# zengxiaofei/HapHiC

Hardware: NVIDIA H100
Metric: hic_pairs_per_sec_matrix_build (higher is better)
Workload: dtype int32 counts / fp32 matrix

## Files before the change

### haphic_b200/_lib.py

```python

from __future__ import annotations

import ctypes as C
import weakref
import os

import numpy as np

HERE = os.path.dirname(os.path.abspath(__file__))
LIB_PATH = os.path.join(HERE, "libhaphic_b200.so")

HH_MEM_HOST, HH_MEM_DEVICE = 0, 1


class HHError(RuntimeError):
    pass


class LinksInfo(C.Structure):
    _fields_ = [("n_records", C.c_int64), ("n_used", C.c_int64), ("nnz_full", C.c_int64), ("nnz_flank", C.c_int64),
                ("table_slots", C.c_int64)]


class MclResult(C.Structure):
    _fields_ = [("rounds", C.c_int32), ("converged", C.c_int32), ("nnz", C.c_int64), ("products", C.c_int64),
                ("bytes", C.c_int64)]


class PreexpInfo(C.Structure):
    _fields_ = [("mode", C.c_int32), ("a_planes", C.c_int32), ("passes", C.c_int32), ("cta_group", C.c_int32),
                ("stages", C.c_int32), ("chunk_kb", C.c_int32), ("total_ms", C.c_float), ("densify_ms", C.c_float),
                ("gemm_ms", C.c_float), ("clip_ms", C.c_float), ("flops", C.c_double), ("products", C.c_int64),
                ("clip", C.c_float), ("b_planes", C.c_int32), ("fmt_a", C.c_int32), ("fmt_b", C.c_int32), ("k_chunks", C.c_int32)]


class MclStepInfo(C.Structure):
    _fields_ = [("it", C.c_int32), ("iter0", C.c_int32), ("iter0_w", C.c_int32), ("blk", C.c_int32), ("blk_f16", C.c_int32),
                ("blk_chunk", C.c_int32), ("blk_ldk", C.c_int64), ("n_win", C.c_int32), ("n_big", C.c_int32),
                ("wmax", C.c_int32), ("small", C.c_int32), ("small_cols", C.c_int32), ("small_overflow", C.c_int32),
                ("col", C.c_int32), ("col_cols", C.c_int32), ("col_w", C.c_int32), ("col_smem", C.c_int32),
                ("col_track", C.c_int32), ("col_flat", C.c_int32)]


class CorrectRoundInfo(C.Structure):
    _fields_ = [("n_examined", C.c_int32), ("n_broken", C.c_int32), ("n_breaks", C.c_int32), ("n_frag", C.c_int32),
                ("n_links", C.c_int64)]


HH_PREEXP_AUTO, HH_PREEXP_SPARSE, HH_PREEXP_DENSE = 0, 1, 2

_P = C.c_void_p
_SIGNATURES = {
    "hh_version": (C.c_int, []),
    "hh_last_error": (C.c_char_p, []),
    "hh_ctx_create": (C.c_int, [C.c_int, C.POINTER(_P)]),
    "hh_ctx_destroy": (C.c_int, [_P]),
    "hh_ctx_sync": (C.c_int, [_P]),
    "hh_ctx_stream": (_P, [_P]),
    "hh_ctx_device": (C.c_int, [_P]),
    "hh_ctx_sm_count": (C.c_int, [_P]),
    "hh_ctx_launches": (C.c_int64, [_P]),
    "hh_ctx_mem_available": (C.c_int, [_P, C.POINTER(C.c_size_t)]),
    "hh_links_create": (C.c_int, [_P, C.c_int32, _P, _P, _P, C.c_int64, C.c_int64, C.POINTER(_P)]),
    "hh_links_create_frags": (C.c_int, [_P, C.c_int32, _P, _P, C.c_int32, _P, _P, _P, C.c_int64, C.c_int64, C.c_int64,
                                        C.POINTER(_P)]),
    "hh_links_add": (C.c_int, [_P, _P, C.c_int64, C.c_int64, C.c_int]),
    "hh_links_add_async": (C.c_int, [_P, _P, C.c_int64, C.c_int64]),
    "hh_links_finish": (C.c_int, [_P, C.POINTER(LinksInfo)]),
    "hh_links_agg_info": (C.c_int, [_P, C.POINTER(C.c_int64), C.POINTER(C.c_int64), C.POINTER(C.c_int64)]),
    "hh_links_fetch": (C.c_int, [_P, _P, _P, _P, _P, _P, _P, _P]),
    "hh_links_fetch_phased": (C.c_int, [_P, _P, C.c_double, _P, _P, _P, _P, C.POINTER(C.c_int64)]),
    "hh_links_set_ul_pairs": (C.c_int, [_P, _P, _P, _P, C.c_int64]),
    "hh_links_fetch_ctg": (C.c_int, [_P, _P]),
    "hh_stats_create": (C.c_int, [_P, C.c_int32, _P, _P, _P, _P, C.c_int64, C.POINTER(_P)]),
    "hh_stats_rank": (C.c_int, [_P, _P, C.c_int32, C.POINTER(C.c_int64)]),
    "hh_stats_fetch_ranked": (C.c_int, [_P, _P, _P, _P, _P]),
    "hh_stats_best": (C.c_int, [_P, _P, C.c_int32, _P, C.c_int, _P, _P, _P, _P, _P, _P]),
    "hh_stats_destroy": (C.c_int, [_P]),
    "hh_links_export": (C.c_int, [_P, _P, _P]),
    "hh_links_merge": (C.c_int, [_P, _P, C.c_int64, _P, C.c_int64, C.c_int64]),
    "hh_links_route": (C.c_int, [_P, _P, C.c_int64, C.c_int64, C.c_int, _P, _P, _P]),
    "hh_links_add_routed": (C.c_int, [_P, _P, _P, C.c_int64]),
    "hh_links_finish_partition": (C.c_int, [_P, _P]),
    "hh_links_adopt": (C.c_int, [_P, _P, C.c_int64, _P, C.c_int64, C.c_int64, C.c_int64]),
    "hh_links_destroy": (C.c_int, [_P]),
    "hh_links_linked_index": (C.c_int, [_P, _P, _P, C.POINTER(C.c_int32)]),
    "hh_matrix_from_links": (C.c_int, [_P, _P, _P, C.c_int32, C.c_int, C.c_int, C.POINTER(_P)]),
    "hh_links_linked_index_phased": (C.c_int, [_P, _P, C.c_int, _P, C.c_double, _P, C.POINTER(C.c_int32)]),
    "hh_matrix_from_links_phased": (C.c_int, [_P, _P, _P, C.c_int32, C.c_int, C.c_int, _P, C.c_double, C.POINTER(_P)]),
    "hh_matrix_from_links_ex": (C.c_int, [_P, _P, _P, C.c_int32, C.c_int, C.c_int, _P, C.c_double, _P, _P, C.POINTER(_P)]),
    "hh_matrix_rank_sums": (C.c_int, [_P, C.c_int, _P]),
    "hh_matrix_from_csc": (C.c_int, [_P, C.c_int32, _P, _P, _P, C.POINTER(_P)]),
    "hh_matrix_info": (C.c_int, [_P, C.POINTER(C.c_int32), C.POINTER(C.c_int64)]),
    "hh_matrix_fetch_csc": (C.c_int, [_P, _P, _P, _P]),
    "hh_matrix_destroy": (C.c_int, [_P]),
    "hh_mcl_create": (C.c_int, [_P, C.c_int, C.c_int32, C.c_int32, C.POINTER(_P)]),
    "hh_mcl_create_ex": (C.c_int, [_P, C.c_int, C.c_int32, C.c_int32, C.c_int, C.POINTER(_P)]),
    "hh_mcl_choose_preexp": (C.c_int, [_P, C.c_int, C.c_int, C.POINTER(C.c_int)]),
    "hh_mcl_footprint": (C.c_int, [_P, C.c_int, C.c_int32, C.c_int, C.c_double, C.POINTER(C.c_size_t), C.POINTER(C.c_size_t)]),
    "hh_mcl_preexp_info": (C.c_int, [_P, C.POINTER(PreexpInfo)]),
    "hh_mcl_info": (C.c_int, [_P, C.POINTER(C.c_int32), C.POINTER(C.c_int64), C.POINTER(C.c_int64),
                              C.POINTER(C.c_float), C.POINTER(C.c_float)]),
    "hh_mcl_fetch_m0": (C.c_int, [_P, _P, _P, _P]),
    "hh_mcl_fetch_m1": (C.c_int, [_P, _P]),
    "hh_mcl_fetch_m1_cols": (C.c_int, [_P, C.c_int32, C.c_int32, _P]),
    "hh_mcl_run": (C.c_int, [_P, C.c_double, C.c_int, C.c_double, C.POINTER(MclResult), _P, _P, _P, _P]),
    "hh_mcl_fetch_result": (C.c_int, [_P, _P, _P, _P]),
    "hh_mcl_begin": (C.c_int, [_P, C.c_double, C.c_double]),
    "hh_mcl_step": (C.c_int, [_P, C.c_int, C.POINTER(C.c_int64), C.POINTER(C.c_int64), C.POINTER(C.c_float),
                              C.POINTER(C.c_float)]),
    "hh_mcl_pack": (C.c_int, [_P, _P, _P, _P]),
    "hh_mcl_unpack": (C.c_int, [_P, C.c_int32, C.c_int32, _P, _P, _P, C.c_int64]),
    "hh_mcl_commit": (C.c_int, [_P]),
    "hh_mcl_step_info": (C.c_int, [_P, C.POINTER(MclStepInfo)]),
    "hh_mcl_set_block": (C.c_int, [_P, C.c_int32, C.c_int32]),
    "hh_mcl_destroy": (C.c_int, [_P]),
    "hh_correct_create": (C.c_int, [_P, C.c_int32, _P, C.c_int64, C.POINTER(_P)]),
    "hh_correct_add": (C.c_int, [_P, _P, C.c_int64, C.c_int]),
    "hh_correct_round": (C.c_int, [_P, C.c_double, C.c_double, C.c_int64, C.c_int, C.POINTER(CorrectRoundInfo)]),
    "hh_correct_fetch_breaks": (C.c_int, [_P, _P, _P, _P]),
    "hh_correct_info": (C.c_int, [_P, C.POINTER(C.c_int32), C.POINTER(C.c_int64), C.POINTER(C.c_int64)]),
    "hh_correct_fetch_cov": (C.c_int, [_P, _P, _P, _P]),
    "hh_correct_set_layout": (C.c_int, [_P, _P, _P, _P, C.c_int32]),
    "hh_correct_remap": (C.c_int, [_P, _P, _P, C.c_int64, C.c_int]),
    "hh_correct_destroy": (C.c_int, [_P]),
    "hh_contact_create": (C.c_int, [_P, C.c_int32, _P, _P, _P, _P, _P, _P, C.c_int32, C.c_int64, C.POINTER(_P)]),
    "hh_contact_load": (C.c_int, [_P, C.c_int32, _P, C.POINTER(_P)]),
    "hh_contact_add": (C.c_int, [_P, _P, C.c_int64, C.c_int]),
    "hh_contact_add_async": (C.c_int, [_P, _P, C.c_int64]),
    "hh_contact_error": (C.c_int, [_P, C.POINTER(C.c_int64), C.POINTER(C.c_int32), C.POINTER(C.c_int32),
                                   C.POINTER(C.c_int64)]),
    "hh_contact_finish": (C.c_int, [_P]),
    "hh_contact_info": (C.c_int, [_P, C.POINTER(C.c_int32), C.POINTER(C.c_int32), C.POINTER(C.c_int64)]),
    "hh_contact_fetch": (C.c_int, [_P, _P]),
    "hh_contact_kr": (C.c_int, [_P, C.c_int32, _P, _P, C.c_double, C.c_double, C.c_double, C.c_int32, C.c_int32, _P, _P,
                                _P, _P]),
    "hh_contact_normalize": (C.c_int, [_P, C.c_int, C.c_int32, _P, _P, _P, _P, _P, C.POINTER(C.c_double),
                                       C.POINTER(C.c_double), C.POINTER(C.c_int64)]),
    "hh_contact_destroy": (C.c_int, [_P]),
    "hh_pairs_open":(C.c_int, [C.c_char_p, _P, C.c_int32, C.c_char_p, C.c_int, C.c_int, C.POINTER(_P)]),
    "hh_pairs_next": (C.c_int, [_P, _P, C.c_int64, C.POINTER(C.c_int64)]),
    "hh_pairs_close": (C.c_int, [_P]),
    "hh_pairs_write": (C.c_int, [C.c_char_p, _P, C.c_int32, _P, C.c_int64, C.c_int64, C.c_int, C.c_int]),
    "hh_bam_open": (C.c_int, [C.c_char_p, C.c_char_p, C.c_int32, C.c_int, C.c_int, C.POINTER(_P)]),
    "hh_bam_header_text": (C.c_int, [_P, C.POINTER(C.c_char_p), C.POINTER(C.c_int64)]),
    "hh_bam_next": (C.c_int, [_P, _P, C.c_int64, C.POINTER(C.c_int64)]),
    "hh_bam_close": (C.c_int, [_P]),
    "hh_ul_open": (C.c_int, [C.c_char_p, C.c_int, C.c_int32, C.c_int64, C.c_int64, C.c_double, C.c_int64, C.POINTER(_P)]),
    "hh_ul_info": (C.c_int, [_P, C.POINTER(C.c_int32), C.POINTER(C.c_int64), C.POINTER(C.c_int64), C.POINTER(C.c_int64)]),
    "hh_ul_fetch": (C.c_int, [_P, _P, _P, _P]),
    "hh_ul_close": (C.c_int, [_P]),
    "hh_pickle_links": (C.c_int, [C.c_char_p, _P, C.c_int32, _P, _P, C.c_int64, _P, _P, _P]),
    "hh_pickle_links_mixed": (C.c_int, [C.c_char_p, _P, C.c_int32, _P, _P, C.c_int64, _P, _P]),
    "hh_clm_from_records": (C.c_int, [C.c_char_p, _P, C.c_int32, _P, C.c_int64, _P, _P, C.c_int]),
}

_lib = None


def exported_symbols():
    return sorted(_SIGNATURES)


def load():
    global _lib
    if _lib is not None:
        return _lib
    if not os.path.exists(LIB_PATH):
        raise HHError(
            "{} is missing: build it with `python -c 'import __graft_entry__ as g; g.build()'` "
            "(or `python -m haphic_b200.build`). haphic_b200 has no CPU fallback.".format(LIB_PATH))
    lib = C.CDLL(LIB_PATH)
    for name, (res, args) in _SIGNATURES.items():
        fn = getattr(lib, name)
        fn.restype = res
        fn.argtypes = args
    _lib = lib
    return lib


def check(rc: int):
    if rc != 0:
        msg = load().hh_last_error()
        raise HHError("libhaphic_b200 error {}: {}".format(rc, msg.decode() if msg else "?"))


def ptr(x):
    if x is None:
        return None
    if isinstance(x, np.ndarray):
        return x.ctypes.data_as(C.c_void_p)
    if hasattr(x, "data_ptr"):
        return C.c_void_p(x.data_ptr())
    if isinstance(x, int):
        return C.c_void_p(x)
    raise TypeError("cannot take the address of {!r}".format(type(x)))


class Context:

    def __init__(self, device: int = 0):
        self._h = C.c_void_p()
        lib = load()
        check(lib.hh_ctx_create(int(device), C.byref(self._h)))
        self.device = int(device)
        self._children = weakref.WeakSet()

    def adopt(self, obj):
        self._children.add(obj)

    @property
    def handle(self):
        if not self._h:
            raise HHError("context already closed")
        return self._h

    def sync(self):
        check(load().hh_ctx_sync(self.handle))

    @property
    def stream(self) -> int:
        return int(load().hh_ctx_stream(self.handle) or 0)

    @property
    def sm_count(self) -> int:
        return load().hh_ctx_sm_count(self.handle)

    @property
    def launches(self) -> int:
        return int(load().hh_ctx_launches(self.handle))

    def close(self):
        if self._h:
            for obj in sorted(self._children, key=lambda o: -getattr(o, "_close_order", 0)):
                obj.close()
            load().hh_ctx_destroy(self._h)
            self._h = C.c_void_p()

    def __enter__(self):
        return self

    def __exit__(self, *exc):
        self.close()

    def __del__(self):
        try:
            self.close()
        except Exception:
            pass
```

### haphic_b200/csrc/hh_common.cuh

```cuda
#pragma once

#include <cuda_runtime.h>
#include <stdint.h>
#include <stdio.h>
#include <stdarg.h>
#include <string.h>
#include <new>
#include <vector>

#include "../../include/haphic_b200.h"

void hh_set_error(const char* fmt, ...);

#define HH_CUDA(expr)                                                                         \
    do {                                                                                      \
        cudaError_t _e = (expr);                                                              \
        if (_e != cudaSuccess) {                                                              \
            hh_set_error("%s:%d: %s failed: %s", __FILE__, __LINE__, #expr, cudaGetErrorString(_e)); \
            return (_e == cudaErrorMemoryAllocation) ? HH_ERR_NOMEM : HH_ERR_CUDA;            \
        }                                                                                     \
    } while (0)

#define HH_CHECK(expr)                                                                        \
    do {                                                                                      \
        int _rc = (expr);                                                                     \
        if (_rc != HH_OK) return _rc;                                                         \
    } while (0)

#define HH_REQUIRE(cond, code, ...)                                                           \
    do {                                                                                      \
        if (!(cond)) {                                                                        \
            hh_set_error(__VA_ARGS__);                                                        \
            return (code);                                                                    \
        }                                                                                     \
    } while (0)

#define HH_LAUNCH(ctx, kernel, grid, block, smem, ...)                                        \
    do {                                                                                      \
        kernel<<<(grid), (block), (smem), (ctx)->stream>>>(__VA_ARGS__);                      \
        (ctx)->launches++;                                                                    \
        HH_CUDA(cudaGetLastError());                                                          \
    } while (0)

struct hh_ctx {
    int device;
    int sm_count;
    size_t smem_optin;
    size_t l2_bytes;
    cudaStream_t stream;
    int64_t launches;
    uint64_t* h_scratch;
    uint64_t* d_scratch;
    struct ws_block {
        void* p;
        size_t bytes;
        bool used;
        uint64_t tick;
    };
    std::vector<ws_block>* ws;
    uint64_t ws_tick;
};

void* hh_ws_alloc_bytes(hh_ctx* ctx, size_t bytes);
bool hh_ws_release(hh_ctx* ctx, void* p);
void hh_ws_free_ptr(hh_ctx* ctx, void* p);
template <typename T>
static inline int hh_ws_alloc(hh_ctx* ctx, T** p, size_t count) {
    *p = reinterpret_cast<T*>(hh_ws_alloc_bytes(ctx, (count ? count : 1) * sizeof(T)));
    return *p ? HH_OK : HH_ERR_NOMEM;
}
template <typename T>
static inline void hh_ws_free(hh_ctx* ctx, T*& p) {
    if (p) hh_ws_free_ptr(ctx, (void*)p);
    p = nullptr;
}

extern thread_local hh_ctx* hh_tls_ctx;
struct hh_scope {
    hh_ctx* prev;
    explicit hh_scope(hh_ctx* c) : prev(hh_tls_ctx) {
        hh_tls_ctx = c;
        if (c) cudaSetDevice(c->device);
    }
    ~hh_scope() { hh_tls_ctx = prev; }
};

#define HH_WS_MIN ((size_t)32 << 20)
template <typename T>
static inline int hh_dmalloc(T** p, size_t count) {
    *p = nullptr;
    if (count == 0) count = 1;
    if (hh_tls_ctx && count * sizeof(T) >= HH_WS_MIN) {
        *p = reinterpret_cast<T*>(hh_ws_alloc_bytes(hh_tls_ctx, count * sizeof(T)));
        return *p ? HH_OK : HH_ERR_NOMEM;
    }
    cudaError_t e = hh_tls_ctx ? cudaMallocAsync((void**)p, count * sizeof(T), hh_tls_ctx->stream)
                               : cudaMalloc((void**)p, count * sizeof(T));
    if (e != cudaSuccess) {
        hh_set_error("cudaMalloc of %zu bytes failed: %s", count * sizeof(T), cudaGetErrorString(e));
        cudaGetLastError();
        return HH_ERR_NOMEM;
    }
    return HH_OK;
}
template <typename T>
static inline void hh_dfree(T*& p) {
    if (p) {
        if (hh_ws_release(hh_tls_ctx, (void*)p)) {
        } else if (hh_tls_ctx) {
            cudaFreeAsync((void*)p, hh_tls_ctx->stream);
        } else {
            cudaFree((void*)p);
        }
    }
    p = nullptr;
}

#define HH_FULL_MASK 0xffffffffu

__device__ __forceinline__ int hh_lane() { return threadIdx.x & 31; }
__device__ __forceinline__ int hh_warp() { return threadIdx.x >> 5; }

__device__ __forceinline__ double hh_warp_sum(double v) {
#pragma unroll
    for (int o = 16; o > 0; o >>= 1) v += __shfl_xor_sync(HH_FULL_MASK, v, o);
    return v;
}
__device__ __forceinline__ int hh_warp_sum(int v) {
#pragma unroll
    for (int o = 16; o > 0; o >>= 1) v += __shfl_xor_sync(HH_FULL_MASK, v, o);
    return v;
}
__device__ __forceinline__ unsigned long long hh_warp_sum(unsigned long long v) {
#pragma unroll
    for (int o = 16; o > 0; o >>= 1) v += __shfl_xor_sync(HH_FULL_MASK, v, o);
    return v;
}
template <typename T>
__device__ __forceinline__ T hh_warp_incl_scan(T v) {
#pragma unroll
    for (int o = 1; o < 32; o <<= 1) {
        const T t = __shfl_up_sync(HH_FULL_MASK, v, o);
        if (hh_lane() >= o) v += t;
    }
    return v;
}
__device__ __forceinline__ float hh_warp_max(float v) {
#pragma unroll
    for (int o = 16; o > 0; o >>= 1) v = fmaxf(v, __shfl_xor_sync(HH_FULL_MASK, v, o));
    return v;
}

__device__ __forceinline__ int4 hh_ld_stream(const int4* p) {
    int4 r;
    asm volatile("ld.global.nc.L1::no_allocate.v4.s32 {%0, %1, %2, %3}, [%4];"
                 : "=r"(r.x), "=r"(r.y), "=r"(r.z), "=r"(r.w)
                 : "l"(p));
    return r;
}
__device__ __forceinline__ float4 hh_ld_stream_f4(const float4* p) {
    float4 r;
    asm volatile("ld.global.nc.L1::no_allocate.v4.f32 {%0, %1, %2, %3}, [%4];"
                 : "=f"(r.x), "=f"(r.y), "=f"(r.z), "=f"(r.w)
                 : "l"(p));
    return r;
}

template <typename K>
static inline int hh_resident_grid(hh_ctx* ctx, K kernel, int threads, size_t smem, int* grid) {
    int per_sm = 0;
    HH_CUDA(cudaOccupancyMaxActiveBlocksPerMultiprocessor(&per_sm, kernel, threads, smem));
    HH_REQUIRE(per_sm > 0, HH_ERR_CUDA, "a kernel of %d threads and %zu bytes of shared memory does not fit an SM", threads, smem);
    *grid = ctx->sm_count * per_sm;
    return HH_OK;
}

__global__ void hh_k_scan_small(const int* __restrict__ in, int64_t* __restrict__ out, int n);
int hh_exclusive_scan_i32(hh_ctx* ctx, const int* d_in, int64_t* d_out, int n);
```

### haphic_b200/csrc/hh_links.cu

```cuda
#include "hh_common.cuh"
#include "hh_internal.cuh"
#include <cub/cub.cuh>
#include <stdlib.h>
#include <algorithm>
#include <vector>

#define HH_EMPTY_KEY 0xFFFFFFFFFFFFFFFFull
#define HH_NONE32 0xFFFFFFFFu

struct __align__(32) hh_slot {
    uint32_t first_full, first_flank, full, flank, ht, th, tt, pad;
};

struct hh_partset {
    int4* buf;
    unsigned long long* cursor;
    uint64_t pcap;
    int64_t sized_for, sent;
};

struct hh_links {
    hh_ctx* ctx;
    int32_t n_ctg;
    int64_t flank_bp;
    int32_t* d_len;
    int32_t* d_rank;
    uint8_t* d_nx;
    int32_t n_src;
    int32_t* d_src_rank;
    int32_t* d_fbase;
    int64_t bin_size;
    unsigned long long* d_ctg;
    uint64_t* d_keys;
    hh_slot* d_vals;
    uint64_t cap;
    unsigned long long* d_counters;
    int64_t n_records, stream_end;
    int64_t known_unique, since_known;
    bool finished;
    bool ordered;
    int64_t nnz, nnz_flank, n_used;
    int64_t peer_used;
    uint32_t* d_compact;
    int4* d_stage[2];
    cudaEvent_t ev_copied[2], ev_consumed[2];
    cudaStream_t copy_stream;
    int64_t stage_records;
    int mode;
    int npart_log;
    uint64_t scap;
    int64_t agg_buckets, agg_smem, agg_fallback;
    uint64_t spill_cap;
    std::vector<hh_partset> psets;
    int4* d_spill;
    unsigned long long* d_spill_cursor;
    int64_t capacity_hint;
    int32_t* d_index;
    int32_t n_linked;
    uint8_t* d_keep;
    int32_t* d_hap;
    bool phased;
    int32_t* d_deg;
    int64_t n_pass;
    uint64_t gen;
    bool ix_valid;
    uint64_t ix_gen;
    int ix_normalize;
    double ix_w;
    std::vector<uint8_t> ix_keep;
    std::vector<int32_t> ix_hap;
    unsigned long long* d_ul_key = nullptr;
    int32_t* d_ul_slot = nullptr;
    int64_t n_ul = 0;
};

__device__ __forceinline__ uint64_t hh_mix64(uint64_t k) {
    k ^= k >> 33;
    k *= 0xff51afd7ed558ccdull;
    k ^= k >> 33;
    k *= 0xc4ceb9fe1a85ec53ull;
    k ^= k >> 33;
    return k;
}

__device__ __forceinline__ uint64_t hh_probe_insert(uint64_t* __restrict__ keys, uint64_t cap, uint64_t key, bool* inserted) {
    const uint64_t mask = cap - 1;
    uint64_t slot = hh_mix64(key) & mask;
    *inserted = false;
    for (uint64_t probes = 0; probes < cap; ++probes) {
        uint64_t k = *((volatile uint64_t*)(keys + slot));
        if (k == key) return slot;
        if (k == HH_EMPTY_KEY) {
            unsigned long long prev = atomicCAS((unsigned long long*)(keys + slot), (unsigned long long)HH_EMPTY_KEY,
                                                (unsigned long long)key);
            if (prev == HH_EMPTY_KEY) {
                *inserted = true;
                return slot;
            }
            if (prev == key) return slot;
        }
        slot = (slot + 1) & mask;
    }
    return cap;
}

__global__ void hh_k_links_init(uint64_t* __restrict__ keys, hh_slot* __restrict__ vals, uint64_t cap) {
    const uint64_t stride = (uint64_t)gridDim.x * blockDim.x;
    for (uint64_t s = (uint64_t)blockIdx.x * blockDim.x + threadIdx.x; s < cap; s += stride) {
        keys[s] = HH_EMPTY_KEY;
        uint4* v = reinterpret_cast<uint4*>(vals + s);
        v[0] = make_uint4(HH_NONE32, HH_NONE32, 0u, 0u);
        v[1] = make_uint4(0u, 0u, 0u, 0u);
    }
}

#define HH_F_FLANK 1u
#define HH_F_TI 2u
#define HH_F_TJ 4u

struct hh_pair {
    int a, b;
    unsigned flags;
};

__device__ __forceinline__ uint64_t hh_pair_key(int a, int b) { return ((uint64_t)(uint32_t)a << 32) | (uint64_t)(uint32_t)b; }

__device__ __forceinline__ void hh_swap_ends(int& a, int& b, int& pa, int& pb) {
    int t = a; a = b; b = t;
    t = pa; pa = pb; pb = t;
}

__device__ __forceinline__ void hh_pair_flags(int a, int b, int pa, int pb, const int32_t* __restrict__ ctg_len,
                                              const uint8_t* __restrict__ in_nx, int64_t flank_bp, hh_pair* out) {
    const int64_t coord_i = (int64_t)pa + 1, coord_j = (int64_t)pb + 1;
    const int64_t li = ctg_len[a], lj = ctg_len[b];
    const bool fi = (flank_bp == 0) || (coord_i <= flank_bp) || (coord_i > li - flank_bp);
    const bool fj = (flank_bp == 0) || (coord_j <= flank_bp) || (coord_j > lj - flank_bp);
    out->a = a;
    out->b = b;
    out->flags = ((fi && fj && in_nx[a] && in_nx[b]) ? HH_F_FLANK : 0u)
                 | ((coord_i * 2 > li) ? HH_F_TI : 0u) | ((coord_j * 2 > lj) ? HH_F_TJ : 0u);
}

__device__ __forceinline__ bool hh_classify_contig(int4 r, int32_t n_ctg, const int32_t* __restrict__ ctg_len,
                                                   const int32_t* __restrict__ name_rank, const uint8_t* __restrict__ in_nx,
                                                   int64_t flank_bp, hh_pair* out) {
    int a = r.x, b = r.z, pa = r.y, pb = r.w;
    if (a == b || (unsigned)a >= (unsigned)n_ctg || (unsigned)b >= (unsigned)n_ctg) return false;
    if (name_rank[a] > name_rank[b]) hh_swap_ends(a, b, pa, pb);
    hh_pair_flags(a, b, pa, pb, ctg_len, in_nx, flank_bp, out);
    return true;
}

__device__ __forceinline__ int64_t hh_floor_div(int64_t x, int64_t d) { return x >= 0 ? x / d : -((-x + d - 1) / d); }

__device__ __forceinline__ bool hh_to_bin(int& f, int& p, int nbins, int64_t bin_size) {
    const int64_t nb = ((int64_t)p + 1 + bin_size - 1) / bin_size;
    const bool exists = p >= 0 && nb >= 1 && nb <= (int64_t)nbins;
    f += (int)(nb - 1);
    p = (int)((int64_t)p - (nb - 1) * bin_size);
    return exists;
}

__device__ __forceinline__ bool hh_classify_frag(int4 r, int32_t n_src, const int32_t* __restrict__ src_rank,
                                                 const int32_t* __restrict__ fbase, int64_t bin_size, const int32_t* __restrict__ ctg_len,
                                                 const int32_t* __restrict__ name_rank, const uint8_t* __restrict__ in_nx,
                                                 int64_t flank_bp, uint32_t idx, unsigned long long* __restrict__ counters,
                                                 hh_pair* out) {
    int a = r.x, b = r.z, pa = r.y, pb = r.w;
    if ((unsigned)a >= (unsigned)n_src || (unsigned)b >= (unsigned)n_src) return false;
    if (a == b && fbase[a + 1] - fbase[a] <= 1) return false;
    if (src_rank[a] > src_rank[b] || (a == b && pa > pb)) hh_swap_ends(a, b, pa, pb);
    int fa = fbase[a], fb = fbase[b];
    const int na = fbase[a + 1] - fa, nb = fbase[b + 1] - fb;
    if (a == b && hh_floor_div((int64_t)pa, bin_size) == hh_floor_div((int64_t)pb, bin_size)) return false;
    bool bad = false;
    if (na > 1) bad = !hh_to_bin(fa, pa, na, bin_size);
    if (nb > 1) bad = !hh_to_bin(fb, pb, nb, bin_size) || bad;
    if (bad) {
        atomicAdd(counters + 5, 1ull);
        atomicMax(counters + 6, (unsigned long long)idx + 1ull);
        return false;
    }
    if (fa == fb) return false;
    if ((na > 1 || nb > 1) && name_rank[fa] > name_rank[fb]) hh_swap_ends(fa, fb, pa, pb);
    hh_pair_flags(fa, fb, pa, pb, ctg_len, in_nx, flank_bp, out);
    return true;
}

struct hh_group {
    bool leader;
    uint32_t first_all, first_flank;
    unsigned full, flank, ht, th, tt;
};

__device__ __forceinline__ hh_group hh_warp_fold(bool ok, uint64_t key, uint32_t idx, unsigned flags) {
    const int lane = threadIdx.x & 31;
    if (!ok) key = HH_EMPTY_KEY - 1 - (uint64_t)lane;
    const unsigned peers = __match_any_sync(HH_FULL_MASK, key);
    const bool fl = ok && (flags & HH_F_FLANK), ti = (flags & HH_F_TI) != 0, tj = (flags & HH_F_TJ) != 0;
    hh_group g;
    g.first_all = __reduce_min_sync(peers, ok ? idx : HH_NONE32);
    g.first_flank = __reduce_min_sync(peers, fl ? idx : HH_NONE32);
    const unsigned b_fl = __ballot_sync(HH_FULL_MASK, fl);
    const unsigned b_ht = __ballot_sync(HH_FULL_MASK, ok && !ti && tj);
    const unsigned b_th = __ballot_sync(HH_FULL_MASK, ok && ti && !tj);
    const unsigned b_tt = __ballot_sync(HH_FULL_MASK, ok && ti && tj);
    g.leader = ok && lane == (__ffs(peers) - 1);
    g.full = __popc(peers);
    g.flank = __popc(peers & b_fl);
    g.ht = __popc(peers & b_ht);
    g.th = __popc(peers & b_th);
    g.tt = __popc(peers & b_tt);
    return g;
}

__device__ __forceinline__ void hh_slot_update(hh_slot* v, const hh_group& g) {
    atomicAdd(&v->full, g.full);
    atomicMin(&v->first_full, g.first_all);
    if (g.flank) {
        atomicAdd(&v->flank, g.flank);
        atomicMin(&v->first_flank, g.first_flank);
    }
    if (g.ht) atomicAdd(&v->ht, g.ht);
    if (g.th) atomicAdd(&v->th, g.th);
    if (g.tt) atomicAdd(&v->tt, g.tt);
}

__device__ __forceinline__ void hh_entry_store(uint32_t* __restrict__ o, uint64_t key, uint32_t full, uint32_t flank, uint32_t first_full,
                                               uint32_t first_flank, uint32_t ht, uint32_t th, uint32_t tt) {
    o[HH_E_I] = (uint32_t)(key >> 32);
    o[HH_E_J] = (uint32_t)key;
    o[HH_E_FULL] = full;
    o[HH_E_FLANK] = flank;
    o[HH_E_FIRST_FULL] = first_full;
    o[HH_E_FIRST_FLANK] = first_flank;
    o[HH_E_HT] = ht;
    o[HH_E_TH] = th;
    o[HH_E_TT] = tt;
}

__device__ __forceinline__ void hh_entry_store(uint32_t* __restrict__ o, uint64_t key, uint4 v0, uint4 v1) {
    hh_entry_store(o, key, v0.z, v0.w, v0.x, v0.y, v1.x, v1.y, v1.z);
}

__device__ __forceinline__ unsigned int hh_block_rank(unsigned int cnt, unsigned int* s_wtot, unsigned int* total) {
    const int lane = threadIdx.x & 31, wv = threadIdx.x >> 5;
    unsigned int incl = cnt;
#pragma unroll
    for (int o = 1; o < 32; o <<= 1) {
        const unsigned int t = __shfl_up_sync(HH_FULL_MASK, incl, o);
        if (lane >= o) incl += t;
    }
    __syncthreads();
    if (lane == 31) s_wtot[wv] = incl;
    __syncthreads();
    unsigned int before = 0, all = 0;
#pragma unroll
    for (int k = 0; k < 8; ++k) {
        const unsigned int t = s_wtot[k];
        before += (k < wv) ? t : 0u;
        all += t;
    }
    *total = all;
    return before + incl - cnt;
}

__global__ void __launch_bounds__(256)
hh_k_links_insert(const int4* __restrict__ rec, int64_t n_rec, uint32_t stream_off, int32_t n_ctg,
                  const int32_t* __restrict__ ctg_len, const int32_t* __restrict__ name_rank,
                  const uint8_t* __restrict__ in_nx, int64_t flank_bp, uint64_t* __restrict__ keys,
                  hh_slot* __restrict__ vals, uint64_t cap, unsigned long long* __restrict__ ctg_links,
                  unsigned long long* __restrict__ counters, const int32_t* __restrict__ src_rank,
                  const int32_t* __restrict__ fbase, int64_t bin_size, int32_t n_src, const uint32_t* __restrict__ pos) {
    __shared__ unsigned int s_new, s_used, s_over;
    if (threadIdx.x == 0) {
        s_new = 0;
        s_used = 0;
        s_over = 0;
    }
    __syncthreads();
    const int lane = threadIdx.x & 31;
    const int64_t stride = (int64_t)gridDim.x * blockDim.x;
    unsigned int my_new = 0, my_used = 0;
    for (int64_t i0 = (int64_t)blockIdx.x * blockDim.x + (threadIdx.x - lane); i0 < n_rec; i0 += stride) {
        const int64_t i = i0 + lane;
        bool ok = i < n_rec;
        hh_pair p = {0, 0, 0u};
        uint32_t idx = HH_NONE32;
        if (ok) {
            const int4 r = hh_ld_stream(rec + i);
            idx = pos ? pos[i] : stream_off + (uint32_t)i;
            ok = fbase == nullptr ? hh_classify_contig(r, n_ctg, ctg_len, name_rank, in_nx, flank_bp, &p)
                                  : hh_classify_frag(r, n_src, src_rank, fbase, bin_size, ctg_len, name_rank, in_nx, flank_bp, idx,
                                                     counters, &p);
        }
        if (ok) my_used++;
        const uint64_t key = hh_pair_key(p.a, p.b);
        const hh_group g = hh_warp_fold(ok, key, idx, p.flags);
        if (g.leader) {
            bool inserted;
            const uint64_t slot = hh_probe_insert(keys, cap, key, &inserted);
            if (slot >= cap) {
                s_over = 1;
            } else {
                if (inserted) my_new++;
                hh_slot_update(vals + slot, g);
                if (g.flank) {
                    atomicAdd(ctg_links + p.a, (unsigned long long)g.flank);
                    atomicAdd(ctg_links + p.b, (unsigned long long)g.flank);
                }
            }
        }
    }
    if (my_new) atomicAdd(&s_new, my_new);
    if (my_used) atomicAdd(&s_used, my_used);
    __syncthreads();
    if (threadIdx.x == 0) {
        if (s_new) atomicAdd(counters + 0, (unsigned long long)s_new);
        if (s_used) atomicAdd(counters + 1, (unsigned long long)s_used);
        if (s_over) atomicExch(counters + 2, 1ull);
    }
}

#define HH_PART_TILE 4096
#define HH_PART_MAX 1024

#define HH_STAGE_SMEM ((size_t)HH_PART_TILE * sizeof(int4))

__device__ __forceinline__ unsigned int hh_tile_scan(unsigned int* c, int n, unsigned int* s_wtot) {
    const int lane = threadIdx.x & 31, wv = threadIdx.x >> 5;
    const int per = (n + 511) >> 9, lo = threadIdx.x * per;
    __syncthreads();
    unsigned int sum = 0;
    for (int k = 0; k < per; ++k)
        if (lo + k < n) sum += c[lo + k];
    unsigned int incl = sum;
#pragma unroll
    for (int o = 1; o < 32; o <<= 1) {
        const unsigned int t = __shfl_up_sync(HH_FULL_MASK, incl, o);
        if (lane >= o) incl += t;
    }
    if (lane == 31) s_wtot[wv] = incl;
    __syncthreads();
    unsigned int run = incl - sum, all = 0;
#pragma unroll
    for (int k = 0; k < 16; ++k) {
        const unsigned int t = s_wtot[k];
        run += (k < wv) ? t : 0u;
        all += t;
    }
    for (int k = 0; k < per; ++k) {
        if (lo + k < n) {
            const unsigned int t = c[lo + k];
            c[lo + k] = run;
            run += t;
        }
    }
    __syncthreads();
    return all;
}

__global__ void __launch_bounds__(512, 2)
hh_k_part_scatter(const int4* __restrict__ rec, int64_t n_rec, uint32_t stream_off, int32_t n_ctg, const int32_t* __restrict__ ctg_len,
                  const int32_t* __restrict__ name_rank, const uint8_t* __restrict__ in_nx, int64_t flank_bp, int npart_log,
                  int4* __restrict__ pbuf, uint64_t pcap, unsigned long long* __restrict__ cursor, int4* __restrict__ spill,
                  uint64_t spill_cap, unsigned long long* __restrict__ spill_cursor, unsigned long long* __restrict__ counters) {
    extern __shared__ int4 s_stage[];
    __shared__ unsigned int s_cnt[HH_PART_MAX];
    __shared__ unsigned long long s_base[HH_PART_MAX];
    __shared__ unsigned int s_wtot[16];
    __shared__ unsigned int s_used;
    const int npart = 1 << npart_log;
    const int64_t tiles = (n_rec + HH_PART_TILE - 1) / HH_PART_TILE;
    unsigned int my_used = 0;
    if (threadIdx.x == 0) s_used = 0;
    for (int64_t t = blockIdx.x; t < tiles; t += gridDim.x) {
        for (int k = threadIdx.x; k < npart; k += 512) s_cnt[k] = 0;
        __syncthreads();
        int4 out[8];
        unsigned int rnk[8];
#pragma unroll
        for (int k = 0; k < 8; ++k) {
            const int64_t i = t * HH_PART_TILE + (int64_t)k * 512 + threadIdx.x;
            rnk[k] = HH_NONE32;
            if (i < n_rec) {
                hh_pair pr;
                if (hh_classify_contig(hh_ld_stream(rec + i), n_ctg, ctg_len, name_rank, in_nx, flank_bp, &pr)) {
                    const int p = (int)(hh_mix64(hh_pair_key(pr.a, pr.b)) >> (64 - npart_log));
                    rnk[k] = atomicAdd(&s_cnt[p], 1u);
                    out[k] = make_int4(pr.a, pr.b, (int)(stream_off + (uint32_t)i), (int)(pr.flags | ((unsigned)p << 8)));
                    my_used++;
                }
            }
        }
        __syncthreads();
        for (int k = threadIdx.x; k < npart; k += 512)
            if (s_cnt[k]) s_base[k] = atomicAdd(cursor + k, (unsigned long long)s_cnt[k]);
        const unsigned int n_tile = hh_tile_scan(s_cnt, npart, s_wtot);
#pragma unroll
        for (int k = 0; k < 8; ++k)
            if (rnk[k] != HH_NONE32) s_stage[s_cnt[(unsigned)out[k].w >> 8] + rnk[k]] = out[k];
        __syncthreads();
        for (unsigned int e = threadIdx.x; e < n_tile; e += 512) {
            const int4 r = s_stage[e];
            const unsigned int p = (unsigned)r.w >> 8;
            const unsigned long long q = s_base[p] + (e - s_cnt[p]);
            if (q < pcap) {
                pbuf[(size_t)p * (size_t)pcap + (size_t)q] = r;
            } else {
                const unsigned long long sq = atomicAdd(spill_cursor, 1ull);
                if (sq < spill_cap) spill[sq] = r;
                else atomicExch(counters + 2, 3ull);
            }
        }
        __syncthreads();
    }
    my_used = (unsigned)hh_warp_sum((int)my_used);
    if ((threadIdx.x & 31) == 0 && my_used) atomicAdd(&s_used, my_used);
    __syncthreads();
    if (threadIdx.x == 0 && s_used) atomicAdd(counters + 1, (unsigned long long)s_used);
}

#define HH_AGG_MEAN 2048
#define HH_SUB_MAX_LOG 12
#define HH_AGG_SLOTS 2048
#define HH_AGG_LIST (HH_AGG_SLOTS / 4 * 3)
#define HH_AGG_THREADS 256
#define HH_AGG_HOT 32

__device__ __forceinline__ uint32_t hh_bucket_of(int4 r, int bucket_log) {
    return (uint32_t)(hh_mix64(hh_pair_key(r.x, r.y)) >> (64 - bucket_log));
}

__global__ void __launch_bounds__(512)
hh_k_part_hist(const int4* __restrict__ pbuf, uint64_t pcap, const unsigned long long* __restrict__ cursor, int npart_log, int64_t tpr,
               const int4* __restrict__ spill, int64_t n_spill, int bucket_log, unsigned int* __restrict__ bcnt) {
    __shared__ unsigned int s_cnt[1 << HH_SUB_MAX_LOG];
    const int sub_log = bucket_log - npart_log, nsub = 1 << sub_log;
    const int64_t region_tiles = ((int64_t)1 << npart_log) * tpr;
    const int64_t tiles = region_tiles + (n_spill + HH_PART_TILE - 1) / HH_PART_TILE;
    for (int64_t t = blockIdx.x; t < tiles; t += gridDim.x) {
        if (t >= region_tiles) {
            const int64_t base = (t - region_tiles) * HH_PART_TILE;
            for (int k = threadIdx.x; k < HH_PART_TILE; k += 512)
                if (base + k < n_spill) atomicAdd(bcnt + hh_bucket_of(hh_ld_stream(spill + base + k), bucket_log), 1u);
            continue;
        }
        const int p = (int)(t / tpr);
        const uint64_t start = (uint64_t)(t % tpr) * HH_PART_TILE;
        const uint64_t fill = min((uint64_t)cursor[p], pcap);
        if (start >= fill) continue;
        for (int k = threadIdx.x; k < nsub; k += 512) s_cnt[k] = 0;
        __syncthreads();
        const int4* reg = pbuf + (size_t)p * (size_t)pcap;
#pragma unroll
        for (int k = 0; k < 8; ++k) {
            const uint64_t i = start + (uint64_t)k * 512 + threadIdx.x;
            if (i < fill) atomicAdd(&s_cnt[hh_bucket_of(hh_ld_stream(reg + i), bucket_log) & (nsub - 1)], 1u);
        }
        __syncthreads();
        for (int k = threadIdx.x; k < nsub; k += 512)
            if (s_cnt[k]) atomicAdd(bcnt + ((size_t)p << sub_log) + k, s_cnt[k]);
        __syncthreads();
    }
}

__global__ void __launch_bounds__(512, 2)
hh_k_part_scatter2(const int4* __restrict__ pbuf, uint64_t pcap, const unsigned long long* __restrict__ cursor, int npart_log, int64_t tpr,
                   const int4* __restrict__ spill, int64_t n_spill, int bucket_log, const int64_t* __restrict__ boff,
                   unsigned int* __restrict__ bfill, int4* __restrict__ out, uint64_t n_out, unsigned long long* __restrict__ counters) {
    extern __shared__ int4 s_stage[];
    __shared__ unsigned int s_cnt[1 << HH_SUB_MAX_LOG];
    __shared__ unsigned int s_base[1 << HH_SUB_MAX_LOG];
    __shared__ unsigned int s_wtot[16];
    const int sub_log = bucket_log - npart_log, nsub = 1 << sub_log;
    const int64_t region_tiles = ((int64_t)1 << npart_log) * tpr;
    const int64_t tiles = region_tiles + (n_spill + HH_PART_TILE - 1) / HH_PART_TILE;
    for (int64_t t = blockIdx.x; t < tiles; t += gridDim.x) {
        if (t >= region_tiles) {
            const int64_t base = (t - region_tiles) * HH_PART_TILE;
            for (int k = threadIdx.x; k < HH_PART_TILE; k += 512) {
                if (base + k >= n_spill) break;
                const int4 r = hh_ld_stream(spill + base + k);
                const uint32_t b = hh_bucket_of(r, bucket_log);
                const uint64_t q = (uint64_t)boff[b] + atomicAdd(bfill + b, 1u);
                if (q < n_out) out[q] = r;
                else atomicExch(counters + 2, 6ull);
            }
            continue;
        }
        const int p = (int)(t / tpr);
        const uint64_t start = (uint64_t)(t % tpr) * HH_PART_TILE;
        const uint64_t fill = min((uint64_t)cursor[p], pcap);
        if (start >= fill) continue;
        for (int k = threadIdx.x; k < nsub; k += 512) s_cnt[k] = 0;
        __syncthreads();
        const int4* reg = pbuf + (size_t)p * (size_t)pcap;
        int4 r[8];
        uint32_t at[8];
#pragma unroll
        for (int k = 0; k < 8; ++k) {
            const uint64_t i = start + (uint64_t)k * 512 + threadIdx.x;
            at[k] = HH_NONE32;
            if (i < fill) {
                r[k] = hh_ld_stream(reg + i);
                const uint32_t sub = hh_bucket_of(r[k], bucket_log) & (nsub - 1);
                at[k] = (sub << 16) | atomicAdd(&s_cnt[sub], 1u);
            }
        }
        __syncthreads();
        for (int k = threadIdx.x; k < nsub; k += 512)
            if (s_cnt[k]) s_base[k] = atomicAdd(bfill + ((size_t)p << sub_log) + k, s_cnt[k]);
        const unsigned int n_tile = hh_tile_scan(s_cnt, nsub, s_wtot);
#pragma unroll
        for (int k = 0; k < 8; ++k)
            if (at[k] != HH_NONE32) s_stage[s_cnt[at[k] >> 16] + (at[k] & 0xFFFFu)] = r[k];
        __syncthreads();
        for (unsigned int e = threadIdx.x; e < n_tile; e += 512) {
            const int4 rec = s_stage[e];
            const uint32_t sub = hh_bucket_of(rec, bucket_log) & (nsub - 1);
            const size_t b = ((size_t)p << sub_log) + sub;
            const uint64_t q = (uint64_t)boff[b] + s_base[sub] + (e - s_cnt[sub]);
            if (q < n_out) out[q] = rec;
            else atomicExch(counters + 2, 6ull);
        }
        __syncthreads();
    }
}

#define HH_PK_FLANK 12
#define HH_PK_HT 24
#define HH_PK_TH 36
#define HH_PK_TT 48
#define HH_PK_MASK 0xFFFull
#define HH_PK_HEAD (1ull << 63)

struct hh_run {
    unsigned long long c;
    uint32_t first_full, first_flank;
};

struct hh_run_op {
    __device__ __forceinline__ hh_run operator()(const hh_run& a, const hh_run& b) const {
        if (b.c & HH_PK_HEAD) return b;
        return hh_run{a.c + b.c, min(a.first_full, b.first_full), min(a.first_flank, b.first_flank)};
    }
};

template <typename K>
__device__ __forceinline__ int hh_lower_bound(const K* a, int n, K k) {
    int lo = 0, hi = n;
    while (lo < hi) {
        const int mid = (lo + hi) >> 1;
        if (a[mid] < k) lo = mid + 1;
        else hi = mid;
    }
    return lo;
}

template <typename K, int ITEMS>
struct hh_bc_smem {
    typedef cub::BlockRadixSort<K, HH_AGG_THREADS, ITEMS, uint32_t> sort_t;
    typedef cub::BlockScan<hh_run, HH_AGG_THREADS> run_scan_t;
    typedef cub::BlockScan<unsigned int, HH_AGG_THREADS> cnt_scan_t;
    K key[HH_AGG_LIST];
    uint32_t val[HH_E_WORDS - 2][HH_AGG_LIST];
    uint32_t z[HH_AGG_THREADS * ITEMS];
    union {
        typename sort_t::TempStorage sort;
        struct {
            K first[HH_AGG_THREADS], last[HH_AGG_THREADS];
        } edge;
        K fresh[HH_AGG_THREADS * ITEMS];
    } u;
    typename run_scan_t::TempStorage run_scan;
    typename cnt_scan_t::TempStorage cnt_scan;
    unsigned long long base;
    int bucket;
};

template <typename K, int ITEMS>
__global__ void __launch_bounds__(HH_AGG_THREADS, 3)
hh_k_bucket_count(const int4* __restrict__ rec, const int64_t* __restrict__ boff, int nbuckets, uint64_t hot, int kbits,
                  uint32_t* __restrict__ compact, uint64_t compact_cap, unsigned long long* __restrict__ ctg_links,
                  unsigned long long* __restrict__ counters, unsigned long long* __restrict__ agg, uint32_t* __restrict__ fallback) {
    typedef hh_bc_smem<K, ITEMS> smem_t;
    constexpr int S = HH_AGG_THREADS * ITEMS;
    extern __shared__ __align__(16) unsigned char hh_agg_smem[];
    smem_t& sm = *reinterpret_cast<smem_t*>(hh_agg_smem);
    const int t = threadIdx.x;
    const K jmask = ((K)1 << kbits) - 1;
    const hh_run none = {HH_PK_HEAD, HH_NONE32, HH_NONE32};
    unsigned int nfl = 0, n_done = 0;
    for (;;) {
        __syncthreads();
        if (t == 0) sm.bucket = (int)atomicAdd(agg + 0, 1ull);
        __syncthreads();
        const int bk = sm.bucket;
        if (bk >= nbuckets) break;
        const int64_t lo = boff[bk], n = boff[bk + 1] - lo;
        if ((uint64_t)n > hot) {
            if (t == 0) fallback[atomicAdd(agg + 1, 1ull)] = (uint32_t)bk;
            continue;
        }
        int tsize = HH_AGG_THREADS;
        while (tsize < HH_AGG_SLOTS && (int64_t)tsize * 2 < n * 3) tsize <<= 1;
        const int limit = tsize / 4 * 3;
        int na = 0;
        bool abandon = false;
        for (int64_t c0 = 0; c0 < n; c0 += S) {
            const int m = (int)min((int64_t)S, n - c0);
            K key[ITEMS];
            uint32_t pay[ITEMS];
            __syncthreads();
#pragma unroll
            for (int q = 0; q < ITEMS; ++q) {
                const int l = q * HH_AGG_THREADS + t;
                key[q] = ~(K)0;
                pay[q] = 0;
                if (l < m) {
                    const int4 r = hh_ld_stream(rec + lo + c0 + l);
                    key[q] = ((K)(uint32_t)r.x << kbits) | (K)(uint32_t)r.y;
                    pay[q] = (uint32_t)l | (((uint32_t)r.w & 7u) << 11);
                    sm.z[l] = (uint32_t)r.z;
                }
            }
            typename smem_t::sort_t(sm.u.sort).Sort(key, pay, 0, 2 * kbits);
            __syncthreads();
            sm.u.edge.first[t] = key[0];
            sm.u.edge.last[t] = key[ITEMS - 1];
            __syncthreads();
            const K prev = t > 0 ? sm.u.edge.last[t - 1] : ~(K)0;
            const K next = t + 1 < HH_AGG_THREADS ? sm.u.edge.first[t + 1] : ~(K)0;
            auto item = [&](int q) -> hh_run {
                const int pos = t * ITEMS + q;
                if (pos >= m) return none;
                const unsigned f = (pay[q] >> 11) & 7u;
                const uint32_t z = sm.z[pay[q] & 0x7FFu];
                const bool fl = f & HH_F_FLANK, ti = f & HH_F_TI, tj = f & HH_F_TJ;
                hh_run r;
                const bool head = pos == 0 || key[q] != (q ? key[q - 1] : prev);
                r.c = 1ull | ((unsigned long long)head << 63) | ((unsigned long long)fl << HH_PK_FLANK) | ((unsigned long long)(!ti && tj) << HH_PK_HT) |
                      ((unsigned long long)(ti && !tj) << HH_PK_TH) | ((unsigned long long)(ti && tj) << HH_PK_TT);
                r.first_full = z;
                r.first_flank = fl ? z : HH_NONE32;
                return r;
            };
            const hh_run_op op;
            hh_run acc = item(0);
#pragma unroll
            for (int q = 1; q < ITEMS; ++q) acc = op(acc, item(q));
            hh_run carry;
            typename smem_t::run_scan_t(sm.run_scan).ExclusiveScan(acc, carry, hh_run{0ull, HH_NONE32, HH_NONE32}, op);
            unsigned int nnew = 0;
            hh_run run = carry;
#pragma unroll
            for (int q = 0; q < ITEMS; ++q) {
                run = op(run, item(q));
                const int pos = t * ITEMS + q;
                if (pos < m && (pos + 1 == m || key[q] != (q + 1 < ITEMS ? key[q + 1] : next))) {
                    const int lb = hh_lower_bound(sm.key, na, key[q]);
                    if (lb < na && sm.key[lb] == key[q]) {
                        sm.val[HH_E_FULL - 2][lb] += (uint32_t)(run.c & HH_PK_MASK);
                        sm.val[HH_E_FLANK - 2][lb] += (uint32_t)((run.c >> HH_PK_FLANK) & HH_PK_MASK);
                        sm.val[HH_E_FIRST_FULL - 2][lb] = min(sm.val[HH_E_FIRST_FULL - 2][lb], run.first_full);
                        sm.val[HH_E_FIRST_FLANK - 2][lb] = min(sm.val[HH_E_FIRST_FLANK - 2][lb], run.first_flank);
                        sm.val[HH_E_HT - 2][lb] += (uint32_t)((run.c >> HH_PK_HT) & HH_PK_MASK);
                        sm.val[HH_E_TH - 2][lb] += (uint32_t)((run.c >> HH_PK_TH) & HH_PK_MASK);
                        sm.val[HH_E_TT - 2][lb] += (uint32_t)((run.c >> HH_PK_TT) & HH_PK_MASK);
                    } else {
                        pay[q] |= (uint32_t)(lb + 1) << 16;
                        nnew++;
                    }
                }
            }
            unsigned int rank, fresh;
            typename smem_t::cnt_scan_t(sm.cnt_scan).ExclusiveSum(nnew, rank, fresh);
            if (na + (int)fresh > limit) {
                abandon = true;
                break;
            }
            if (fresh == 0) continue;
            if (na) {
                unsigned int r = rank;
#pragma unroll
                for (int q = 0; q < ITEMS; ++q)
                    if (pay[q] >> 16) sm.u.fresh[r++] = key[q];
                __syncthreads();
                for (int hi = na; hi > 0; hi -= HH_AGG_THREADS) {
                    const int a = hi - HH_AGG_THREADS + t;
                    K k = 0;
                    uint32_t v[HH_E_WORDS - 2];
                    int d = a;
                    if (a >= 0) {
                        k = sm.key[a];
#pragma unroll
                        for (int w = 0; w < HH_E_WORDS - 2; ++w) v[w] = sm.val[w][a];
                        d = a + hh_lower_bound(sm.u.fresh, (int)fresh, k);
                    }
                    __syncthreads();
                    if (d > a) {
                        sm.key[d] = k;
#pragma unroll
                        for (int w = 0; w < HH_E_WORDS - 2; ++w) sm.val[w][d] = v[w];
                    }
                    __syncthreads();
                }
            }
            run = carry;
#pragma unroll
            for (int q = 0; q < ITEMS; ++q) {
                run = op(run, item(q));
                if ((pay[q] >> 16) == 0) continue;
                const int d = (int)(pay[q] >> 16) - 1 + (int)rank++;
                const hh_run& o = run;
                sm.key[d] = key[q];
                sm.val[HH_E_FULL - 2][d] = (uint32_t)(o.c & HH_PK_MASK);
                sm.val[HH_E_FLANK - 2][d] = (uint32_t)((o.c >> HH_PK_FLANK) & HH_PK_MASK);
                sm.val[HH_E_FIRST_FULL - 2][d] = o.first_full;
                sm.val[HH_E_FIRST_FLANK - 2][d] = o.first_flank;
                sm.val[HH_E_HT - 2][d] = (uint32_t)((o.c >> HH_PK_HT) & HH_PK_MASK);
                sm.val[HH_E_TH - 2][d] = (uint32_t)((o.c >> HH_PK_TH) & HH_PK_MASK);
                sm.val[HH_E_TT - 2][d] = (uint32_t)((o.c >> HH_PK_TT) & HH_PK_MASK);
            }
            na += (int)fresh;
        }
        if (abandon) {
            if (t == 0) fallback[atomicAdd(agg + 1, 1ull)] = (uint32_t)bk;
            continue;
        }
        __syncthreads();
        if (t == 0) sm.base = na ? atomicAdd(counters + 0, (unsigned long long)na) : 0ull;
        __syncthreads();
        const unsigned long long base = sm.base;
        for (int w = t; w < na * HH_E_WORDS; w += HH_AGG_THREADS) {
            const int e = w / HH_E_WORDS, f = w - e * HH_E_WORDS;
            const uint32_t x = f == HH_E_I ? (uint32_t)(sm.key[e] >> kbits)
                             : f == HH_E_J ? (uint32_t)(sm.key[e] & jmask) : sm.val[f - 2][e];
            if (base + e < compact_cap) compact[base * HH_E_WORDS + w] = x;
            else atomicExch(counters + 2, 5ull);
        }
        for (int e = t; e < na; e += HH_AGG_THREADS) {
            const uint32_t flank = sm.val[HH_E_FLANK - 2][e];
            if (flank) {
                nfl++;
                atomicAdd(ctg_links + (uint32_t)(sm.key[e] >> kbits), (unsigned long long)flank);
                atomicAdd(ctg_links + (uint32_t)(sm.key[e] & jmask), (unsigned long long)flank);
            }
        }
        n_done++;
    }
    nfl = (unsigned)hh_warp_sum((int)nfl);
    if ((t & 31) == 0 && nfl) atomicAdd(counters + 3, (unsigned long long)nfl);
    if (t == 0 && n_done) atomicAdd(agg + 2, (unsigned long long)n_done);
}

#define HH_FB_BATCH (1 << 19)

__global__ void hh_k_gather_buckets(const int4* __restrict__ src, const int64_t* __restrict__ src_off, const int64_t* __restrict__ pre,
                                    int nf, int4* __restrict__ dst) {
    const int64_t total = pre[nf];
    const int64_t stride = (int64_t)gridDim.x * blockDim.x;
    for (int64_t i = (int64_t)blockIdx.x * blockDim.x + threadIdx.x; i < total; i += stride) {
        int lo = 0, hi = nf - 1;
        while (lo < hi) {
            const int mid = (lo + hi + 1) >> 1;
            if (pre[mid] <= i) lo = mid;
            else hi = mid - 1;
        }
        dst[i] = hh_ld_stream(src + src_off[lo] + (i - pre[lo]));
    }
}

__device__ __forceinline__ void hh_part_count(const int4* __restrict__ prec, int64_t n, uint64_t* __restrict__ keys,
                                              hh_slot* __restrict__ vals, uint64_t cap, unsigned long long* __restrict__ counters) {
    const int lane = threadIdx.x & 31;
    const int64_t stride = (int64_t)gridDim.x * blockDim.x;
    for (int64_t i0 = (int64_t)blockIdx.x * blockDim.x + (threadIdx.x - lane); i0 < n; i0 += stride) {
        const int64_t i = i0 + lane;
        const bool ok = i < n;
        int4 r = make_int4(0, 0, 0, 0);
        if (ok) r = hh_ld_stream(prec + i);
        const uint64_t key = hh_pair_key(r.x, r.y);
        const hh_group g = hh_warp_fold(ok, key, (uint32_t)r.z, (unsigned)r.w);
        if (g.leader) {
            bool inserted;
            const uint64_t slot = hh_probe_insert(keys, cap, key, &inserted);
            if (slot >= cap) atomicExch(counters + 2, 4ull);
            else hh_slot_update(vals + slot, g);
        }
    }
}

__global__ void __launch_bounds__(256)
hh_k_part_step(const int4* __restrict__ prec, int64_t n, uint64_t* __restrict__ ckeys, hh_slot* __restrict__ cvals,
               uint64_t* __restrict__ ekeys, hh_slot* __restrict__ evals, uint64_t cap, uint32_t* __restrict__ compact,
               uint64_t compact_cap, unsigned long long* __restrict__ ctg_links, unsigned long long* __restrict__ counters) {
    if (ekeys != nullptr) {
        __shared__ unsigned int s_wtot[8];
        __shared__ unsigned long long s_base;
        unsigned int nfl = 0;
        constexpr int E = 2;
        for (uint64_t r0 = (uint64_t)blockIdx.x * (256ull * E); r0 < cap; r0 += (uint64_t)gridDim.x * (256ull * E)) {
            uint64_t key[E];
            unsigned int cnt = 0;
#pragma unroll
            for (int q = 0; q < E; ++q) {
                const uint64_t sl = r0 + (uint64_t)q * 256ull + threadIdx.x;
                key[q] = (sl < cap) ? ekeys[sl] : HH_EMPTY_KEY;
                cnt += (key[q] != HH_EMPTY_KEY) ? 1u : 0u;
            }
            unsigned int total;
            const unsigned int rank = hh_block_rank(cnt, s_wtot, &total);
            if (threadIdx.x == 0) s_base = total ? atomicAdd(counters + 0, (unsigned long long)total) : 0ull;
            __syncthreads();
            if (cnt) {
                unsigned long long pos = s_base + rank;
                uint4 v0[E], v1[E];
#pragma unroll
                for (int q = 0; q < E; ++q) {
                    if (key[q] != HH_EMPTY_KEY) {
                        const uint4* vp = reinterpret_cast<const uint4*>(evals + (r0 + (uint64_t)q * 256ull + threadIdx.x));
                        v0[q] = vp[0];
                        v1[q] = vp[1];
                    }
                }
#pragma unroll
                for (int q = 0; q < E; ++q) {
                    if (key[q] == HH_EMPTY_KEY) continue;
                    const uint64_t sl = r0 + (uint64_t)q * 256ull + threadIdx.x;
                    if (pos < compact_cap) hh_entry_store(compact + pos * HH_E_WORDS, key[q], v0[q], v1[q]);
                    else atomicExch(counters + 2, 5ull);
                    pos++;
                    if (v0[q].w) {
                        nfl++;
                        atomicAdd(ctg_links + (uint32_t)(key[q] >> 32), (unsigned long long)v0[q].w);
                        atomicAdd(ctg_links + (uint32_t)key[q], (unsigned long long)v0[q].w);
                    }
                    ekeys[sl] = HH_EMPTY_KEY;
                    uint4* vw = reinterpret_cast<uint4*>(evals + sl);
                    vw[0] = make_uint4(HH_NONE32, HH_NONE32, 0u, 0u);
                    vw[1] = make_uint4(0u, 0u, 0u, 0u);
                }
            }
        }
        nfl = (unsigned)hh_warp_sum((int)nfl);
        if ((threadIdx.x & 31) == 0 && nfl) atomicAdd(counters + 3, (unsigned long long)nfl);
    }
    if (ckeys != nullptr && n > 0) hh_part_count(prec, n, ckeys, cvals, cap, counters);
}

__global__ void hh_k_links_rehash(const uint64_t* __restrict__ okeys, const hh_slot* __restrict__ ovals, uint64_t ocap,
                                  uint64_t* __restrict__ keys, hh_slot* __restrict__ vals, uint64_t cap,
                                  unsigned long long* __restrict__ counters) {
    const uint64_t stride = (uint64_t)gridDim.x * blockDim.x;
    for (uint64_t s = (uint64_t)blockIdx.x * blockDim.x + threadIdx.x; s < ocap; s += stride) {
        const uint64_t k = okeys[s];
        if (k == HH_EMPTY_KEY) continue;
        bool inserted;
        const uint64_t slot = hh_probe_insert(keys, cap, k, &inserted);
        if (slot >= cap) {
            atomicExch(counters + 2, 1ull);
            continue;
        }
        const uint4* src = reinterpret_cast<const uint4*>(ovals + s);
        uint4* dst = reinterpret_cast<uint4*>(vals + slot);
        dst[0] = src[0];
        dst[1] = src[1];
    }
}

__global__ void hh_k_links_merge(const uint32_t* __restrict__ ent, int64_t n_ent, uint64_t* __restrict__ keys,
                                 hh_slot* __restrict__ vals, uint64_t cap, unsigned long long* __restrict__ counters) {
    __shared__ unsigned int s_new;
    if (threadIdx.x == 0) s_new = 0;
    __syncthreads();
    const int64_t stride = (int64_t)gridDim.x * blockDim.x;
    unsigned int my_new = 0, my_last = 0;
    for (int64_t e = (int64_t)blockIdx.x * blockDim.x + threadIdx.x; e < n_ent; e += stride) {
        const uint32_t* p = ent + e * HH_E_WORDS;
        const uint64_t key = ((uint64_t)p[HH_E_I] << 32) | (uint64_t)p[HH_E_J];
        bool inserted;
        const uint64_t slot = hh_probe_insert(keys, cap, key, &inserted);
        if (slot >= cap) {
            atomicExch(counters + 2, 1ull);
            continue;
        }
        if (inserted) my_new++;
        hh_slot* v = vals + slot;
        atomicAdd(&v->full, p[HH_E_FULL]);
        if (p[HH_E_FLANK]) atomicAdd(&v->flank, p[HH_E_FLANK]);
        atomicMin(&v->first_full, p[HH_E_FIRST_FULL]);
        atomicMin(&v->first_flank, p[HH_E_FIRST_FLANK]);
        my_last = max(my_last, p[HH_E_FIRST_FULL]);
        if (p[HH_E_HT]) atomicAdd(&v->ht, p[HH_E_HT]);
        if (p[HH_E_TH]) atomicAdd(&v->th, p[HH_E_TH]);
        if (p[HH_E_TT]) atomicAdd(&v->tt, p[HH_E_TT]);
    }
    if (my_new) atomicAdd(&s_new, my_new);
    my_last = __reduce_max_sync(HH_FULL_MASK, my_last);
    if ((threadIdx.x & 31) == 0 && my_last) atomicMax(counters + 4, (unsigned long long)my_last);
    __syncthreads();
    if (threadIdx.x == 0 && s_new) atomicAdd(counters + 0, (unsigned long long)s_new);
}

__global__ void hh_k_add_u64(unsigned long long* __restrict__ dst, const int64_t* __restrict__ src, int n) {
    int i = blockIdx.x * blockDim.x + threadIdx.x;
    if (i < n) dst[i] += (unsigned long long)src[i];
}

#define HH_MAX_WORLD 64

__device__ __forceinline__ int hh_owner(int a, int b, int world) {
    const uint32_t lo = (uint32_t)min(a, b), hi = (uint32_t)max(a, b);
    return (int)(hh_mix64(((uint64_t)lo << 32) | (uint64_t)hi) % (uint64_t)world);
}

__device__ __forceinline__ int hh_route_dest(const int4 r, int n_src, bool contig_mode, int world) {
    if ((unsigned)r.x >= (unsigned)n_src || (unsigned)r.z >= (unsigned)n_src) return -1;
    if (contig_mode && r.x == r.z) return -1;
    return hh_owner(r.x, r.z, world);
}

__global__ void __launch_bounds__(256)
hh_k_route_count(const int4* __restrict__ rec, int64_t n_rec, int n_src, int contig_mode, int world,
                 unsigned long long* __restrict__ counts) {
    __shared__ unsigned int s_cnt[HH_MAX_WORLD];
    if (threadIdx.x < HH_MAX_WORLD) s_cnt[threadIdx.x] = 0;
    __syncthreads();
    const int64_t stride = (int64_t)gridDim.x * blockDim.x;
    for (int64_t i = (int64_t)blockIdx.x * blockDim.x + threadIdx.x; i < n_rec; i += stride) {
        const int d = hh_route_dest(hh_ld_stream(rec + i), n_src, contig_mode != 0, world);
        if (d >= 0) atomicAdd(&s_cnt[d], 1u);
    }
    __syncthreads();
    if (threadIdx.x < world && s_cnt[threadIdx.x]) atomicAdd(counts + threadIdx.x, (unsigned long long)s_cnt[threadIdx.x]);
}

__global__ void __launch_bounds__(256)
hh_k_route_scatter(const int4* __restrict__ rec, int64_t n_rec, uint32_t stream_off, int n_src, int contig_mode, int world,
                   unsigned long long* __restrict__ cursor, int4* __restrict__ rec_out, uint32_t* __restrict__ pos_out) {
    __shared__ unsigned int s_cnt[HH_MAX_WORLD];
    __shared__ unsigned long long s_base[HH_MAX_WORLD];
    const int64_t tiles = (n_rec + 255) / 256;
    for (int64_t t = blockIdx.x; t < tiles; t += gridDim.x) {
        if (threadIdx.x < HH_MAX_WORLD) s_cnt[threadIdx.x] = 0;
        __syncthreads();
        const int64_t i = t * 256 + threadIdx.x;
        int4 r = make_int4(-1, 0, -1, 0);
        int d = -1;
        unsigned int my = 0;
        if (i < n_rec) {
            r = hh_ld_stream(rec + i);
            d = hh_route_dest(r, n_src, contig_mode != 0, world);
            if (d >= 0) my = atomicAdd(&s_cnt[d], 1u);
        }
        __syncthreads();
        if (threadIdx.x < world && s_cnt[threadIdx.x])
            s_base[threadIdx.x] = atomicAdd(cursor + threadIdx.x, (unsigned long long)s_cnt[threadIdx.x]);
        __syncthreads();
        if (d >= 0) {
            const unsigned long long q = s_base[d] + my;
            rec_out[q] = r;
            pos_out[q] = stream_off + (uint32_t)i;
        }
        __syncthreads();
    }
}

__global__ void hh_k_links_mark_slots(const uint64_t* __restrict__ keys, uint64_t cap, uint32_t* __restrict__ order) {
    const uint64_t stride = (uint64_t)gridDim.x * blockDim.x;
    for (uint64_t s = (uint64_t)blockIdx.x * blockDim.x + threadIdx.x; s < cap; s += stride)
        order[s] = (keys[s] == HH_EMPTY_KEY) ? HH_NONE32 : (uint32_t)s;
}

__global__ void hh_k_list_scatter_order(const uint32_t* __restrict__ ent, int64_t nnz, uint32_t* __restrict__ order, int64_t stream_end,
                                        unsigned long long* __restrict__ counters) {
    const int64_t stride = (int64_t)gridDim.x * blockDim.x;
    for (int64_t e = (int64_t)blockIdx.x * blockDim.x + threadIdx.x; e < nnz; e += stride) {
        const uint32_t f = ent[e * HH_E_WORDS + HH_E_FIRST_FULL];
        if ((int64_t)f < stream_end) order[f] = (uint32_t)e;
        else atomicExch(counters + 2, 2ull);
    }
}

__global__ void hh_k_list_count_flank(const uint32_t* __restrict__ ent, int64_t nnz, unsigned long long* __restrict__ counters) {
    const int64_t stride = (int64_t)gridDim.x * blockDim.x;
    unsigned int c = 0;
    for (int64_t e = (int64_t)blockIdx.x * blockDim.x + threadIdx.x; e < nnz; e += stride)
        c += ent[e * HH_E_WORDS + HH_E_FLANK] ? 1u : 0u;
    c = hh_warp_sum((int)c);
    if ((threadIdx.x & 31) == 0 && c) atomicAdd(counters + 3, (unsigned long long)c);
}

__global__ void hh_k_links_scatter_order(const uint64_t* __restrict__ keys, const hh_slot* __restrict__ vals, uint64_t cap,
                                         uint32_t* __restrict__ order, int64_t stream_end,
                                         unsigned long long* __restrict__ counters) {
    const uint64_t stride = (uint64_t)gridDim.x * blockDim.x;
    for (uint64_t s = (uint64_t)blockIdx.x * blockDim.x + threadIdx.x; s < cap; s += stride) {
        if (keys[s] == HH_EMPTY_KEY) continue;
        const uint32_t f = vals[s].first_full;
        if ((int64_t)f < stream_end) order[f] = (uint32_t)s;
        else atomicExch(counters + 2, 2ull);
    }
}

#define HH_CMP_TILE 2048

__global__ void __launch_bounds__(256)
hh_k_compact_count(const uint32_t* __restrict__ order, int64_t n, int* __restrict__ block_cnt) {
    __shared__ int s_cnt;
    if (threadIdx.x == 0) s_cnt = 0;
    __syncthreads();
    const int64_t base = (int64_t)blockIdx.x * HH_CMP_TILE + (int64_t)threadIdx.x * 8;
    int c = 0;
#pragma unroll
    for (int k = 0; k < 8; ++k) {
        const int64_t e = base + k;
        if (e < n && order[e] != HH_NONE32) c++;
    }
    c = hh_warp_sum(c);
    if ((threadIdx.x & 31) == 0 && c) atomicAdd(&s_cnt, c);
    __syncthreads();
    if (threadIdx.x == 0) block_cnt[blockIdx.x] = s_cnt;
}

__global__ void __launch_bounds__(256)
hh_k_compact_gather(const uint32_t* __restrict__ order, int64_t n, const int64_t* __restrict__ block_off,
                    const uint64_t* __restrict__ keys, const hh_slot* __restrict__ vals,
                    uint32_t* __restrict__ compact, unsigned long long* __restrict__ counters) {
    __shared__ unsigned int s_wtot[8];
    __shared__ unsigned int s_flank;
    if (threadIdx.x == 0) s_flank = 0;
    const int64_t base = (int64_t)blockIdx.x * HH_CMP_TILE + (int64_t)threadIdx.x * 8;
    uint32_t slot[8];
    unsigned int c = 0;
#pragma unroll
    for (int k = 0; k < 8; ++k) {
        const int64_t e = base + k;
        slot[k] = (e < n) ? order[e] : HH_NONE32;
        if (slot[k] != HH_NONE32) c++;
    }
    unsigned int total;
    int64_t q = block_off[blockIdx.x] + hh_block_rank(c, s_wtot, &total);
    unsigned int nfl = 0;
#pragma unroll
    for (int k = 0; k < 8; ++k) {
        if (slot[k] == HH_NONE32) continue;
        uint32_t* o = compact + q * HH_E_WORDS;
        q++;
        if (keys == nullptr) {
            const uint32_t* src = reinterpret_cast<const uint32_t*>(vals) + (size_t)slot[k] * HH_E_WORDS;
#pragma unroll
            for (int w = 0; w < HH_E_WORDS; ++w) o[w] = src[w];
            continue;
        }
        const uint4* v = reinterpret_cast<const uint4*>(vals + slot[k]);
        const uint4 v0 = v[0], v1 = v[1];
        hh_entry_store(o, keys[slot[k]], v0, v1);
        if (v0.w) nfl++;
    }
    if (nfl) atomicAdd(&s_flank, nfl);
    __syncthreads();
    if (threadIdx.x == 0 && s_flank) atomicAdd(counters + 3, (unsigned long long)s_flank);
}

__global__ void __launch_bounds__(256)
hh_k_touch(const uint32_t* __restrict__ compact, int64_t nnz, const uint8_t* __restrict__ keep,
           const unsigned long long* __restrict__ ctg_tot, int normalize, const int32_t* __restrict__ hap, double w,
           unsigned long long* __restrict__ touch, int* __restrict__ deg, unsigned long long* __restrict__ n_pass) {
    __shared__ unsigned int s_pass;
    if (threadIdx.x == 0) s_pass = 0;
    __syncthreads();
    unsigned int my_pass = 0;
    const int64_t stride = (int64_t)gridDim.x * blockDim.x;
    for (int64_t e = (int64_t)blockIdx.x * blockDim.x + threadIdx.x; e < nnz; e += stride) {
        const uint32_t* p = compact + e * HH_E_WORDS;
        if (p[HH_E_FLANK] == 0) continue;
        const uint32_t i = p[HH_E_I], j = p[HH_E_J];
        if (!keep[i] || !keep[j]) continue;
        double x;
        if (!hh_flank_value(p, ctg_tot, normalize, hap, w, nullptr, nullptr, &x)) continue;
        const unsigned long long t = (unsigned long long)p[HH_E_FIRST_FLANK] * 2ull;
        if (t < __ldcg(touch + i)) atomicMin(touch + i, t);
        if (t + 1ull < __ldcg(touch + j)) atomicMin(touch + j, t + 1ull);
        atomicAdd(deg + i, 1);
        atomicAdd(deg + j, 1);
        my_pass++;
    }
    my_pass = (unsigned)hh_warp_sum((int)my_pass);
    if ((threadIdx.x & 31) == 0 && my_pass) atomicAdd(&s_pass, my_pass);
    __syncthreads();
    if (threadIdx.x == 0 && s_pass) atomicAdd(n_pass, (unsigned long long)s_pass);
}

__global__ void hh_k_iota_i32(int32_t* __restrict__ p, int n) {
    const int k = blockIdx.x * blockDim.x + threadIdx.x;
    if (k < n) p[k] = k;
}

__global__ void hh_k_rank_sorted(const unsigned long long* __restrict__ touch_sorted, const int32_t* __restrict__ frag_sorted, int n,
                                 int32_t* __restrict__ index, unsigned long long* __restrict__ out) {
    const int k = blockIdx.x * blockDim.x + threadIdx.x;
    if (k >= n) return;
    const bool touched = touch_sorted[k] != ~0ull;
    index[frag_sorted[k]] = touched ? k : -1;
    if (touched && (k == n - 1 || touch_sorted[k + 1] == ~0ull)) out[0] = (unsigned long long)(k + 1);
}

static inline int hh_grid(hh_ctx* ctx, int per_sm) { return ctx->sm_count * per_sm; }

static inline int links_grid(hh_ctx* ctx, int64_t n) {
    return (int)std::max<int64_t>(1, std::min<int64_t>((n + 255) / 256, hh_grid(ctx, 8)));
}

static int links_alloc_table(hh_links* lk, uint64_t cap, uint64_t** keys, hh_slot** vals) {
    HH_CHECK(hh_dmalloc(keys, cap));
    int rc = hh_dmalloc(vals, cap);
    if (rc != HH_OK) {
        hh_dfree(*keys);
        return rc;
    }
    HH_LAUNCH(lk->ctx, hh_k_links_init, hh_grid(lk->ctx, 8), 256, 0, *keys, *vals, cap);
    return HH_OK;
}

static int links_read_counters(hh_links* lk, unsigned long long out[8]) {
    hh_ctx* ctx = lk->ctx;
    HH_CUDA(cudaMemcpyAsync(ctx->h_scratch, lk->d_counters, 8 * sizeof(unsigned long long), cudaMemcpyDeviceToHost, ctx->stream));
    HH_CUDA(cudaStreamSynchronize(ctx->stream));
    for (int k = 0; k < 8; ++k) out[k] = ctx->h_scratch[k];
    return HH_OK;
}

static int links_need_table(hh_links* lk) {
    if (lk->d_keys) return HH_OK;
    uint64_t cap = 1ull << 16;
    const double want = lk->capacity_hint > 0 ? (double)lk->capacity_hint / 0.5 : 0.0;
    while ((double)cap < want) cap <<= 1;
    HH_CHECK(links_alloc_table(lk, cap, &lk->d_keys, &lk->d_vals));
    lk->cap = cap;
    return HH_OK;
}

static int links_ensure_capacity(hh_links* lk, int64_t incoming) {
    const double max_load = 0.7;
    HH_CHECK(links_need_table(lk));
    if ((double)(lk->known_unique + lk->since_known + incoming) <= max_load * (double)lk->cap) return HH_OK;
    unsigned long long c[8];
    HH_CHECK(links_read_counters(lk, c));
    HH_REQUIRE(c[2] == 0, HH_ERR_CAPACITY, "hh_links: hash table overflow (capacity %llu slots)", (unsigned long long)lk->cap);
    lk->known_unique = (int64_t)c[0];
    lk->since_known = 0;
    if ((double)(lk->known_unique + incoming) <= max_load * (double)lk->cap) return HH_OK;
    uint64_t ncap = lk->cap;
    while ((double)(lk->known_unique + incoming) > max_load * (double)ncap) ncap <<= 1;
    uint64_t* nkeys;
    hh_slot* nvals;
    HH_CHECK(links_alloc_table(lk, ncap, &nkeys, &nvals));
    HH_LAUNCH(lk->ctx, hh_k_links_rehash, hh_grid(lk->ctx, 8), 256, 0, lk->d_keys, lk->d_vals, lk->cap, nkeys, nvals, ncap,
              lk->d_counters);
    HH_CUDA(cudaStreamSynchronize(lk->ctx->stream));
    hh_dfree(lk->d_keys);
    hh_dfree(lk->d_vals);
    lk->d_keys = nkeys;
    lk->d_vals = nvals;
    lk->cap = ncap;
    return HH_OK;
}

static int links_create_common(hh_ctx* ctx, int32_t n_key, const int64_t* key_len, const int32_t* key_rank, const uint8_t* in_nx,
                               int64_t flank_bp, int64_t capacity_hint, int32_t n_src, const int32_t* src_rank,
                               const int32_t* frag_base, int64_t bin_size, hh_links** out) {
    *out = nullptr;
    std::vector<int32_t> len32(n_key);
    for (int32_t c = 0; c < n_key; ++c) {
        HH_REQUIRE(key_len[c] > 0 && key_len[c] <= 0x7fffffffLL, HH_ERR_UNSUPPORTED,
                   "hh_links_create: object %d has length %lld; records carry int32 positions (pos_int_type int32, "
                   "HapHiC_cluster.py:116-147)", c, (long long)key_len[c]);
        HH_REQUIRE(key_rank[c] >= 0 && key_rank[c] < n_key, HH_ERR_ARG, "hh_links_create: name_rank[%d] out of range", c);
        len32[c] = (int32_t)key_len[c];
    }
    hh_links* lk = new (std::nothrow) hh_links();
    HH_REQUIRE(lk != nullptr, HH_ERR_NOMEM, "hh_links_create: out of host memory");
    lk->ctx = ctx;
    lk->n_ctg = n_key;
    lk->n_src = frag_base ? n_src : n_key;
    lk->bin_size = bin_size;
    lk->flank_bp = flank_bp;
    int rc = HH_OK;
    do {
        if ((rc = hh_dmalloc(&lk->d_len, n_key)) != HH_OK) break;
        if ((rc = hh_dmalloc(&lk->d_rank, n_key)) != HH_OK) break;
        if ((rc = hh_dmalloc(&lk->d_nx, n_key)) != HH_OK) break;
        if ((rc = hh_dmalloc(&lk->d_ctg, n_key)) != HH_OK) break;
        if ((rc = hh_dmalloc(&lk->d_counters, 8)) != HH_OK) break;
        if ((rc = hh_dmalloc(&lk->d_index, n_key)) != HH_OK) break;
        if ((rc = hh_dmalloc(&lk->d_keep, n_key)) != HH_OK) break;
        if ((rc = hh_dmalloc(&lk->d_deg, n_key)) != HH_OK) break;
        if (frag_base) {
            if ((rc = hh_dmalloc(&lk->d_src_rank, n_src)) != HH_OK) break;
            if ((rc = hh_dmalloc(&lk->d_fbase, (size_t)n_src + 1)) != HH_OK) break;
        }
    } while (0);
    if (rc != HH_OK) {
        hh_links_destroy(lk);
        return rc;
    }
    cudaStream_t st = ctx->stream;
    HH_CUDA(cudaMemcpyAsync(lk->d_len, len32.data(), n_key * sizeof(int32_t), cudaMemcpyHostToDevice, st));
    HH_CUDA(cudaMemcpyAsync(lk->d_rank, key_rank, n_key * sizeof(int32_t), cudaMemcpyHostToDevice, st));
    HH_CUDA(cudaMemcpyAsync(lk->d_nx, in_nx, n_key * sizeof(uint8_t), cudaMemcpyHostToDevice, st));
    HH_CUDA(cudaMemsetAsync(lk->d_ctg, 0, n_key * sizeof(unsigned long long), st));
    HH_CUDA(cudaMemsetAsync(lk->d_counters, 0, 8 * sizeof(unsigned long long), st));
    if (frag_base) {
        HH_CUDA(cudaMemcpyAsync(lk->d_src_rank, src_rank, (size_t)n_src * sizeof(int32_t), cudaMemcpyHostToDevice, st));
        HH_CUDA(cudaMemcpyAsync(lk->d_fbase, frag_base, ((size_t)n_src + 1) * sizeof(int32_t), cudaMemcpyHostToDevice, st));
    }
    HH_CUDA(cudaStreamSynchronize(st));
    lk->capacity_hint = capacity_hint;
    HH_CUDA(cudaStreamCreateWithFlags(&lk->copy_stream, cudaStreamNonBlocking));
    for (int k = 0; k < 2; ++k) {
        HH_CUDA(cudaEventCreateWithFlags(&lk->ev_copied[k], cudaEventDisableTiming));
        HH_CUDA(cudaEventCreateWithFlags(&lk->ev_consumed[k], cudaEventDisableTiming));
    }
    *out = lk;
    return HH_OK;
}

extern "C" int hh_links_create(hh_ctx* ctx, int32_t n_ctg, const int64_t* ctg_len, const int32_t* name_rank,
                               const uint8_t* in_nx, int64_t flank_bp, int64_t capacity_hint, hh_links** out) {
    HH_REQUIRE(ctx && out && ctg_len && name_rank && in_nx, HH_ERR_ARG, "hh_links_create: NULL argument");
    HH_REQUIRE(n_ctg > 0, HH_ERR_ARG, "hh_links_create: n_ctg must be positive");
    HH_REQUIRE(flank_bp >= 0, HH_ERR_ARG, "hh_links_create: flank_bp must be >= 0");
    hh_scope _scope(ctx);
    return links_create_common(ctx, n_ctg, ctg_len, name_rank, in_nx, flank_bp, capacity_hint, n_ctg, nullptr, nullptr, 0, out);
}

extern "C" int hh_links_create_frags(hh_ctx* ctx, int32_t n_ctg, const int32_t* ctg_rank, const int32_t* frag_base,
                                     int32_t n_frag, const int64_t* frag_len, const int32_t* frag_rank, const uint8_t* frag_in_nx,
                                     int64_t bin_size, int64_t flank_bp, int64_t capacity_hint, hh_links** out) {
    HH_REQUIRE(ctx && out && ctg_rank && frag_base && frag_len && frag_rank && frag_in_nx, HH_ERR_ARG,
               "hh_links_create_frags: NULL argument");
    HH_REQUIRE(n_ctg > 0 && n_frag >= n_ctg, HH_ERR_ARG, "hh_links_create_frags: need n_frag >= n_ctg > 0");
    HH_REQUIRE(flank_bp >= 0 && bin_size > 0, HH_ERR_ARG, "hh_links_create_frags: flank_bp >= 0 and bin_size > 0 required");
    HH_REQUIRE(frag_base[0] == 0 && frag_base[n_ctg] == n_frag, HH_ERR_ARG, "hh_links_create_frags: frag_base must span [0, n_frag]");
    for (int32_t c = 0; c < n_ctg; ++c) {
        HH_REQUIRE(frag_base[c + 1] > frag_base[c], HH_ERR_ARG, "hh_links_create_frags: contig %d has no fragment", c);
        HH_REQUIRE(ctg_rank[c] >= 0 && ctg_rank[c] < n_ctg, HH_ERR_ARG, "hh_links_create_frags: ctg_rank[%d] out of range", c);
    }
    hh_scope _scope(ctx);
    return links_create_common(ctx, n_frag, frag_len, frag_rank, frag_in_nx, flank_bp, capacity_hint, n_ctg, ctg_rank, frag_base,
                               bin_size, out);
}

static int links_env_int(const char* name, int dflt) {
    const char* v = getenv(name);
    return (v && *v) ? atoi(v) : dflt;
}

static int links_new_partset(hh_links* lk, int64_t n_rec) {
    const int npart = 1 << lk->npart_log;
    hh_partset ps;
    memset(&ps, 0, sizeof(ps));
    ps.pcap = (uint64_t)((double)n_rec / npart * 1.5) + 4096;
    ps.sized_for = n_rec;
    HH_CHECK(hh_ws_alloc(lk->ctx, &ps.buf, (size_t)npart * (size_t)ps.pcap));
    int rc = hh_dmalloc(&ps.cursor, (size_t)npart);
    if (rc != HH_OK) {
        hh_ws_free(lk->ctx, ps.buf);
        return rc;
    }
    HH_CUDA(cudaMemsetAsync(ps.cursor, 0, (size_t)npart * sizeof(unsigned long long), lk->ctx->stream));
    lk->psets.push_back(ps);
    return HH_OK;
}

static int links_size_spill(hh_links* lk) {
    int64_t sized = 0;
    for (const hh_partset& ps : lk->psets) sized += ps.sized_for;
    const uint64_t need = (uint64_t)(sized / 8) + (4u << 20);
    if (lk->d_spill && need <= lk->spill_cap) return HH_OK;
    int4* grown = nullptr;
    HH_CHECK(hh_ws_alloc(lk->ctx, &grown, (size_t)need));
    if (lk->d_spill) {
        const cudaError_t e = cudaMemcpyAsync(grown, lk->d_spill, (size_t)lk->spill_cap * sizeof(int4), cudaMemcpyDeviceToDevice,
                                              lk->ctx->stream);
        if (e != cudaSuccess) hh_ws_free(lk->ctx, grown);
        HH_CUDA(e);
        hh_ws_free(lk->ctx, lk->d_spill);
    }
    lk->d_spill = grown;
    lk->spill_cap = need;
    return HH_OK;
}

static int links_choose_mode(hh_links* lk, int64_t total) {
    if (lk->mode) return HH_OK;
    const int want = links_env_int("HH_LINKS_PARTITION", -1);
    const bool can = lk->d_fbase == nullptr && lk->d_keys == nullptr;
    const bool big = total >= (16ll << 20) && lk->n_ctg >= 2048;
    if (!can || want == 0 || (want < 0 && !big)) {
        lk->mode = 1;
        return HH_OK;
    }
    lk->mode = 2;
    int lg = 4;
    while (lg < 9 && ((int64_t)400000 << lg) < total) lg++;
    lk->npart_log = links_env_int("HH_LINKS_NPART_LOG", lg);
    if (lk->npart_log < 1) lk->npart_log = 1;
    if (lk->npart_log > 10) lk->npart_log = 10;
    HH_CHECK(links_new_partset(lk, total));
    HH_CHECK(links_size_spill(lk));
    HH_CHECK(hh_dmalloc(&lk->d_spill_cursor, 1));
    HH_CUDA(cudaMemsetAsync(lk->d_spill_cursor, 0, sizeof(unsigned long long), lk->ctx->stream));
    return HH_OK;
}

static int links_launch_insert(hh_links* lk, const int4* d_rec, int64_t n_rec, int64_t stream_offset,
                               const uint32_t* d_pos = nullptr) {
    hh_ctx* ctx = lk->ctx;
    if (lk->mode == 2 && d_pos == nullptr) {
        const int64_t tiles = (n_rec + HH_PART_TILE - 1) / HH_PART_TILE;
        int grid = 0;
        HH_CUDA(cudaFuncSetAttribute(hh_k_part_scatter, cudaFuncAttributeMaxDynamicSharedMemorySize, (int)HH_STAGE_SMEM));
        HH_CHECK(hh_resident_grid(ctx, hh_k_part_scatter, 512, HH_STAGE_SMEM, &grid));
        grid = (int)std::max<int64_t>(1, std::min<int64_t>(tiles, grid));
        const hh_partset& ps = lk->psets.back();
        HH_LAUNCH(ctx, hh_k_part_scatter, grid, 512, HH_STAGE_SMEM, d_rec, n_rec, (uint32_t)stream_offset, lk->n_ctg, lk->d_len, lk->d_rank, lk->d_nx,
                  lk->flank_bp, lk->npart_log, ps.buf, ps.pcap, ps.cursor, lk->d_spill, lk->spill_cap, lk->d_spill_cursor,
                  lk->d_counters);
        return HH_OK;
    }
    HH_CHECK(links_need_table(lk));
    HH_LAUNCH(ctx, hh_k_links_insert, links_grid(ctx, n_rec), 256, 0, d_rec, n_rec, (uint32_t)stream_offset, lk->n_ctg, lk->d_len,
              lk->d_rank, lk->d_nx, lk->flank_bp, lk->d_keys, lk->d_vals, lk->cap, lk->d_ctg, lk->d_counters, lk->d_src_rank,
              lk->d_fbase, lk->bin_size, lk->n_src, d_pos);
    return HH_OK;
}

static int links_part_room(hh_links* lk, int64_t n_rec) {
    hh_partset& ps = lk->psets.back();
    if (ps.sent > 0 && ps.sent + n_rec > ps.sized_for + ps.sized_for / 8) {
        HH_CHECK(links_new_partset(lk, n_rec));
        lk->psets.back().sent = n_rec;
        return links_size_spill(lk);
    }
    ps.sent += n_rec;
    return HH_OK;
}

static const int64_t HH_ADD_CHUNK = 1ll << 23;
static int links_add_chunks(hh_links* lk, const int4* d_rec, const uint32_t* d_pos, int64_t n_rec, int64_t stream_offset) {
    for (int64_t off = 0; off < n_rec; off += HH_ADD_CHUNK) {
        const int64_t m = std::min(n_rec - off, HH_ADD_CHUNK);
        if (lk->mode != 2) HH_CHECK(links_ensure_capacity(lk, m));
        HH_CHECK(links_launch_insert(lk, d_rec + off, m, stream_offset + off, d_pos ? d_pos + off : nullptr));
        lk->since_known += m;
    }
    return HH_OK;
}

extern "C" int hh_links_add_async(hh_links* lk, const int32_t* rec_dev, int64_t n_rec, int64_t stream_offset) {
    HH_REQUIRE(lk && (rec_dev || n_rec == 0), HH_ERR_ARG, "hh_links_add_async: NULL argument");
    hh_scope _scope(lk->ctx);
    HH_REQUIRE(!lk->finished, HH_ERR_STATE, "hh_links_add_async: stream already finished");
    HH_REQUIRE(n_rec >= 0 && stream_offset >= 0 && stream_offset + n_rec <= 0xFFFFFFFELL, HH_ERR_UNSUPPORTED,
               "hh_links_add: stream indices must fit 32 bits (offset %lld + %lld records)", (long long)stream_offset,
               (long long)n_rec);
    HH_REQUIRE(((uintptr_t)rec_dev & 15) == 0, HH_ERR_ARG, "hh_links_add: records must be 16-byte aligned");
    if (n_rec == 0) return HH_OK;
    HH_CUDA(cudaSetDevice(lk->ctx->device));
    HH_CHECK(links_choose_mode(lk, n_rec));
    if (lk->mode == 2) HH_CHECK(links_part_room(lk, n_rec));
    HH_CHECK(links_launch_insert(lk, reinterpret_cast<const int4*>(rec_dev), n_rec, stream_offset));
    lk->n_records += n_rec;
    lk->since_known += n_rec;
    if (stream_offset + n_rec > lk->stream_end) lk->stream_end = stream_offset + n_rec;
    return HH_OK;
}

extern "C" int hh_links_add(hh_links* lk, const int32_t* rec, int64_t n_rec, int64_t stream_offset, int mem) {
    HH_REQUIRE(lk && (rec || n_rec == 0), HH_ERR_ARG, "hh_links_add: NULL argument");
    hh_scope _scope(lk->ctx);
    HH_REQUIRE(!lk->finished, HH_ERR_STATE, "hh_links_add: stream already finished");
    HH_REQUIRE(mem == HH_MEM_HOST || mem == HH_MEM_DEVICE, HH_ERR_ARG, "hh_links_add: bad mem flag %d", mem);
    HH_REQUIRE(n_rec >= 0 && stream_offset >= 0 && stream_offset + n_rec <= 0xFFFFFFFELL, HH_ERR_UNSUPPORTED,
               "hh_links_add: stream indices must fit 32 bits (offset %lld + %lld records)", (long long)stream_offset,
               (long long)n_rec);
    if (n_rec == 0) return HH_OK;
    hh_ctx* ctx = lk->ctx;
    HH_CUDA(cudaSetDevice(ctx->device));
    const int64_t CH = HH_ADD_CHUNK;
    HH_CHECK(links_choose_mode(lk, n_rec));
    if (lk->mode == 2) HH_CHECK(links_part_room(lk, n_rec));
    if (mem == HH_MEM_DEVICE) {
        HH_REQUIRE(((uintptr_t)rec & 15) == 0, HH_ERR_ARG, "hh_links_add: records must be 16-byte aligned");
        HH_CHECK(links_add_chunks(lk, reinterpret_cast<const int4*>(rec), nullptr, n_rec, stream_offset));
    } else {
        if (!lk->d_stage[0]) {
            lk->stage_records = CH;
            HH_CUDA(cudaMalloc((void**)&lk->d_stage[0], (size_t)CH * sizeof(int4)));
            HH_CUDA(cudaMalloc((void**)&lk->d_stage[1], (size_t)CH * sizeof(int4)));
        }
        int buf = 0;
        for (int64_t off = 0; off < n_rec; off += CH, buf ^= 1) {
            const int64_t m = (n_rec - off < CH) ? (n_rec - off) : CH;
            HH_CUDA(cudaStreamWaitEvent(lk->copy_stream, lk->ev_consumed[buf], 0));
            HH_CUDA(cudaMemcpyAsync(lk->d_stage[buf], rec + off * 4, (size_t)m * 16, cudaMemcpyHostToDevice, lk->copy_stream));
            HH_CUDA(cudaEventRecord(lk->ev_copied[buf], lk->copy_stream));
            if (lk->mode != 2) HH_CHECK(links_ensure_capacity(lk, m));
            HH_CUDA(cudaStreamWaitEvent(ctx->stream, lk->ev_copied[buf], 0));
            HH_CHECK(links_launch_insert(lk, lk->d_stage[buf], m, stream_offset + off));
            HH_CUDA(cudaEventRecord(lk->ev_consumed[buf], ctx->stream));
            lk->since_known += m;
        }
        HH_CUDA(cudaStreamSynchronize(ctx->stream));
    }
    lk->n_records += n_rec;
    if (stream_offset + n_rec > lk->stream_end) lk->stream_end = stream_offset + n_rec;
    return HH_OK;
}

static void links_free_partsets(hh_links* lk) {
    for (hh_partset& ps : lk->psets) {
        hh_ws_free(lk->ctx, ps.buf);
        hh_dfree(ps.cursor);
    }
    lk->psets.clear();
    hh_ws_free(lk->ctx, lk->d_spill);
    hh_dfree(lk->d_spill_cursor);
}

static int links_bucket_log(int64_t n_used, int npart_log) {
    int b = npart_log;
    while (b < npart_log + HH_SUB_MAX_LOG && (n_used >> b) > HH_AGG_MEAN) b++;
    return b;
}

static uint64_t links_hot_records(int64_t n_used, int bucket_log) {
    const uint64_t mean = ((uint64_t)n_used + (1ull << bucket_log) - 1) >> bucket_log;
    return (uint64_t)HH_AGG_HOT * (mean > HH_AGG_MEAN / 2 ? mean : HH_AGG_MEAN / 2);
}

template <typename K, int ITEMS>
static int links_bucket_count(hh_links* lk, const int4* rec, const int64_t* boff, int nb, uint64_t hot, int kbits, uint32_t* compact,
                              uint64_t compact_cap, unsigned long long* agg, uint32_t* fallback) {
    hh_ctx* ctx = lk->ctx;
    auto kernel = hh_k_bucket_count<K, ITEMS>;
    const size_t smem = sizeof(hh_bc_smem<K, ITEMS>);
    HH_CUDA(cudaFuncSetAttribute(kernel, cudaFuncAttributeMaxDynamicSharedMemorySize, (int)smem));
    int grid = 0;
    HH_CHECK(hh_resident_grid(ctx, kernel, HH_AGG_THREADS, smem, &grid));
    HH_LAUNCH(ctx, kernel, grid, HH_AGG_THREADS, smem, rec, boff, nb, hot, kbits, compact, compact_cap, lk->d_ctg, lk->d_counters, agg,
              fallback);
    return HH_OK;
}

static int links_finish_partitioned(hh_links* lk) {
    hh_ctx* ctx = lk->ctx;
    unsigned long long c[8];
    HH_CHECK(links_read_counters(lk, c));
    HH_REQUIRE(c[2] == 0, HH_ERR_CAPACITY,
               "hh_links_finish: the spill list of the partitioned counting overflowed (a few contig pairs own most of the stream): "
               "set HH_LINKS_PARTITION=0 to use the direct hash table");
    lk->n_used = lk->peer_used + (int64_t)c[1];
    const int64_t U = (int64_t)c[1];
    HH_REQUIRE(U < (1ll << 31), HH_ERR_UNSUPPORTED,
               "hh_links_finish: %lld usable records; the partitioned counting takes fewer than 2^31: set HH_LINKS_PARTITION=0",
               (long long)U);
    unsigned long long n_spill = 0;
    HH_CUDA(cudaMemcpyAsync(&n_spill, lk->d_spill_cursor, sizeof(unsigned long long), cudaMemcpyDeviceToHost, ctx->stream));
    HH_CUDA(cudaStreamSynchronize(ctx->stream));
    const int blog = links_bucket_log(U, lk->npart_log);
    const int nb = 1 << blog;
    const uint64_t hot = links_hot_records(U, blog);
    const uint64_t compact_cap = (uint64_t)(U > 0 ? U : 1);
    unsigned int *d_bcnt = nullptr, *d_bfill = nullptr;
    uint32_t *d_fallback = nullptr, *d_stage_compact = nullptr;
    int64_t* d_boff = nullptr;
    unsigned long long* d_agg = nullptr;
    int4 *d_rec2 = nullptr, *d_fb_rec = nullptr;
    int64_t* d_fb_off = nullptr;
    uint64_t* skeys[2] = {nullptr, nullptr};
    hh_slot* svals[2] = {nullptr, nullptr};
    hh_dfree(lk->d_compact);
    int rc = [&]() -> int {
        HH_CHECK(hh_dmalloc(&d_bcnt, (size_t)nb));
        HH_CHECK(hh_dmalloc(&d_bfill, (size_t)nb));
        HH_CHECK(hh_dmalloc(&d_boff, (size_t)nb + 1));
        HH_CHECK(hh_dmalloc(&d_fallback, (size_t)nb));
        HH_CHECK(hh_dmalloc(&d_agg, 4));
        HH_CHECK(hh_ws_alloc(ctx, &d_rec2, (size_t)compact_cap));
        HH_CUDA(cudaMemsetAsync(d_bcnt, 0, (size_t)nb * sizeof(unsigned int), ctx->stream));
        HH_CUDA(cudaMemsetAsync(d_bfill, 0, (size_t)nb * sizeof(unsigned int), ctx->stream));
        HH_CUDA(cudaMemsetAsync(d_agg, 0, 4 * sizeof(unsigned long long), ctx->stream));
        int grid = 0, grid2 = 0;
        HH_CHECK(hh_resident_grid(ctx, hh_k_part_hist, 512, 0, &grid));
        HH_CUDA(cudaFuncSetAttribute(hh_k_part_scatter2, cudaFuncAttributeMaxDynamicSharedMemorySize, (int)HH_STAGE_SMEM));
        HH_CHECK(hh_resident_grid(ctx, hh_k_part_scatter2, 512, HH_STAGE_SMEM, &grid2));
        for (size_t k = 0; k < lk->psets.size(); ++k) {
            const hh_partset& ps = lk->psets[k];
            const int64_t tpr = (int64_t)((ps.pcap + HH_PART_TILE - 1) / HH_PART_TILE);
            HH_LAUNCH(ctx, hh_k_part_hist, grid, 512, 0, ps.buf, ps.pcap, ps.cursor, lk->npart_log, tpr, lk->d_spill,
                      k == 0 ? (int64_t)n_spill : 0, blog, d_bcnt);
        }
        HH_CHECK(hh_exclusive_scan_i32(ctx, reinterpret_cast<const int*>(d_bcnt), d_boff, nb));
        for (size_t k = 0; k < lk->psets.size(); ++k) {
            const hh_partset& ps = lk->psets[k];
            const int64_t tpr = (int64_t)((ps.pcap + HH_PART_TILE - 1) / HH_PART_TILE);
            HH_LAUNCH(ctx, hh_k_part_scatter2, grid2, 512, HH_STAGE_SMEM, ps.buf, ps.pcap, ps.cursor, lk->npart_log, tpr, lk->d_spill,
                      k == 0 ? (int64_t)n_spill : 0, blog, d_boff, d_bfill, d_rec2, compact_cap, lk->d_counters);
        }
        links_free_partsets(lk);
        HH_CHECK(hh_ws_alloc(ctx, &d_stage_compact, (size_t)compact_cap * HH_E_WORDS));
        HH_CUDA(cudaMemsetAsync(lk->d_counters + 0, 0, sizeof(unsigned long long), ctx->stream));
        HH_CUDA(cudaMemsetAsync(lk->d_counters + 3, 0, sizeof(unsigned long long), ctx->stream));
        int kbits = 1;
        while ((1ll << kbits) < (int64_t)lk->n_ctg) kbits++;
        auto count = 2 * kbits <= 32 ? links_bucket_count<uint32_t, 8> : links_bucket_count<uint64_t, 5>;
        HH_CHECK(count(lk, d_rec2, d_boff, nb, hot, kbits, d_stage_compact, compact_cap, d_agg, d_fallback));
        unsigned long long agg[4];
        HH_CUDA(cudaMemcpyAsync(agg, d_agg, sizeof(agg), cudaMemcpyDeviceToHost, ctx->stream));
        HH_CHECK(links_read_counters(lk, c));
        lk->agg_buckets = nb;
        lk->agg_smem = (int64_t)agg[2];
        lk->agg_fallback = (int64_t)agg[1];
        lk->scap = HH_AGG_SLOTS;
        if (agg[1]) {
            const int nf = (int)agg[1];
            std::vector<uint32_t> fb((size_t)nf);
            std::vector<int64_t> off((size_t)nb + 1), src_off((size_t)nf), pre((size_t)nf + 1, 0);
            HH_CUDA(cudaMemcpyAsync(fb.data(), d_fallback, fb.size() * sizeof(uint32_t), cudaMemcpyDeviceToHost, ctx->stream));
            HH_CUDA(cudaMemcpyAsync(off.data(), d_boff, off.size() * sizeof(int64_t), cudaMemcpyDeviceToHost, ctx->stream));
            HH_CUDA(cudaStreamSynchronize(ctx->stream));
            std::vector<int64_t> cut(1, 0);
            for (int k = 0; k < nf; ++k) {
                src_off[k] = off[fb[k]];
                const int64_t n = off[fb[k] + 1] - off[fb[k]];
                if (pre[k] > cut.back() && pre[k] + n - cut.back() > HH_FB_BATCH) cut.push_back(pre[k]);
                pre[k + 1] = pre[k] + n;
            }
            cut.push_back(pre[nf]);
            int64_t worst = 1;
            for (size_t t = 0; t + 1 < cut.size(); ++t) worst = std::max(worst, cut[t + 1] - cut[t]);
            uint64_t scap = 1ull << 12;
            while ((double)scap * 0.6 < (double)worst) scap <<= 1;
            lk->scap = scap;
            HH_CHECK(hh_dmalloc(&d_fb_off, 2 * (size_t)nf + 1));
            HH_CUDA(cudaMemcpyAsync(d_fb_off, src_off.data(), (size_t)nf * sizeof(int64_t), cudaMemcpyHostToDevice, ctx->stream));
            HH_CUDA(cudaMemcpyAsync(d_fb_off + nf, pre.data(), ((size_t)nf + 1) * sizeof(int64_t), cudaMemcpyHostToDevice, ctx->stream));
            HH_CHECK(hh_ws_alloc(ctx, &d_fb_rec, (size_t)pre[nf]));
            HH_LAUNCH(ctx, hh_k_gather_buckets, hh_grid(ctx, 8), 256, 0, d_rec2, d_fb_off, d_fb_off + nf, nf, d_fb_rec);
            hh_ws_free(ctx, d_rec2);
            for (int t = 0; t < 2; ++t) HH_CHECK(links_alloc_table(lk, scap, &skeys[t], &svals[t]));
            const int g = hh_grid(ctx, 8);
            const int nbatch = (int)cut.size() - 1;
            for (int t = 0; t <= nbatch; ++t) {
                const int cb = t & 1, eb = cb ^ 1;
                const bool have = t < nbatch;
                HH_LAUNCH(ctx, hh_k_part_step, g, 256, 0, have ? d_fb_rec + cut[t] : (const int4*)nullptr,
                          have ? cut[t + 1] - cut[t] : (int64_t)0, have ? skeys[cb] : (uint64_t*)nullptr,
                          have ? svals[cb] : (hh_slot*)nullptr, t > 0 ? skeys[eb] : (uint64_t*)nullptr,
                          t > 0 ? svals[eb] : (hh_slot*)nullptr, scap, d_stage_compact, compact_cap, lk->d_ctg, lk->d_counters);
            }
            HH_CHECK(links_read_counters(lk, c));
        }
        HH_REQUIRE(c[2] == 0, HH_ERR_CAPACITY,
                   "hh_links_finish: a bucket of the partitioned counting overflowed (code %llu): set HH_LINKS_PARTITION=0", c[2]);
        lk->nnz = (int64_t)c[0];
        lk->nnz_flank = (int64_t)c[3];
        HH_CHECK(hh_dmalloc(&lk->d_compact, (size_t)(lk->nnz > 0 ? lk->nnz : 1) * HH_E_WORDS));
        if (lk->nnz)
            HH_CUDA(cudaMemcpyAsync(lk->d_compact, d_stage_compact, (size_t)lk->nnz * HH_E_WORDS * sizeof(uint32_t), cudaMemcpyDeviceToDevice,
                                    ctx->stream));
        return HH_OK;
    }();
    hh_ws_free(ctx, d_stage_compact);
    hh_ws_free(ctx, d_rec2);
    hh_ws_free(ctx, d_fb_rec);
    hh_dfree(d_fb_off);
    hh_dfree(d_bcnt);
    hh_dfree(d_bfill);
    hh_dfree(d_boff);
    hh_dfree(d_fallback);
    hh_dfree(d_agg);
    for (int t = 0; t < 2; ++t) {
        hh_dfree(skeys[t]);
        hh_dfree(svals[t]);
    }
    links_free_partsets(lk);
    HH_CHECK(rc);
    lk->finished = true;
    lk->gen++;
    lk->ordered = false;
    return HH_OK;
}

extern "C" int hh_links_agg_info(hh_links* lk, int64_t* buckets, int64_t* smem_buckets, int64_t* fallback_buckets) {
    HH_REQUIRE(lk != nullptr, HH_ERR_ARG, "hh_links_agg_info: NULL handle");
    if (buckets) *buckets = lk->agg_buckets;
    if (smem_buckets) *smem_buckets = lk->agg_smem;
    if (fallback_buckets) *fallback_buckets = lk->agg_fallback;
    return HH_OK;
}

static int links_compact(hh_links* lk, const uint32_t* d_order, int64_t S, const uint64_t* keys, const hh_slot* vals, uint32_t* dst) {
    hh_ctx* ctx = lk->ctx;
    const int64_t nb = (S + HH_CMP_TILE - 1) / HH_CMP_TILE;
    int* d_bcnt = nullptr;
    int64_t* d_boff = nullptr;
    const int rc = [&]() -> int {
        HH_CHECK(hh_dmalloc(&d_bcnt, (size_t)nb));
        HH_CHECK(hh_dmalloc(&d_boff, (size_t)nb + 1));
        HH_LAUNCH(ctx, hh_k_compact_count, (unsigned)nb, 256, 0, d_order, S, d_bcnt);
        HH_CHECK(hh_exclusive_scan_i32(ctx, d_bcnt, d_boff, (int)nb));
        HH_LAUNCH(ctx, hh_k_compact_gather, (unsigned)nb, 256, 0, d_order, S, d_boff, keys, vals, dst, lk->d_counters);
        return HH_OK;
    }();
    hh_dfree(d_bcnt);
    hh_dfree(d_boff);
    return rc;
}

static int links_finish_direct(hh_links* lk, bool ordered, const char* who) {
    hh_ctx* ctx = lk->ctx;
    HH_CHECK(links_need_table(lk));
    unsigned long long c[8];
    HH_CHECK(links_read_counters(lk, c));
    HH_REQUIRE(c[2] == 0, HH_ERR_CAPACITY, "%s: hash table overflow (capacity %llu slots)%s", who, (unsigned long long)lk->cap,
               ordered ? ": pass a larger capacity_hint or use hh_links_add" : "");
    HH_REQUIRE(c[5] == 0, HH_ERR_ARG,
               "%s: %llu records have a position outside their contig's bins (e.g. record %llu of the stream)%s", who, c[5], c[6] - 1ull,
               ordered ? ": positions must lie in [0, contig length)" : "");
    lk->nnz = (int64_t)c[0];
    lk->n_used = lk->peer_used + (int64_t)c[1];
    HH_CUDA(cudaMemsetAsync(lk->d_counters + 3, 0, sizeof(unsigned long long), ctx->stream));
    if (ordered && lk->nnz > 0 && (int64_t)c[4] + 1 > lk->stream_end) lk->stream_end = (int64_t)c[4] + 1;
    hh_dfree(lk->d_compact);
    HH_CHECK(hh_dmalloc(&lk->d_compact, (size_t)(lk->nnz > 0 ? lk->nnz : 1) * HH_E_WORDS));
    if (lk->nnz > 0) {
        HH_REQUIRE(ordered || lk->cap <= 0xFFFFFFFFull, HH_ERR_UNSUPPORTED, "%s: table too large", who);
        const int64_t S = ordered ? lk->stream_end : (int64_t)lk->cap;
        uint32_t* d_order = nullptr;
        HH_CHECK(hh_dmalloc(&d_order, (size_t)S));
        const int rc = [&]() -> int {
            if (ordered) {
                HH_CUDA(cudaMemsetAsync(d_order, 0xFF, (size_t)S * sizeof(uint32_t), ctx->stream));
                HH_LAUNCH(ctx, hh_k_links_scatter_order, hh_grid(ctx, 8), 256, 0, lk->d_keys, lk->d_vals, lk->cap, d_order, S,
                          lk->d_counters);
            } else {
                HH_LAUNCH(ctx, hh_k_links_mark_slots, hh_grid(ctx, 8), 256, 0, lk->d_keys, lk->cap, d_order);
            }
            HH_CHECK(links_compact(lk, d_order, S, lk->d_keys, lk->d_vals, lk->d_compact));
            return links_read_counters(lk, c);
        }();
        hh_dfree(d_order);
        HH_CHECK(rc);
        HH_REQUIRE(c[2] == 0, HH_ERR_STATE, "%s: first-seen index beyond the stream end (stream_offset misuse)", who);
        lk->nnz_flank = (int64_t)c[3];
    }
    lk->finished = true;
    lk->gen++;
    lk->ordered = ordered;
    return HH_OK;
}

static void links_fill_info(hh_links* lk, hh_links_info* info, int64_t table_slots) {
    if (!info) return;
    info->n_records = lk->n_records;
    info->n_used = lk->n_used;
    info->nnz_full = lk->nnz;
    info->nnz_flank = lk->nnz_flank;
    info->table_slots = table_slots;
}

extern "C" int hh_links_finish(hh_links* lk, hh_links_info* info) {
    HH_REQUIRE(lk != nullptr, HH_ERR_ARG, "hh_links_finish: NULL handle");
    hh_scope _scope(lk->ctx);
    HH_CUDA(cudaSetDevice(lk->ctx->device));
    if (!lk->finished) HH_CHECK(lk->mode == 2 ? links_finish_partitioned(lk) : links_finish_direct(lk, true, "hh_links_finish"));
    links_fill_info(lk, info, (int64_t)(lk->mode == 2 ? lk->scap : lk->cap));
    return HH_OK;
}

__device__ __forceinline__ int hh_ul_slot(const unsigned long long* __restrict__ keys, const int32_t* __restrict__ slot, int64_t n,
                                          uint32_t i, uint32_t j) {
    const unsigned long long key = ((unsigned long long)i << 32) | j;
    int64_t lo = 0, hi = n;
    while (lo < hi) {
        const int64_t mid = (lo + hi) >> 1;
        if (keys[mid] < key) lo = mid + 1;
        else hi = mid;
    }
    return (lo < n && keys[lo] == key) ? slot[lo] : -1;
}

__global__ void hh_k_links_split(const uint32_t* __restrict__ compact, int64_t nnz, uint32_t* __restrict__ soa, int64_t ht_off,
                                 const unsigned long long* __restrict__ ul_key, const int32_t* __restrict__ ul_slot, int64_t n_ul,
                                 int* __restrict__ overflow) {
    const int64_t stride = (int64_t)gridDim.x * blockDim.x;
    for (int64_t e = (int64_t)blockIdx.x * blockDim.x + threadIdx.x; e < nnz; e += stride) {
        const uint32_t* p = compact + e * HH_E_WORDS;
#pragma unroll
        for (int w = HH_E_I; w <= HH_E_FIRST_FLANK; ++w) soa[w * nnz + e] = p[w];
        uint4 h;
        h.y = p[HH_E_HT];
        h.z = p[HH_E_TH];
        h.w = p[HH_E_TT];
        h.x = p[HH_E_FULL] - p[HH_E_HT] - p[HH_E_TH] - p[HH_E_TT];
        const int s = n_ul ? hh_ul_slot(ul_key, ul_slot, n_ul, p[HH_E_I], p[HH_E_J]) : -1;
        if (s >= 0) {
            const uint32_t hs = s == 0 ? h.x : s == 1 ? h.y : s == 2 ? h.z : h.w;
            if (p[HH_E_FULL] > 0x7FFFFFFFu || hs > 0x7FFFFFFFu) atomicExch(overflow, 1);
            soa[HH_E_FULL * nnz + e] = p[HH_E_FULL] * 2u;
            h.x = s == 0 ? h.x * 2u : h.x;
            h.y = s == 1 ? h.y * 2u : h.y;
            h.z = s == 2 ? h.z * 2u : h.z;
            h.w = s == 3 ? h.w * 2u : h.w;
        }
        reinterpret_cast<uint4*>(soa + ht_off)[e] = h;
    }
}

extern "C" int hh_links_route(hh_links* lk, const int32_t* rec_dev, int64_t n_rec, int64_t stream_offset, int world,
                              int32_t* rec_out_dev, uint32_t* pos_out_dev, int64_t* counts) {
    HH_REQUIRE(lk && counts && (n_rec == 0 || (rec_dev && rec_out_dev && pos_out_dev)), HH_ERR_ARG, "hh_links_route: NULL argument");
    HH_REQUIRE(world >= 1 && world <= HH_MAX_WORLD, HH_ERR_ARG, "hh_links_route: world must be in [1, %d]", HH_MAX_WORLD);
    HH_REQUIRE(n_rec >= 0 && stream_offset >= 0 && stream_offset + n_rec <= 0xFFFFFFFELL, HH_ERR_UNSUPPORTED,
               "hh_links_route: stream indices must fit 32 bits (offset %lld + %lld records)", (long long)stream_offset,
               (long long)n_rec);
    HH_REQUIRE((((uintptr_t)rec_dev | (uintptr_t)rec_out_dev) & 15) == 0, HH_ERR_ARG, "hh_links_route: records must be 16-byte aligned");
    hh_scope _scope(lk->ctx);
    hh_ctx* ctx = lk->ctx;
    HH_CUDA(cudaSetDevice(ctx->device));
    for (int d = 0; d < world; ++d) counts[d] = 0;
    if (n_rec == 0) return HH_OK;
    unsigned long long* d_cnt = nullptr;
    HH_CHECK(hh_dmalloc(&d_cnt, 2 * HH_MAX_WORLD));
    int rc = [&]() -> int {
        HH_CUDA(cudaMemsetAsync(d_cnt, 0, 2 * HH_MAX_WORLD * sizeof(unsigned long long), ctx->stream));
        const int contig_mode = lk->d_fbase == nullptr;
        const int grid = links_grid(ctx, n_rec);
        const int4* rec4 = reinterpret_cast<const int4*>(rec_dev);
        HH_LAUNCH(ctx, hh_k_route_count, grid, 256, 0, rec4, n_rec, lk->n_src, contig_mode, world, d_cnt);
        unsigned long long h[HH_MAX_WORLD];
        HH_CUDA(cudaMemcpyAsync(h, d_cnt, (size_t)world * sizeof(unsigned long long), cudaMemcpyDeviceToHost, ctx->stream));
        HH_CUDA(cudaStreamSynchronize(ctx->stream));
        unsigned long long base[HH_MAX_WORLD], acc = 0;
        for (int d = 0; d < world; ++d) {
            counts[d] = (int64_t)h[d];
            base[d] = acc;
            acc += h[d];
        }
        HH_CUDA(cudaMemcpyAsync(d_cnt + HH_MAX_WORLD, base, (size_t)world * sizeof(unsigned long long), cudaMemcpyHostToDevice,
                                ctx->stream));
        HH_LAUNCH(ctx, hh_k_route_scatter, grid, 256, 0, rec4, n_rec, (uint32_t)stream_offset, lk->n_src, contig_mode, world,
                  d_cnt + HH_MAX_WORLD, reinterpret_cast<int4*>(rec_out_dev), pos_out_dev);
        HH_CUDA(cudaStreamSynchronize(ctx->stream));
        return HH_OK;
    }();
    hh_dfree(d_cnt);
    HH_CHECK(rc);
    lk->n_records += n_rec;
    if (stream_offset + n_rec > lk->stream_end) lk->stream_end = stream_offset + n_rec;
    return HH_OK;
}

extern "C" int hh_links_add_routed(hh_links* lk, const int32_t* rec_dev, const uint32_t* pos_dev, int64_t n_rec) {
    HH_REQUIRE(lk && (n_rec == 0 || (rec_dev && pos_dev)), HH_ERR_ARG, "hh_links_add_routed: NULL argument");
    hh_scope _scope(lk->ctx);
    HH_REQUIRE(!lk->finished, HH_ERR_STATE, "hh_links_add_routed: stream already finished");
    HH_REQUIRE(n_rec >= 0, HH_ERR_ARG, "hh_links_add_routed: negative record count");
    HH_REQUIRE(((uintptr_t)rec_dev & 15) == 0, HH_ERR_ARG, "hh_links_add_routed: records must be 16-byte aligned");
    if (n_rec == 0) return HH_OK;
    HH_CUDA(cudaSetDevice(lk->ctx->device));
    HH_REQUIRE(lk->mode != 2, HH_ERR_STATE, "hh_links_add_routed: this table counts a partitioned stream (hh_links_add of a long stream)");
    lk->mode = 1;
    return links_add_chunks(lk, reinterpret_cast<const int4*>(rec_dev), pos_dev, n_rec, 0);
}

extern "C" int hh_links_finish_partition(hh_links* lk, hh_links_info* info) {
    HH_REQUIRE(lk != nullptr, HH_ERR_ARG, "hh_links_finish_partition: NULL handle");
    hh_scope _scope(lk->ctx);
    HH_CUDA(cudaSetDevice(lk->ctx->device));
    if (!lk->finished)
        HH_CHECK(lk->mode == 2 ? links_finish_partitioned(lk) : links_finish_direct(lk, false, "hh_links_finish_partition"));
    links_fill_info(lk, info, (int64_t)lk->cap);
    return HH_OK;
}

extern "C" int hh_links_adopt(hh_links* lk, const uint32_t* entries_dev, int64_t n_entries, const int64_t* ctg_links_dev,
                              int64_t n_records, int64_t n_used, int64_t stream_end) {
    HH_REQUIRE(lk && ctg_links_dev && (entries_dev || n_entries == 0), HH_ERR_ARG, "hh_links_adopt: NULL argument");
    HH_REQUIRE(n_entries >= 0 && stream_end >= 0 && stream_end <= 0xFFFFFFFELL, HH_ERR_ARG, "hh_links_adopt: bad sizes");
    hh_scope _scope(lk->ctx);
    hh_ctx* ctx = lk->ctx;
    HH_CUDA(cudaSetDevice(ctx->device));
    hh_dfree(lk->d_keys);
    hh_dfree(lk->d_vals);
    lk->d_keys = nullptr;
    lk->d_vals = nullptr;
    lk->cap = 0;
    hh_dfree(lk->d_compact);
    lk->d_compact = nullptr;
    lk->gen++;
    HH_CHECK(hh_dmalloc(&lk->d_compact, (size_t)(n_entries > 0 ? n_entries : 1) * HH_E_WORDS));
    HH_CUDA(cudaMemsetAsync(lk->d_counters + 2, 0, 2 * sizeof(unsigned long long), ctx->stream));
    if (n_entries) {
        HH_CUDA(cudaMemcpyAsync(lk->d_compact, entries_dev, (size_t)n_entries * HH_E_WORDS * sizeof(uint32_t), cudaMemcpyDeviceToDevice,
                                ctx->stream));
        const int grid = links_grid(ctx, n_entries);
        HH_LAUNCH(ctx, hh_k_list_count_flank, grid, 256, 0, lk->d_compact, n_entries, lk->d_counters);
    }
    HH_CUDA(cudaMemcpyAsync(lk->d_ctg, ctg_links_dev, (size_t)lk->n_ctg * sizeof(int64_t), cudaMemcpyDeviceToDevice, ctx->stream));
    unsigned long long c[8];
    HH_CHECK(links_read_counters(lk, c));
    lk->nnz = n_entries;
    lk->nnz_flank = (int64_t)c[3];
    lk->n_records = n_records;
    lk->n_used = n_used;
    lk->peer_used = 0;
    lk->stream_end = stream_end;
    lk->finished = true;
    lk->ordered = false;
    return HH_OK;
}

static int links_order_list(hh_links* lk) {
    if (lk->ordered || lk->nnz == 0) {
        lk->ordered = true;
        return HH_OK;
    }
    hh_ctx* ctx = lk->ctx;
    const int64_t S = lk->stream_end;
    uint32_t *d_order = nullptr, *d_sorted = nullptr;
    const int rc = [&]() -> int {
        HH_CHECK(hh_dmalloc(&d_order, (size_t)S));
        HH_CHECK(hh_dmalloc(&d_sorted, (size_t)lk->nnz * HH_E_WORDS));
        HH_CUDA(cudaMemsetAsync(d_order, 0xFF, (size_t)S * sizeof(uint32_t), ctx->stream));
        HH_CUDA(cudaMemsetAsync(lk->d_counters + 2, 0, sizeof(unsigned long long), ctx->stream));
        HH_LAUNCH(ctx, hh_k_list_scatter_order, links_grid(ctx, lk->nnz), 256, 0, lk->d_compact, lk->nnz, d_order, S, lk->d_counters);
        HH_CHECK(links_compact(lk, d_order, S, nullptr, reinterpret_cast<const hh_slot*>(lk->d_compact), d_sorted));
        unsigned long long c[8];
        HH_CHECK(links_read_counters(lk, c));
        HH_REQUIRE(c[2] == 0, HH_ERR_STATE, "hh_links: first-seen index beyond the stream end (stream_end misuse in hh_links_adopt)");
        return HH_OK;
    }();
    hh_dfree(d_order);
    if (rc != HH_OK) {
        hh_dfree(d_sorted);
        return rc;
    }
    hh_dfree(lk->d_compact);
    lk->d_compact = d_sorted;
    lk->ordered = true;
    return HH_OK;
}

extern "C" int hh_links_fetch(hh_links* lk, int32_t* key_i, int32_t* key_j, uint32_t* full, uint32_t* flank,
                              uint32_t* first_full, uint32_t* first_flank, uint32_t* ht) {
    HH_REQUIRE(lk != nullptr, HH_ERR_ARG, "hh_links_fetch: NULL handle");
    hh_scope _scope(lk->ctx);
    HH_REQUIRE(lk->finished, HH_ERR_STATE, "hh_links_fetch: call hh_links_finish first");
    if (lk->nnz == 0) return HH_OK;
    hh_ctx* ctx = lk->ctx;
    HH_CUDA(cudaSetDevice(ctx->device));
    HH_CHECK(links_order_list(lk));
    const int64_t nnz = lk->nnz;
    uint32_t* d_soa = nullptr;
    HH_CHECK(hh_dmalloc(&d_soa, (size_t)nnz * 10 + 4));
    int rc = [&]() -> int {
        uint32_t* base = d_soa;
        const int64_t ht_off = (6 * nnz + 3) & ~3ll;
        const int grid = links_grid(ctx, nnz);
        int* d_err = reinterpret_cast<int*>(ctx->d_scratch + 10);
        HH_CUDA(cudaMemsetAsync(d_err, 0, sizeof(int), ctx->stream));
        HH_LAUNCH(ctx, hh_k_links_split, grid, 256, 0, lk->d_compact, nnz, base, ht_off, lk->d_ul_key, lk->d_ul_slot, lk->n_ul, d_err);
        void* dst[6] = {key_i, key_j, full, flank, first_full, first_flank};
        for (int k = 0; k < 6; ++k)
            if (dst[k])
                HH_CUDA(cudaMemcpyAsync(dst[k], base + (size_t)k * nnz, (size_t)nnz * 4, cudaMemcpyDeviceToHost, ctx->stream));
        if (ht) HH_CUDA(cudaMemcpyAsync(ht, base + ht_off, (size_t)nnz * 16, cudaMemcpyDeviceToHost, ctx->stream));
        HH_CUDA(cudaMemcpyAsync(ctx->h_scratch + 10, d_err, sizeof(int), cudaMemcpyDeviceToHost, ctx->stream));
        HH_CUDA(cudaStreamSynchronize(ctx->stream));
        HH_REQUIRE(*reinterpret_cast<int*>(ctx->h_scratch + 10) == 0, HH_ERR_UNSUPPORTED,
                   "hh_links_fetch: an ultra-long-read doubled link count exceeds 2^32 - 1");
        return HH_OK;
    }();
    hh_dfree(d_soa);
    return rc;
}

__device__ __forceinline__ double hh_full_value(const uint32_t* __restrict__ p, const int32_t* __restrict__ hap, double w,
                                                bool* is_float) {
    const double x = (double)p[HH_E_FULL];
    *is_float = hap[p[HH_E_I]] != hap[p[HH_E_J]];
    return *is_float ? __dsub_rn(x, __dmul_rn(x, w)) : x;
}

__global__ void __launch_bounds__(256)
hh_k_phased_mark(const uint32_t* __restrict__ compact, int64_t nnz, const int32_t* __restrict__ hap, double w,
                 uint32_t* __restrict__ order, unsigned long long* __restrict__ n_kept) {
    const int64_t stride = (int64_t)gridDim.x * blockDim.x;
    int kept = 0;
    for (int64_t e = (int64_t)blockIdx.x * blockDim.x + threadIdx.x; e < nnz; e += stride) {
        bool f;
        const bool keep = hh_full_value(compact + e * HH_E_WORDS, hap, w, &f) != 0.0;
        order[e] = keep ? (uint32_t)e : HH_NONE32;
        kept += keep;
    }
    kept = hh_warp_sum(kept);
    if ((threadIdx.x & 31) == 0 && kept) atomicAdd(n_kept, (unsigned long long)kept);
}

__global__ void __launch_bounds__(256)
hh_k_phased_split(const uint32_t* __restrict__ kept, int64_t n, const int32_t* __restrict__ hap, double w, int32_t* __restrict__ ki,
                  int32_t* __restrict__ kj, double* __restrict__ val, uint8_t* __restrict__ flt,
                  const unsigned long long* __restrict__ ul_key, const int32_t* __restrict__ ul_slot, int64_t n_ul) {
    const int64_t stride = (int64_t)gridDim.x * blockDim.x;
    for (int64_t e = (int64_t)blockIdx.x * blockDim.x + threadIdx.x; e < n; e += stride) {
        const uint32_t* p = kept + e * HH_E_WORDS;
        bool f;
        const bool ul = n_ul && hh_ul_slot(ul_key, ul_slot, n_ul, p[HH_E_I], p[HH_E_J]) >= 0;
        val[e] = (ul ? 2.0 : 1.0) * hh_full_value(p, hap, w, &f);
        ki[e] = (int32_t)p[HH_E_I];
        kj[e] = (int32_t)p[HH_E_J];
        flt[e] = f;
    }
}

extern "C" int hh_links_fetch_phased(hh_links* lk, const int32_t* hap, double w, int32_t* key_i, int32_t* key_j, double* values,
                                     uint8_t* is_float, int64_t* n_out) {
    HH_REQUIRE(lk && hap && key_i && key_j && values && is_float && n_out, HH_ERR_ARG, "hh_links_fetch_phased: NULL argument");
    HH_REQUIRE(w >= 0.0 && w <= 1.0, HH_ERR_ARG, "hh_links_fetch_phased: phasing weight %g outside [0, 1]", w);
    hh_scope _scope(lk->ctx);
    HH_REQUIRE(lk->finished, HH_ERR_STATE, "hh_links_fetch_phased: call hh_links_finish first");
    *n_out = 0;
    if (lk->nnz == 0) return HH_OK;
    hh_ctx* ctx = lk->ctx;
    HH_CHECK(links_order_list(lk));
    const int64_t nnz = lk->nnz;
    int32_t* d_hap = nullptr;
    uint32_t *d_order = nullptr, *d_kept = nullptr;
    uint8_t* d_soa = nullptr;
    unsigned long long* d_n = nullptr;
    const int rc = [&]() -> int {
        HH_CHECK(hh_dmalloc(&d_hap, (size_t)lk->n_ctg));
        HH_CHECK(hh_dmalloc(&d_order, (size_t)nnz));
        HH_CHECK(hh_dmalloc(&d_n, 1));
        HH_CUDA(cudaMemcpyAsync(d_hap, hap, (size_t)lk->n_ctg * sizeof(int32_t), cudaMemcpyHostToDevice, ctx->stream));
        HH_CUDA(cudaMemsetAsync(d_n, 0, sizeof(unsigned long long), ctx->stream));
        HH_LAUNCH(ctx, hh_k_phased_mark, links_grid(ctx, nnz), 256, 0, lk->d_compact, nnz, d_hap, w, d_order, d_n);
        unsigned long long n_kept = 0;
        HH_CUDA(cudaMemcpyAsync(&n_kept, d_n, sizeof(n_kept), cudaMemcpyDeviceToHost, ctx->stream));
        HH_CUDA(cudaStreamSynchronize(ctx->stream));
        const int64_t n = (int64_t)n_kept;
        *n_out = n;
        if (n == 0) return HH_OK;
        HH_CHECK(hh_dmalloc(&d_kept, (size_t)n * HH_E_WORDS));
        HH_CHECK(links_compact(lk, d_order, nnz, nullptr, reinterpret_cast<const hh_slot*>(lk->d_compact), d_kept));
        HH_CHECK(hh_dmalloc(&d_soa, (size_t)n * 17));
        int32_t* ki = reinterpret_cast<int32_t*>(d_soa);
        double* val = reinterpret_cast<double*>(d_soa + (size_t)n * 8);
        uint8_t* flt = d_soa + (size_t)n * 16;
        HH_LAUNCH(ctx, hh_k_phased_split, links_grid(ctx, n), 256, 0, d_kept, n, d_hap, w, ki, ki + n, val, flt, lk->d_ul_key,
                  lk->d_ul_slot, lk->n_ul);
        HH_CUDA(cudaMemcpyAsync(key_i, ki, (size_t)n * 4, cudaMemcpyDeviceToHost, ctx->stream));
        HH_CUDA(cudaMemcpyAsync(key_j, ki + n, (size_t)n * 4, cudaMemcpyDeviceToHost, ctx->stream));
        HH_CUDA(cudaMemcpyAsync(values, val, (size_t)n * 8, cudaMemcpyDeviceToHost, ctx->stream));
        HH_CUDA(cudaMemcpyAsync(is_float, flt, (size_t)n, cudaMemcpyDeviceToHost, ctx->stream));
        HH_CUDA(cudaStreamSynchronize(ctx->stream));
        return HH_OK;
    }();
    hh_dfree(d_hap);
    hh_dfree(d_order);
    hh_dfree(d_kept);
    hh_dfree(d_soa);
    hh_dfree(d_n);
    return rc;
}

extern "C" int hh_links_set_ul_pairs(hh_links* lk, const int32_t* key_i, const int32_t* key_j, const int32_t* ht_slot, int64_t n_pairs) {
    HH_REQUIRE(lk && n_pairs >= 0 && (n_pairs == 0 || (key_i && key_j && ht_slot)), HH_ERR_ARG, "hh_links_set_ul_pairs: bad argument");
    hh_scope _scope(lk->ctx);
    hh_ctx* ctx = lk->ctx;
    HH_CUDA(cudaSetDevice(ctx->device));
    std::vector<std::pair<unsigned long long, int32_t>> pairs((size_t)n_pairs);
    for (int64_t k = 0; k < n_pairs; ++k) {
        HH_REQUIRE(key_i[k] >= 0 && key_i[k] < lk->n_ctg && key_j[k] >= 0 && key_j[k] < lk->n_ctg && key_i[k] != key_j[k] &&
                       ht_slot[k] >= 0 && ht_slot[k] < 4,
                   HH_ERR_ARG, "hh_links_set_ul_pairs: pair %lld is out of range", (long long)k);
        pairs[(size_t)k] = {((unsigned long long)key_i[k] << 32) | (uint32_t)key_j[k], ht_slot[k]};
    }
    std::sort(pairs.begin(), pairs.end());
    for (size_t k = 1; k < pairs.size(); ++k)
        HH_REQUIRE(pairs[k].first != pairs[k - 1].first, HH_ERR_ARG, "hh_links_set_ul_pairs: a contig pair is listed twice");
    hh_dfree(lk->d_ul_key);
    hh_dfree(lk->d_ul_slot);
    lk->d_ul_key = nullptr;
    lk->d_ul_slot = nullptr;
    lk->n_ul = 0;
    if (n_pairs == 0) return HH_OK;
    std::vector<unsigned long long> keys((size_t)n_pairs);
    std::vector<int32_t> slots((size_t)n_pairs);
    for (size_t k = 0; k < pairs.size(); ++k) {
        keys[k] = pairs[k].first;
        slots[k] = pairs[k].second;
    }
    HH_CHECK(hh_dmalloc(&lk->d_ul_key, (size_t)n_pairs));
    HH_CHECK(hh_dmalloc(&lk->d_ul_slot, (size_t)n_pairs));
    HH_CUDA(cudaMemcpyAsync(lk->d_ul_key, keys.data(), keys.size() * sizeof(unsigned long long), cudaMemcpyHostToDevice, ctx->stream));
    HH_CUDA(cudaMemcpyAsync(lk->d_ul_slot, slots.data(), slots.size() * sizeof(int32_t), cudaMemcpyHostToDevice, ctx->stream));
    HH_CUDA(cudaStreamSynchronize(ctx->stream));
    lk->n_ul = n_pairs;
    return HH_OK;
}

extern "C" int hh_links_fetch_ctg(hh_links* lk, int64_t* ctg_links) {
    HH_REQUIRE(lk && ctg_links, HH_ERR_ARG, "hh_links_fetch_ctg: NULL argument");
    HH_CUDA(cudaSetDevice(lk->ctx->device));
    HH_CUDA(cudaMemcpyAsync(ctg_links, lk->d_ctg, (size_t)lk->n_ctg * sizeof(int64_t), cudaMemcpyDeviceToHost, lk->ctx->stream));
    HH_CUDA(cudaStreamSynchronize(lk->ctx->stream));
    return HH_OK;
}

extern "C" int hh_links_export(hh_links* lk, uint32_t* entries_dev, int64_t* ctg_links_dev) {
    HH_REQUIRE(lk != nullptr, HH_ERR_ARG, "hh_links_export: NULL handle");
    HH_REQUIRE(lk->finished, HH_ERR_STATE, "hh_links_export: call hh_links_finish first");
    HH_CUDA(cudaSetDevice(lk->ctx->device));
    if (entries_dev && lk->nnz)
        HH_CUDA(cudaMemcpyAsync(entries_dev, lk->d_compact, (size_t)lk->nnz * HH_E_WORDS * sizeof(uint32_t), cudaMemcpyDeviceToDevice,
                                lk->ctx->stream));
    if (ctg_links_dev)
        HH_CUDA(cudaMemcpyAsync(ctg_links_dev, lk->d_ctg, (size_t)lk->n_ctg * sizeof(int64_t), cudaMemcpyDeviceToDevice,
                                lk->ctx->stream));
    HH_CUDA(cudaStreamSynchronize(lk->ctx->stream));
    return HH_OK;
}

extern "C" int hh_links_merge(hh_links* lk, const uint32_t* entries_dev, int64_t n_entries, const int64_t* ctg_links_dev,
                              int64_t n_records, int64_t n_used) {
    HH_REQUIRE(lk != nullptr, HH_ERR_ARG, "hh_links_merge: NULL handle");
    hh_scope _scope(lk->ctx);
    HH_REQUIRE(lk->mode != 2 && !(lk->finished && lk->d_keys == nullptr), HH_ERR_STATE,
               "hh_links_merge: this table holds an entry list (hh_links_adopt / partitioned counting), not a hash table");
    lk->mode = 1;
    HH_CHECK(links_need_table(lk));
    lk->finished = false;
    lk->gen++;
    HH_REQUIRE(n_entries >= 0 && (entries_dev || n_entries == 0), HH_ERR_ARG, "hh_links_merge: bad entries");
    hh_ctx* ctx = lk->ctx;
    HH_CUDA(cudaSetDevice(ctx->device));
    if (n_entries) {
        HH_CHECK(links_ensure_capacity(lk, n_entries));
        const int grid = links_grid(ctx, n_entries);
        HH_LAUNCH(ctx, hh_k_links_merge, grid, 256, 0, entries_dev, n_entries, lk->d_keys, lk->d_vals, lk->cap, lk->d_counters);
        lk->since_known += n_entries;
    }
    if (ctg_links_dev)
        HH_LAUNCH(ctx, hh_k_add_u64, (lk->n_ctg + 255) / 256, 256, 0, lk->d_ctg, ctg_links_dev, lk->n_ctg);
    HH_CUDA(cudaStreamSynchronize(ctx->stream));
    lk->n_records += n_records;
    lk->peer_used += n_used;
    return HH_OK;
}

extern "C" int hh_links_linked_index(hh_links* lk, const uint8_t* keep, int32_t* index, int32_t* n_linked) {
    return hh_links_linked_index_phased(lk, keep, 0, nullptr, 0.0, index, n_linked);
}

static bool links_index_current(const hh_links* lk, const uint8_t* keep, int normalize, const int32_t* hap, double w) {
    if (!lk->ix_valid || lk->ix_gen != lk->gen || lk->ix_normalize != normalize) return false;
    if ((hap != nullptr) != !lk->ix_hap.empty()) return false;
    if (hap && (lk->ix_w != w || memcmp(hap, lk->ix_hap.data(), (size_t)lk->n_ctg * sizeof(int32_t)) != 0)) return false;
    return memcmp(keep, lk->ix_keep.data(), (size_t)lk->n_ctg) == 0;
}

extern "C" int hh_links_linked_index_phased(hh_links* lk, const uint8_t* keep, int normalize_by_nlinks, const int32_t* hap,
                                            double w, int32_t* index, int32_t* n_linked) {
    HH_REQUIRE(lk && keep, HH_ERR_ARG, "hh_links_linked_index: NULL argument");
    hh_scope _scope(lk->ctx);
    HH_REQUIRE(lk->finished, HH_ERR_STATE, "hh_links_linked_index: call hh_links_finish first");
    HH_REQUIRE(!hap || (w >= 0.0 && w <= 1.0), HH_ERR_ARG, "hh_links_linked_index_phased: phasing weight %g outside [0, 1]", w);
    hh_ctx* ctx = lk->ctx;
    HH_CUDA(cudaSetDevice(ctx->device));
    const int n_ctg = lk->n_ctg;
    if (!links_index_current(lk, keep, normalize_by_nlinks, hap, w)) {
        lk->ix_valid = false;
        lk->phased = hap != nullptr;
        if (hap) {
            if (!lk->d_hap) HH_CHECK(hh_dmalloc(&lk->d_hap, (size_t)n_ctg));
            HH_CUDA(cudaMemcpyAsync(lk->d_hap, hap, (size_t)n_ctg * sizeof(int32_t), cudaMemcpyHostToDevice, ctx->stream));
        }
        unsigned long long *d_touch = nullptr, *d_touch_sorted = nullptr;
        int32_t *d_frag = nullptr, *d_frag_sorted = nullptr;
        uint8_t* d_tmp = nullptr;
        int rc = [&]() -> int {
            HH_CHECK(hh_dmalloc(&d_touch, (size_t)n_ctg * 2));
            HH_CHECK(hh_dmalloc(&d_frag, (size_t)n_ctg * 2));
            d_touch_sorted = d_touch + n_ctg;
            d_frag_sorted = d_frag + n_ctg;
            size_t tmp_bytes = 0;
            HH_CUDA(cub::DeviceRadixSort::SortPairs(nullptr, tmp_bytes, d_touch, d_touch_sorted, d_frag, d_frag_sorted, n_ctg, 0, 34,
                                                    ctx->stream));
            HH_CHECK(hh_dmalloc(&d_tmp, tmp_bytes));
            HH_CUDA(cudaMemcpyAsync(lk->d_keep, keep, (size_t)n_ctg, cudaMemcpyHostToDevice, ctx->stream));
            HH_CUDA(cudaMemsetAsync(d_touch, 0xFF, (size_t)n_ctg * sizeof(unsigned long long), ctx->stream));
            HH_CUDA(cudaMemsetAsync(lk->d_deg, 0, (size_t)n_ctg * sizeof(int32_t), ctx->stream));
            unsigned long long* d_out = reinterpret_cast<unsigned long long*>(ctx->d_scratch + 8);
            HH_CUDA(cudaMemsetAsync(d_out, 0, 2 * sizeof(unsigned long long), ctx->stream));
            if (lk->nnz) {
                int grid = 0;
                HH_CHECK(hh_resident_grid(ctx, hh_k_touch, 256, 0, &grid));
                grid = std::min(grid, links_grid(ctx, lk->nnz));
                HH_LAUNCH(ctx, hh_k_touch, grid, 256, 0, lk->d_compact, lk->nnz, lk->d_keep, lk->d_ctg, normalize_by_nlinks,
                          hh_links_hap_dev(lk), w, d_touch, lk->d_deg, d_out + 1);
            }
            HH_LAUNCH(ctx, hh_k_iota_i32, (n_ctg + 255) / 256, 256, 0, d_frag, n_ctg);
            HH_CUDA(cub::DeviceRadixSort::SortPairs(d_tmp, tmp_bytes, d_touch, d_touch_sorted, d_frag, d_frag_sorted, n_ctg, 0, 34,
                                                    ctx->stream));
            HH_LAUNCH(ctx, hh_k_rank_sorted, (n_ctg + 255) / 256, 256, 0, d_touch_sorted, d_frag_sorted, n_ctg, lk->d_index, d_out);
            HH_CUDA(cudaMemcpyAsync(ctx->h_scratch + 8, d_out, 2 * sizeof(unsigned long long), cudaMemcpyDeviceToHost, ctx->stream));
            HH_CUDA(cudaStreamSynchronize(ctx->stream));
            lk->n_linked = (int32_t)ctx->h_scratch[8];
            lk->n_pass = (int64_t)ctx->h_scratch[9];
            return HH_OK;
        }();
        hh_dfree(d_touch);
        hh_dfree(d_frag);
        hh_dfree(d_tmp);
        HH_CHECK(rc);
        lk->ix_keep.assign(keep, keep + n_ctg);
        if (hap) lk->ix_hap.assign(hap, hap + n_ctg);
        else lk->ix_hap.clear();
        lk->ix_w = w;
        lk->ix_normalize = normalize_by_nlinks;
        lk->ix_gen = lk->gen;
        lk->ix_valid = true;
    }
    if (index) {
        HH_CUDA(cudaMemcpyAsync(index, lk->d_index, (size_t)n_ctg * sizeof(int32_t), cudaMemcpyDeviceToHost, ctx->stream));
        HH_CUDA(cudaStreamSynchronize(ctx->stream));
    }
    if (n_linked) *n_linked = lk->n_linked;
    return HH_OK;
}

extern "C" int hh_links_destroy(hh_links* lk) {
    if (!lk) return HH_OK;
    hh_scope _scope(lk->ctx);
    cudaSetDevice(lk->ctx->device);
    cudaStreamSynchronize(lk->ctx->stream);
    if (lk->copy_stream) {
        cudaStreamSynchronize(lk->copy_stream);
        cudaStreamDestroy(lk->copy_stream);
    }
    for (int k = 0; k < 2; ++k) {
        if (lk->ev_copied[k]) cudaEventDestroy(lk->ev_copied[k]);
        if (lk->ev_consumed[k]) cudaEventDestroy(lk->ev_consumed[k]);
        if (lk->d_stage[k]) cudaFree(lk->d_stage[k]);
    }
    hh_dfree(lk->d_src_rank);
    hh_dfree(lk->d_fbase);
    hh_dfree(lk->d_len);
    hh_dfree(lk->d_rank);
    hh_dfree(lk->d_nx);
    hh_dfree(lk->d_ctg);
    hh_dfree(lk->d_keys);
    hh_dfree(lk->d_vals);
    hh_dfree(lk->d_counters);
    hh_dfree(lk->d_compact);
    hh_dfree(lk->d_index);
    hh_dfree(lk->d_keep);
    hh_dfree(lk->d_hap);
    hh_dfree(lk->d_deg);
    hh_dfree(lk->d_ul_key);
    hh_dfree(lk->d_ul_slot);
    links_free_partsets(lk);
    delete lk;
    return HH_OK;
}

int32_t hh_links_n_ctg(hh_links* lk) { return lk->n_ctg; }
hh_ctx* hh_links_ctx(hh_links* lk) { return lk->ctx; }
const uint32_t* hh_links_compact(hh_links* lk, int64_t* nnz) { *nnz = lk->nnz; return lk->d_compact; }
const unsigned long long* hh_links_ctg_totals(hh_links* lk) { return lk->d_ctg; }
const int32_t* hh_links_index_dev(hh_links* lk, int32_t* n_linked) { *n_linked = lk->n_linked; return lk->d_index; }
const int32_t* hh_links_degree_dev(hh_links* lk, int64_t* n_pass) { *n_pass = lk->n_pass; return lk->d_deg; }
uint8_t* hh_links_keep_dev(hh_links* lk) { return lk->d_keep; }
bool hh_links_finished(hh_links* lk) { return lk->finished; }
const int32_t* hh_links_hap_dev(hh_links* lk) { return lk->phased ? lk->d_hap : nullptr; }
```

### haphic_b200/links.py

```python

from __future__ import annotations

import ctypes as C
from collections import defaultdict

import numpy as np

from . import _lib
from ._lib import Context, LinksInfo, check, load, ptr

NONE32 = 0xFFFFFFFF

_PINNED = {}


def _host_buffer(tag, shape, dtype):
    n = int(np.prod(shape))
    if n * np.dtype(dtype).itemsize < (1 << 20):
        return np.empty(shape, dtype)
    try:
        import torch
        key = (tag, np.dtype(dtype).str)
        buf = _PINNED.get(key)
        nbytes = n * np.dtype(dtype).itemsize
        if buf is None or buf.numel() < nbytes:
            buf = torch.empty(int(nbytes * 1.25), dtype=torch.uint8, pin_memory=True)
            _PINNED[key] = buf
        return buf[:nbytes].numpy().view(dtype).reshape(shape)
    except Exception:
        return np.empty(shape, dtype)


def name_rank(names) -> np.ndarray:
    order = sorted(range(len(names)), key=names.__getitem__)
    rank = np.empty(len(names), dtype=np.int32)
    rank[order] = np.arange(len(names), dtype=np.int32)
    return rank


class LinkTable:
    _close_order = 0

    def __init__(self, ctx: Context, ctg_len, rank, in_nx, flank_bp: int, capacity_hint: int = 0, frags=None):
        self.ctx = ctx
        self.n_ctg = len(ctg_len)
        self._len = np.ascontiguousarray(ctg_len, dtype=np.int64)
        self._rank = np.ascontiguousarray(rank, dtype=np.int32)
        self._nx = np.ascontiguousarray(in_nx, dtype=np.uint8)
        if not (len(self._rank) == self.n_ctg == len(self._nx)):
            raise ValueError("ctg_len, rank and in_nx must have one entry per contig")
        self._h = C.c_void_p()
        if frags is None:
            check(load().hh_links_create(ctx.handle, self.n_ctg, ptr(self._len), ptr(self._rank), ptr(self._nx),
                                         int(flank_bp), int(capacity_hint), C.byref(self._h)))
        else:
            self._src_rank = np.ascontiguousarray(frags["ctg_rank"], dtype=np.int32)
            self._fbase = np.ascontiguousarray(frags["frag_base"], dtype=np.int32)
            check(load().hh_links_create_frags(ctx.handle, len(self._src_rank), ptr(self._src_rank), ptr(self._fbase),
                                               self.n_ctg, ptr(self._len), ptr(self._rank), ptr(self._nx),
                                               int(frags["bin_size"]), int(flank_bp), int(capacity_hint), C.byref(self._h)))
        ctx.adopt(self)
        self._stream_pos = 0
        self.info = None

    def add(self, rec, stream_offset: int | None = None, asynchronous: bool = False):
        n_rec = int(rec.shape[0])
        if n_rec == 0:
            return
        off = self._stream_pos if stream_offset is None else int(stream_offset)
        if isinstance(rec, np.ndarray):
            if rec.dtype != np.int32 or rec.ndim != 2 or rec.shape[1] != 4 or not rec.flags.c_contiguous:
                rec = np.ascontiguousarray(rec, dtype=np.int32).reshape(-1, 4)
            mem = _lib.HH_MEM_HOST
        else:
            import torch
            if rec.dtype != torch.int32 or rec.dim() != 2 or rec.shape[1] != 4 or not rec.is_contiguous():
                raise ValueError("records must be a contiguous int32 [P, 4] tensor")
            mem = _lib.HH_MEM_DEVICE if rec.is_cuda else _lib.HH_MEM_HOST
            if rec.is_cuda:
                torch.cuda.current_stream(rec.device).synchronize()
        if asynchronous:
            if mem != _lib.HH_MEM_DEVICE:
                raise ValueError("asynchronous add needs device-resident records")
            check(load().hh_links_add_async(self._h, ptr(rec), n_rec, off))
        else:
            check(load().hh_links_add(self._h, ptr(rec), n_rec, off, mem))
        self._stream_pos = max(self._stream_pos, off + n_rec)

    def finish(self) -> LinksInfo:
        info = LinksInfo()
        check(load().hh_links_finish(self._h, C.byref(info)))
        self.info = info
        return info

    def agg_info(self) -> dict:
        b, s, f = C.c_int64(), C.c_int64(), C.c_int64()
        check(load().hh_links_agg_info(self._h, C.byref(b), C.byref(s), C.byref(f)))
        return {"buckets": int(b.value), "smem_buckets": int(s.value), "fallback_buckets": int(f.value)}

    def fetch(self, pinned: bool = False) -> dict:
        if self.info is None:
            self.finish()
        nnz = int(self.info.nnz_full)
        hb = _host_buffer if pinned else (lambda _tag, shape, dtype: np.empty(shape, dtype))
        out = {
            "key_i": hb("key_i", (nnz,), np.int32), "key_j": hb("key_j", (nnz,), np.int32),
            "full": hb("full", (nnz,), np.uint32), "flank": hb("flank", (nnz,), np.uint32),
            "first_full": hb("first_full", (nnz,), np.uint32), "first_flank": hb("first_flank", (nnz,), np.uint32),
            "ht": hb("ht", (nnz, 4), np.uint32),
        }
        check(load().hh_links_fetch(self._h, ptr(out["key_i"]), ptr(out["key_j"]), ptr(out["full"]), ptr(out["flank"]),
                                    ptr(out["first_full"]), ptr(out["first_flank"]), ptr(out["ht"])))
        return out

    def fetch_phased(self, hap, phasing_weight: float) -> dict:
        if self.info is None:
            self.finish()
        hap = self._hap(hap)
        nnz = int(self.info.nnz_full)
        out = {"key_i": np.empty(nnz, np.int32), "key_j": np.empty(nnz, np.int32), "values": np.empty(nnz, np.float64),
               "is_float": np.empty(nnz, np.uint8)}
        n = C.c_int64()
        check(load().hh_links_fetch_phased(self._h, ptr(hap), float(phasing_weight), ptr(out["key_i"]), ptr(out["key_j"]),
                                           ptr(out["values"]), ptr(out["is_float"]), C.byref(n)))
        return {k: v[:int(n.value)] for k, v in out.items()}

    def fetch_ctg(self) -> np.ndarray:
        tot = np.empty(self.n_ctg, np.int64)
        check(load().hh_links_fetch_ctg(self._h, ptr(tot)))
        return tot

    def _hap(self, hap):
        if hap is None:
            return None
        hap = np.ascontiguousarray(hap, dtype=np.int32)
        if hap.shape != (self.n_ctg,):
            raise ValueError("hap must have one entry per fragment of the table")
        return hap

    def linked_index(self, keep, hap=None, phasing_weight: float = 0.0, normalize_by_nlinks: bool = False):
        if self.info is None:
            self.finish()
        keep = np.ascontiguousarray(keep, dtype=np.uint8)
        hap = self._hap(hap)
        index = np.empty(self.n_ctg, np.int32)
        n_linked = C.c_int32()
        check(load().hh_links_linked_index_phased(self._h, ptr(keep), int(bool(normalize_by_nlinks)),
                                                  ptr(hap) if hap is not None else None, float(phasing_weight), ptr(index),
                                                  C.byref(n_linked)))
        return index, int(n_linked.value)

    def to_matrix(self, keep, tail=None, normalize_by_nlinks: bool = False, add_self_loops: bool = True, hap=None,
                  phasing_weight: float = 0.0, ul=None) -> "LinkMatrix":
        if self.info is None:
            self.finish()
        keep = np.ascontiguousarray(keep, dtype=np.uint8)
        tail = np.ascontiguousarray(tail if tail is not None else [], dtype=np.int32)
        hap = self._hap(hap)
        ul_path = ul_parent = None
        if ul is not None:
            ul_path, ul_parent = (np.ascontiguousarray(a, dtype=np.int32) for a in ul)
            if ul_path.shape != (self.n_ctg,) or ul_parent.shape != (self.n_ctg,):
                raise ValueError("ul_path and ul_parent must have one entry per fragment of the table")
        h = C.c_void_p()
        check(load().hh_matrix_from_links_ex(self._h, ptr(keep), ptr(tail) if len(tail) else None, len(tail),
                                             int(bool(normalize_by_nlinks)), int(bool(add_self_loops)),
                                             ptr(hap) if hap is not None else None, float(phasing_weight),
                                             ptr(ul_path) if ul is not None else None, ptr(ul_parent) if ul is not None else None,
                                             C.byref(h)))
        return LinkMatrix(self.ctx, h)

    def set_ul_pairs(self, key_i, key_j, ht_slot):
        ki, kj, hs = (np.ascontiguousarray(a, dtype=np.int32) for a in (key_i, key_j, ht_slot))
        n = len(ki)
        if not (len(kj) == len(hs) == n):
            raise ValueError("key_i, key_j and ht_slot must have the same length")
        check(load().hh_links_set_ul_pairs(self._h, ptr(ki) if n else None, ptr(kj) if n else None, ptr(hs) if n else None, n))

    def export(self):
        import torch
        if self.info is None:
            self.finish()
        dev = torch.device("cuda", self.ctx.device)
        ent = torch.empty((int(self.info.nnz_full), 9), dtype=torch.int32, device=dev)
        tot = torch.empty(self.n_ctg, dtype=torch.int64, device=dev)
        check(load().hh_links_export(self._h, ptr(ent), ptr(tot)))
        return ent, tot, int(self.info.n_records), int(self.info.n_used)

    def merge(self, entries, ctg_totals, n_records: int, n_used: int):
        n = int(entries.shape[0])
        check(load().hh_links_merge(self._h, ptr(entries) if n else None, n, ptr(ctg_totals), int(n_records), int(n_used)))
        self.info = None

    def route(self, rec, stream_offset: int, world: int):
        import torch
        if not rec.is_cuda or rec.dtype != torch.int32 or rec.dim() != 2 or rec.shape[1] != 4 or not rec.is_contiguous():
            raise ValueError("records must be a contiguous int32 [P, 4] CUDA tensor")
        n_rec = int(rec.shape[0])
        rec_out = torch.empty((max(n_rec, 1), 4), dtype=torch.int32, device=rec.device)
        pos_out = torch.empty(max(n_rec, 1), dtype=torch.int32, device=rec.device)
        counts = np.zeros(world, np.int64)
        check(load().hh_links_route(self._h, ptr(rec) if n_rec else None, n_rec, int(stream_offset), int(world),
                                    ptr(rec_out), ptr(pos_out), ptr(counts)))
        m = int(counts.sum())
        self._stream_pos = max(self._stream_pos, int(stream_offset) + n_rec)
        return rec_out[:m], pos_out[:m], [int(c) for c in counts]

    def add_routed(self, rec, pos):
        n_rec = int(rec.shape[0])
        if n_rec:
            check(load().hh_links_add_routed(self._h, ptr(rec), ptr(pos), n_rec))

    def finish_partition(self) -> LinksInfo:
        info = LinksInfo()
        check(load().hh_links_finish_partition(self._h, C.byref(info)))
        self.info = info
        return info

    def adopt(self, entries, ctg_totals, n_records: int, n_used: int, stream_end: int):
        n = int(entries.shape[0])
        check(load().hh_links_adopt(self._h, ptr(entries) if n else None, n, ptr(ctg_totals), int(n_records), int(n_used),
                                    int(stream_end)))
        self.info = None
        return self.finish()

    def close(self):
        if self._h:
            load().hh_links_destroy(self._h)
            self._h = C.c_void_p()

    def __del__(self):
        try:
            self.close()
        except Exception:
            pass


class LinkMatrix:

    _close_order = 1

    def __init__(self, ctx: Context, handle):
        self.ctx = ctx
        self._h = handle
        ctx.adopt(self)
        n = C.c_int32()
        nnz = C.c_int64()
        check(load().hh_matrix_info(self._h, C.byref(n), C.byref(nnz)))
        self.n, self.nnz = int(n.value), int(nnz.value)

    @classmethod
    def from_csc(cls, ctx: Context, matrix) -> "LinkMatrix":
        import scipy.sparse as sp
        m = sp.csc_matrix(matrix, dtype=np.float32)
        if m.shape[0] != m.shape[1]:
            raise ValueError("link matrix must be square")
        indptr = np.ascontiguousarray(m.indptr, dtype=np.int64)
        indices = np.ascontiguousarray(m.indices, dtype=np.int32)
        data = np.ascontiguousarray(m.data, dtype=np.float32)
        h = C.c_void_p()
        check(load().hh_matrix_from_csc(ctx.handle, m.shape[0], ptr(indptr), ptr(indices), ptr(data), C.byref(h)))
        return cls(ctx, h)

    def rank_sums(self, topN: int = 10) -> np.ndarray:
        out = np.empty(self.n, np.int64)
        check(load().hh_matrix_rank_sums(self._h, int(topN), ptr(out)))
        return out

    def to_scipy(self):
        import scipy.sparse as sp
        indptr = np.empty(self.n + 1, np.int64)
        check(load().hh_matrix_fetch_csc(self._h, ptr(indptr), None, None))
        nnz = int(indptr[-1])
        indices = np.empty(nnz, np.int32)
        data = np.empty(nnz, np.float32)
        check(load().hh_matrix_fetch_csc(self._h, ptr(indptr), ptr(indices), ptr(data)))
        return sp.csc_matrix((data, indices, indptr), shape=(self.n, self.n))

    def close(self):
        if self._h:
            load().hh_matrix_destroy(self._h)
            self._h = C.c_void_p()

    def __del__(self):
        try:
            self.close()
        except Exception:
            pass


class GroupLinkStats:

    _close_order = 1

    def __init__(self, ctx: Context, n_ctg: int, key_i, key_j, values, is_float=None):
        self.ctx = ctx
        self.n_ctg = int(n_ctg)
        ki = np.ascontiguousarray(key_i, dtype=np.int32)
        kj = np.ascontiguousarray(key_j, dtype=np.int32)
        v = np.ascontiguousarray(values, dtype=np.float64)
        m = len(ki)
        f = np.zeros(m, np.uint8) if is_float is None else np.ascontiguousarray(is_float, dtype=np.uint8)
        self._h = C.c_void_p()
        check(load().hh_stats_create(ctx.handle, self.n_ctg, ptr(ki) if m else None, ptr(kj) if m else None, ptr(v) if m else None,
                                     ptr(f) if m else None, m, C.byref(self._h)))
        ctx.adopt(self)
        self.n_ranked = 0

    def rank(self, group, n_groups: int) -> int:
        g = np.ascontiguousarray(group, dtype=np.int32)
        if g.shape != (self.n_ctg,):
            raise ValueError("group must have one entry per contig")
        n = C.c_int64()
        check(load().hh_stats_rank(self._h, ptr(g), int(n_groups), C.byref(n)))
        self.n_ranked = int(n.value)
        return self.n_ranked

    def fetch_ranked(self):
        n = self.n_ranked
        c, g = np.empty(n, np.int32), np.empty(n, np.int32)
        s, f = np.empty(n, np.float64), np.empty(n, np.uint8)
        check(load().hh_stats_fetch_ranked(self._h, ptr(c), ptr(g), ptr(s), ptr(f)))
        return c, g, s, f.astype(bool)

    def best(self, group_re, ctg_re, compensated: bool) -> dict:
        gre = np.ascontiguousarray(group_re, dtype=np.int64)
        cre = np.ascontiguousarray(ctg_re, dtype=np.int64)
        if cre.shape != (self.n_ctg,):
            raise ValueError("ctg_re must have one entry per contig")
        n = self.n_ctg
        out = {"has": np.empty(n, np.uint8), "top_links": np.empty(n, np.float64), "top_is_float": np.empty(n, np.uint8),
               "top_density": np.empty(n, np.float64), "others": np.empty(n, np.float64), "ratio": np.empty(n, np.float64)}
        check(load().hh_stats_best(self._h, ptr(gre), len(gre), ptr(cre), int(bool(compensated)), ptr(out["has"]),
                                   ptr(out["top_links"]), ptr(out["top_is_float"]), ptr(out["top_density"]), ptr(out["others"]),
                                   ptr(out["ratio"])))
        return out

    def close(self):
        if self._h:
            load().hh_stats_destroy(self._h)
            self._h = C.c_void_p()

    def __del__(self):
        try:
            self.close()
        except Exception:
            pass



def link_dicts(table: LinkTable, names):
    f = table.fetch()
    ki, kj = f["key_i"].tolist(), f["key_j"].tolist()
    full_link_dict = defaultdict(int)
    for a, b, v in zip(ki, kj, f["full"].tolist()):
        full_link_dict[(names[a], names[b])] = v
    sel = np.nonzero(f["flank"] > 0)[0]
    sel = sel[np.argsort(f["first_flank"][sel], kind="stable")]
    flank_link_dict = defaultdict(int)
    for e in sel.tolist():
        flank_link_dict[(names[ki[e]], names[kj[e]])] = int(f["flank"][e])
    HT_link_dict = defaultdict(int)
    suffix = ("_H", "_T")
    ht = f["ht"]
    for e, (a, b) in enumerate(zip(ki, kj)):
        for c in range(4):
            v = int(ht[e, c])
            if v:
                HT_link_dict[(names[a] + suffix[c >> 1], names[b] + suffix[c & 1])] = v
    tot = table.fetch_ctg()
    ctg_link_dict = defaultdict(int)
    touch = {}
    for e in sel.tolist():
        t = int(f["first_flank"][e]) * 2
        a, b = ki[e], kj[e]
        if t < touch.get(a, 1 << 62):
            touch[a] = t
        if t + 1 < touch.get(b, 1 << 62):
            touch[b] = t + 1
    for c in sorted(touch, key=touch.__getitem__):
        ctg_link_dict[names[c]] = int(tot[c])
    return full_link_dict, flank_link_dict, HT_link_dict, ctg_link_dict
```

### include/haphic_b200.h

```cpp
#ifndef HAPHIC_B200_H
#define HAPHIC_B200_H

#include <stdint.h>

#ifdef __cplusplus
extern "C" {
#endif

#define HH_VERSION 100

enum {
    HH_OK = 0,
    HH_ERR_CUDA = 1,
    HH_ERR_ARG = 2,
    HH_ERR_CAPACITY = 3,
    HH_ERR_NOMEM = 4,
    HH_ERR_STATE = 5,
    HH_ERR_UNSUPPORTED = 6
};

enum { HH_MEM_HOST = 0, HH_MEM_DEVICE = 1 };

typedef struct hh_ctx hh_ctx;
typedef struct hh_links hh_links;
typedef struct hh_matrix hh_matrix;
typedef struct hh_mcl hh_mcl;

int hh_version(void);
const char* hh_last_error(void);

int hh_ctx_create(int device, hh_ctx** out);
int hh_ctx_destroy(hh_ctx* ctx);
int hh_ctx_sync(hh_ctx* ctx);
void* hh_ctx_stream(hh_ctx* ctx);
int hh_ctx_device(hh_ctx* ctx);
int hh_ctx_sm_count(hh_ctx* ctx);
int64_t hh_ctx_launches(hh_ctx* ctx);

int hh_links_create(hh_ctx* ctx, int32_t n_ctg, const int64_t* ctg_len, const int32_t* name_rank,
                    const uint8_t* in_nx, int64_t flank_bp, int64_t capacity_hint, hh_links** out);
int hh_links_create_frags(hh_ctx* ctx, int32_t n_ctg, const int32_t* ctg_rank, const int32_t* frag_base,
                          int32_t n_frag, const int64_t* frag_len, const int32_t* frag_rank,
                          const uint8_t* frag_in_nx, int64_t bin_size, int64_t flank_bp, int64_t capacity_hint,
                          hh_links** out);
int hh_links_add(hh_links* lk, const int32_t* rec, int64_t n_rec, int64_t stream_offset, int mem);
int hh_links_add_async(hh_links* lk, const int32_t* rec_dev, int64_t n_rec, int64_t stream_offset);

typedef struct {
    int64_t n_records;
    int64_t n_used;
    int64_t nnz_full;
    int64_t nnz_flank;
    int64_t table_slots;
} hh_links_info;

int hh_links_finish(hh_links* lk, hh_links_info* info);
int hh_links_agg_info(hh_links* lk, int64_t* buckets, int64_t* smem_buckets, int64_t* fallback_buckets);

int hh_links_fetch(hh_links* lk, int32_t* key_i, int32_t* key_j, uint32_t* full, uint32_t* flank,
                   uint32_t* first_full, uint32_t* first_flank, uint32_t* ht);
int hh_links_fetch_phased(hh_links* lk, const int32_t* hap, double w, int32_t* key_i, int32_t* key_j, double* values,
                          uint8_t* is_float, int64_t* n_out);
int hh_links_set_ul_pairs(hh_links* lk, const int32_t* key_i, const int32_t* key_j, const int32_t* ht_slot, int64_t n_pairs);
int hh_links_fetch_ctg(hh_links* lk, int64_t* ctg_links);
int hh_links_export(hh_links* lk, uint32_t* entries_dev, int64_t* ctg_links_dev);
int hh_links_merge(hh_links* lk, const uint32_t* entries_dev, int64_t n_entries, const int64_t* ctg_links_dev,
                   int64_t n_records, int64_t n_used);
int hh_links_route(hh_links* lk, const int32_t* rec_dev, int64_t n_rec, int64_t stream_offset, int world,
                   int32_t* rec_out_dev, uint32_t* pos_out_dev, int64_t* counts);
int hh_links_add_routed(hh_links* lk, const int32_t* rec_dev, const uint32_t* pos_dev, int64_t n_rec);
int hh_links_finish_partition(hh_links* lk, hh_links_info* info);
int hh_links_adopt(hh_links* lk, const uint32_t* entries_dev, int64_t n_entries, const int64_t* ctg_links_dev,
                   int64_t n_records, int64_t n_used, int64_t stream_end);
int hh_links_destroy(hh_links* lk);

int hh_links_linked_index(hh_links* lk, const uint8_t* keep, int32_t* index, int32_t* n_linked);
int hh_matrix_from_links(hh_links* lk, const uint8_t* keep, const int32_t* tail, int32_t n_tail,
                         int normalize_by_nlinks, int add_self_loops, hh_matrix** out);
int hh_links_linked_index_phased(hh_links* lk, const uint8_t* keep, int normalize_by_nlinks, const int32_t* hap, double w,
                                 int32_t* index, int32_t* n_linked);
int hh_matrix_from_links_phased(hh_links* lk, const uint8_t* keep, const int32_t* tail, int32_t n_tail,
                                int normalize_by_nlinks, int add_self_loops, const int32_t* hap, double w, hh_matrix** out);
int hh_matrix_from_links_ex(hh_links* lk, const uint8_t* keep, const int32_t* tail, int32_t n_tail, int normalize_by_nlinks,
                            int add_self_loops, const int32_t* hap, double w, const int32_t* ul_path, const int32_t* ul_parent,
                            hh_matrix** out);
int hh_matrix_rank_sums(hh_matrix* m, int topN, int64_t* rank_sum);
int hh_matrix_from_csc(hh_ctx* ctx, int32_t n, const int64_t* indptr, const int32_t* indices,
                       const float* data, hh_matrix** out);
int hh_matrix_info(hh_matrix* m, int32_t* n, int64_t* nnz);
int hh_matrix_fetch_csc(hh_matrix* m, int64_t* indptr, int32_t* indices, float* data);
int hh_matrix_destroy(hh_matrix* m);

typedef struct hh_stats hh_stats;
int hh_stats_create(hh_ctx* ctx, int32_t n_ctg, const int32_t* key_i, const int32_t* key_j, const double* values,
                    const uint8_t* is_float, int64_t n_entries, hh_stats** out);
int hh_stats_rank(hh_stats* st, const int32_t* group, int32_t n_groups, int64_t* n_ranked);
int hh_stats_fetch_ranked(hh_stats* st, int32_t* ctg, int32_t* group, double* links, uint8_t* is_float);
int hh_stats_best(hh_stats* st, const int64_t* group_re, int32_t n_groups, const int64_t* ctg_re, int compensated, uint8_t* has,
                  double* top_links, uint8_t* top_is_float, double* top_density, double* others, double* ratio);
int hh_stats_destroy(hh_stats* st);

int hh_mcl_create(hh_matrix* m, int expansion, int32_t col_lo, int32_t col_hi, hh_mcl** out);
enum { HH_PREEXP_AUTO = 0, HH_PREEXP_SPARSE = 1, HH_PREEXP_DENSE = 2 };
int hh_mcl_create_ex(hh_matrix* m, int expansion, int32_t col_lo, int32_t col_hi, int preexp_mode, hh_mcl** out);
int hh_mcl_choose_preexp(hh_matrix* m, int expansion, int requested, int* mode);
int hh_mcl_footprint(hh_matrix* m, int expansion, int32_t ncols, int mode, double pruning, size_t* m1_bytes, size_t* fixed_bytes);
int hh_ctx_mem_available(hh_ctx* ctx, size_t* bytes);
typedef struct {
    int32_t mode;
    int32_t a_planes;
    int32_t passes;
    int32_t cta_group;
    int32_t stages;
    int32_t chunk_kb;
    float total_ms;
    float densify_ms;
    float gemm_ms;
    float clip_ms;
    double flops;
    int64_t products;
    float clip;
    int32_t b_planes;
    int32_t fmt_a, fmt_b;
    int32_t k_chunks;
} hh_preexp_info;
int hh_mcl_preexp_info(hh_mcl* mc, hh_preexp_info* info);
int hh_mcl_info(hh_mcl* mc, int32_t* n, int64_t* nnz_m0, int64_t* preexp_products, float* normalize_ms,
                float* preexp_ms);
int hh_mcl_fetch_m0(hh_mcl* mc, int64_t* indptr, int32_t* indices, float* data);
int hh_mcl_fetch_m1(hh_mcl* mc, float* dense);
int hh_mcl_fetch_m1_cols(hh_mcl* mc, int32_t col_lo, int32_t col_hi, float* dense);

typedef struct {
    int32_t rounds;
    int32_t converged;
    int64_t nnz;
    int64_t products;
    int64_t bytes;
} hh_mcl_result;

int hh_mcl_run(hh_mcl* mc, double inflation, int max_iter, double pruning, hh_mcl_result* res,
               int64_t* iter_nnz, int64_t* iter_products, float* iter_delta, float* iter_ms);
int hh_mcl_fetch_result(hh_mcl* mc, int64_t* indptr, int32_t* indices, float* data);

int hh_mcl_begin(hh_mcl* mc, double inflation, double pruning);
int hh_mcl_step(hh_mcl* mc, int it, int64_t* nnz_owned, int64_t* products, float* delta, float* kernel_ms);
int hh_mcl_pack(hh_mcl* mc, int32_t* len_dev, int32_t* idx_dev, float* val_dev);
int hh_mcl_unpack(hh_mcl* mc, int32_t col_lo, int32_t col_hi, const int32_t* len_dev,
                  const int32_t* idx_dev, const float* val_dev, int64_t nnz_block);
int hh_mcl_commit(hh_mcl* mc);
typedef struct {
    int32_t it;
    int32_t iter0;
    int32_t iter0_w;
    int32_t blk;
    int32_t blk_f16;
    int32_t blk_chunk;
    int64_t blk_ldk;
    int32_t n_win;
    int32_t n_big;
    int32_t wmax;
    int32_t small;
    int32_t small_cols;
    int32_t small_overflow;
    int32_t col;
    int32_t col_cols;
    int32_t col_w;
    int32_t col_smem;
    int32_t col_track;
    int32_t col_flat;
} hh_mcl_step_info_t;
int hh_mcl_step_info(hh_mcl* mc, hh_mcl_step_info_t* info);
int hh_mcl_set_block(hh_mcl* mc, int32_t col_lo, int32_t col_hi);
int hh_mcl_destroy(hh_mcl* mc);

typedef struct hh_correct hh_correct;
typedef struct {
    int32_t n_examined;
    int32_t n_broken;
    int32_t n_breaks;
    int32_t n_frag;
    int64_t n_links;
} hh_correct_round_info;
int hh_correct_create(hh_ctx* ctx, int32_t n_ctg, const int64_t* ctg_len, int64_t resolution, hh_correct** out);
int hh_correct_add(hh_correct* cr, const int32_t* rec, int64_t n_rec, int mem);
int hh_correct_round(hh_correct* cr, double median_cov_ratio, double region_len_ratio, int64_t min_region_cutoff,
                     int last_round, hh_correct_round_info* info);
int hh_correct_fetch_breaks(hh_correct* cr, int32_t* frag, int32_t* bin, int32_t* cov);
int hh_correct_info(hh_correct* cr, int32_t* n_active, int64_t* active_bins, int64_t* n_links);
int hh_correct_fetch_cov(hh_correct* cr, int32_t* frag, int32_t* nbins, int32_t* cov);
int hh_correct_set_layout(hh_correct* cr, const int32_t* src_base, const int64_t* piece_start, const int32_t* piece_id,
                          int32_t n_pieces);
int hh_correct_remap(hh_correct* cr, const int32_t* rec_in, int32_t* rec_out, int64_t n_rec, int mem);
int hh_correct_destroy(hh_correct* cr);

typedef struct hh_contact hh_contact;
int hh_contact_create(hh_ctx* ctx, int32_t n_ctg, const uint8_t* in_set, const int64_t* slot_base, const int64_t* cand_off,
                      const int64_t* cand_lo, const int64_t* cand_hi, const int32_t* cand_bin, int32_t nb, int64_t bin_size,
                      hh_contact** out);
int hh_contact_load(hh_ctx* ctx, int32_t nb, const int64_t* counts, hh_contact** out);
int hh_contact_add(hh_contact* h, const int32_t* rec, int64_t n_rec, int mem);
int hh_contact_add_async(hh_contact* h, const int32_t* rec_dev, int64_t n_rec);
int hh_contact_error(hh_contact* h, int64_t* index, int32_t* end, int32_t* ctg, int64_t* pos);
int hh_contact_finish(hh_contact* h);
int hh_contact_info(hh_contact* h, int32_t* nb, int32_t* count_bytes, int64_t* n_records);
int hh_contact_fetch(hh_contact* h, int64_t* out);
int hh_contact_kr(hh_contact* h, int32_t n_prob, const int32_t* off, const int32_t* n, double tol, double delta, double Delta,
                  int32_t max_outer, int32_t max_inner, double* x_out, int32_t* n_outer, int64_t* n_inner, int32_t* status);
int hh_contact_normalize(hh_contact* h, int mode, int32_t n_blk, const int32_t* blk_off, const int32_t* blk_n,
                         const double* x_blocks, const double* x_whole, double* out, double* median_lo, double* median_hi,
                         int64_t* n_values);
int hh_contact_destroy(hh_contact* h);

typedef struct hh_pairs_reader hh_pairs_reader;
int hh_pairs_open(const char* path, const char* names_blob, int32_t n_names, const char* bed_path, int inter_only,
                  int threads, hh_pairs_reader** out);
int hh_pairs_next(hh_pairs_reader* r, int32_t* rec, int64_t max_records, int64_t* n_out);
int hh_pairs_close(hh_pairs_reader* r);
int hh_pairs_write(const char* path, const char* names_blob, int32_t n_names, const int32_t* rec, int64_t n_rec, int64_t first_index,
                   int append, int threads);
typedef struct hh_bam_reader hh_bam_reader;
int hh_bam_open(const char* path, const char* names_blob, int32_t n_names, int inter_only, int threads, hh_bam_reader** out);
int hh_bam_header_text(hh_bam_reader* r, const char** text, int64_t* len);
int hh_bam_next(hh_bam_reader* r, int32_t* rec, int64_t max_records, int64_t* n_out);
int hh_bam_close(hh_bam_reader* r);
typedef struct hh_ul_reader hh_ul_reader;
int hh_ul_open(const char* path, int threads, int32_t min_mapq, int64_t min_alignment_length, int64_t max_distance_to_end,
               double max_overlap_ratio, int64_t max_gap_len, hh_ul_reader** out);
int hh_ul_info(hh_ul_reader* r, int32_t* n_ref, int64_t* names_bytes, int64_t* n_events, int64_t* n_records);
int hh_ul_fetch(hh_ul_reader* r, char* names, int64_t* ref_len, int32_t* events);
int hh_ul_close(hh_ul_reader* r);

int hh_clm_from_records(const char* path, const char* names_blob, int32_t n_names, const int32_t* rec, int64_t n_rec,
                        const int64_t* ctg_len, const int32_t* name_rank, int threads);
int hh_pickle_links(const char* path, const char* names_blob, int32_t n_names, const int32_t* key_i, const int32_t* key_j,
                    int64_t n_entries, const int64_t* values_i64, const double* values_f64, const uint32_t* ht);
int hh_pickle_links_mixed(const char* path, const char* names_blob, int32_t n_names, const int32_t* key_i, const int32_t* key_j,
                          int64_t n_entries, const double* values, const uint8_t* is_float);

#ifdef __cplusplus
}
#endif
#endif
```

Baseline: 6.173 billion.

## Pack partition and bucket records into 8-byte narrow format when keys fit

```diff
diff --git a/haphic_b200/_lib.py b/haphic_b200/_lib.py
--- a/haphic_b200/_lib.py
+++ b/haphic_b200/_lib.py
@@ -68,6 +68,7 @@
     "hh_links_add_async": (C.c_int, [_P, _P, C.c_int64, C.c_int64]),
     "hh_links_finish": (C.c_int, [_P, C.POINTER(LinksInfo)]),
     "hh_links_agg_info": (C.c_int, [_P, C.POINTER(C.c_int64), C.POINTER(C.c_int64), C.POINTER(C.c_int64)]),
+    "hh_links_record_bytes": (C.c_int, [_P, C.POINTER(C.c_int32), C.c_int32, C.POINTER(C.c_int32), C.POINTER(C.c_int32)]),
     "hh_links_fetch": (C.c_int, [_P, _P, _P, _P, _P, _P, _P, _P]),
     "hh_links_fetch_phased": (C.c_int, [_P, _P, C.c_double, _P, _P, _P, _P, C.POINTER(C.c_int64)]),
     "hh_links_set_ul_pairs": (C.c_int, [_P, _P, _P, _P, C.c_int64]),
diff --git a/haphic_b200/csrc/hh_common.cuh b/haphic_b200/csrc/hh_common.cuh
--- a/haphic_b200/csrc/hh_common.cuh
+++ b/haphic_b200/csrc/hh_common.cuh
@@ -158,6 +158,11 @@
                  : "l"(p));
     return r;
 }
+__device__ __forceinline__ unsigned long long hh_ld_stream_u64(const unsigned long long* p) {
+    unsigned long long r;
+    asm volatile("ld.global.nc.L1::no_allocate.u64 %0, [%1];" : "=l"(r) : "l"(p));
+    return r;
+}
 __device__ __forceinline__ float4 hh_ld_stream_f4(const float4* p) {
     float4 r;
     asm volatile("ld.global.nc.L1::no_allocate.v4.f32 {%0, %1, %2, %3}, [%4];"
diff --git a/haphic_b200/csrc/hh_links.cu b/haphic_b200/csrc/hh_links.cu
--- a/haphic_b200/csrc/hh_links.cu
+++ b/haphic_b200/csrc/hh_links.cu
@@ -13,7 +13,8 @@
 };
 
 struct hh_partset {
-    int4* buf;
+    void* buf;
+    bool narrow;
     unsigned long long* cursor;
     uint64_t pcap;
     int64_t sized_for, sent;
@@ -48,6 +49,9 @@
     int64_t stage_records;
     int mode;
     int npart_log;
+    int kbits;
+    std::vector<int32_t> set_bytes;
+    int32_t bucket_bytes;
     uint64_t scap;
     int64_t agg_buckets, agg_smem, agg_fallback;
     uint64_t spill_cap;
@@ -326,6 +330,42 @@
 #define HH_PART_TILE 4096
 #define HH_PART_MAX 1024
 
+#define HH_NREC_KBITS 16
+#define HH_NREC_ZBITS 29
+#define HH_NREC_ZEND (1ll << HH_NREC_ZBITS)
+
+struct __align__(8) hh_nrec {
+    unsigned long long v;
+};
+
+__device__ __forceinline__ int4 hh_ld_rec(const int4* p) { return hh_ld_stream(p); }
+__device__ __forceinline__ hh_nrec hh_ld_rec(const hh_nrec* p) { return hh_nrec{hh_ld_stream_u64(&p->v)}; }
+
+__device__ __forceinline__ uint32_t hh_rec_i(int4 r, int) { return (uint32_t)r.x; }
+__device__ __forceinline__ uint32_t hh_rec_j(int4 r, int) { return (uint32_t)r.y; }
+__device__ __forceinline__ uint32_t hh_rec_z(int4 r) { return (uint32_t)r.z; }
+__device__ __forceinline__ unsigned hh_rec_flags(int4 r) { return (unsigned)r.w & 7u; }
+__device__ __forceinline__ uint32_t hh_rec_i(hh_nrec r, int kbits) { return (uint32_t)(r.v >> 32) >> kbits; }
+__device__ __forceinline__ uint32_t hh_rec_j(hh_nrec r, int kbits) { return (uint32_t)(r.v >> 32) & ((1u << kbits) - 1u); }
+__device__ __forceinline__ uint32_t hh_rec_z(hh_nrec r) { return (uint32_t)r.v & (uint32_t)(HH_NREC_ZEND - 1); }
+__device__ __forceinline__ unsigned hh_rec_flags(hh_nrec r) { return (uint32_t)r.v >> HH_NREC_ZBITS; }
+
+__device__ __forceinline__ hh_nrec hh_nrec_make(uint32_t i, uint32_t j, uint32_t z, unsigned flags, int kbits) {
+    return hh_nrec{((unsigned long long)((i << kbits) | j) << 32) | ((unsigned long long)flags << HH_NREC_ZBITS) | z};
+}
+
+__device__ __forceinline__ void hh_rec_put(int4* d, int4 s, int) { *d = s; }
+__device__ __forceinline__ void hh_rec_put(hh_nrec* d, hh_nrec s, int) { *d = s; }
+__device__ __forceinline__ void hh_rec_put(int4* d, hh_nrec s, int kbits) {
+    *d = make_int4((int)hh_rec_i(s, kbits), (int)hh_rec_j(s, kbits), (int)hh_rec_z(s), (int)hh_rec_flags(s));
+}
+__device__ __forceinline__ void hh_rec_put(hh_nrec* d, int4 s, int kbits) {
+    *d = hh_nrec_make(hh_rec_i(s, kbits), hh_rec_j(s, kbits), hh_rec_z(s), hh_rec_flags(s), kbits);
+}
+
+__device__ __forceinline__ void hh_rec_set_z(int4* r, uint32_t z) { r->z = (int)z; }
+__device__ __forceinline__ void hh_rec_set_z(hh_nrec* r, uint32_t z) { r->v = (r->v & ~(unsigned long long)(HH_NREC_ZEND - 1)) | z; }
+
 #define HH_STAGE_SMEM ((size_t)HH_PART_TILE * sizeof(int4))
 
 __device__ __forceinline__ unsigned int hh_tile_scan(unsigned int* c, int n, unsigned int* s_wtot) {
@@ -361,35 +401,54 @@
     return all;
 }
 
+template <typename R>
+__device__ __forceinline__ uint32_t hh_bucket_of(R r, int bucket_log, int kbits) {
+    return (uint32_t)(hh_mix64(hh_pair_key((int)hh_rec_i(r, kbits), (int)hh_rec_j(r, kbits))) >> (64 - bucket_log));
+}
+
+__device__ __forceinline__ void hh_part_rec(int4* o, const hh_pair& pr, uint32_t z, unsigned p, int) {
+    *o = make_int4(pr.a, pr.b, (int)z, (int)(pr.flags | (p << 8)));
+}
+__device__ __forceinline__ void hh_part_rec(hh_nrec* o, const hh_pair& pr, uint32_t z, unsigned, int kbits) {
+    *o = hh_nrec_make((uint32_t)pr.a, (uint32_t)pr.b, z, pr.flags, kbits);
+}
+__device__ __forceinline__ unsigned hh_part_of(int4 r, int, int) { return (unsigned)r.w >> 8; }
+__device__ __forceinline__ unsigned hh_part_of(hh_nrec r, int npart_log, int kbits) { return hh_bucket_of(r, npart_log, kbits); }
+
+template <typename R>
+__host__ __device__ constexpr int hh_scatter_tile() { return (int)(HH_STAGE_SMEM / sizeof(R)); }
+
+template <typename R>
 __global__ void __launch_bounds__(512, 2)
 hh_k_part_scatter(const int4* __restrict__ rec, int64_t n_rec, uint32_t stream_off, int32_t n_ctg, const int32_t* __restrict__ ctg_len,
-                  const int32_t* __restrict__ name_rank, const uint8_t* __restrict__ in_nx, int64_t flank_bp, int npart_log,
-                  int4* __restrict__ pbuf, uint64_t pcap, unsigned long long* __restrict__ cursor, int4* __restrict__ spill,
+                  const int32_t* __restrict__ name_rank, const uint8_t* __restrict__ in_nx, int64_t flank_bp, int npart_log, int kbits,
+                  R* __restrict__ pbuf, uint64_t pcap, unsigned long long* __restrict__ cursor, int4* __restrict__ spill,
                   uint64_t spill_cap, unsigned long long* __restrict__ spill_cursor, unsigned long long* __restrict__ counters) {
-    extern __shared__ int4 s_stage[];
+    constexpr int TILE = hh_scatter_tile<R>(), ITEMS = TILE / 512;
+    extern __shared__ int4 s_stage_mem[];
+    R* s_stage = reinterpret_cast<R*>(s_stage_mem);
     __shared__ unsigned int s_cnt[HH_PART_MAX];
     __shared__ unsigned long long s_base[HH_PART_MAX];
     __shared__ unsigned int s_wtot[16];
     __shared__ unsigned int s_used;
     const int npart = 1 << npart_log;
-    const int64_t tiles = (n_rec + HH_PART_TILE - 1) / HH_PART_TILE;
+    const int64_t tiles = (n_rec + TILE - 1) / TILE;
     unsigned int my_used = 0;
     if (threadIdx.x == 0) s_used = 0;
     for (int64_t t = blockIdx.x; t < tiles; t += gridDim.x) {
         for (int k = threadIdx.x; k < npart; k += 512) s_cnt[k] = 0;
         __syncthreads();
-        int4 out[8];
-        unsigned int rnk[8];
+        R out[ITEMS];
+        uint32_t live = 0;
 #pragma unroll
-        for (int k = 0; k < 8; ++k) {
-            const int64_t i = t * HH_PART_TILE + (int64_t)k * 512 + threadIdx.x;
-            rnk[k] = HH_NONE32;
+        for (int k = 0; k < ITEMS; ++k) {
+            const int64_t i = t * TILE + (int64_t)k * 512 + threadIdx.x;
             if (i < n_rec) {
                 hh_pair pr;
                 if (hh_classify_contig(hh_ld_stream(rec + i), n_ctg, ctg_len, name_rank, in_nx, flank_bp, &pr)) {
-                    const int p = (int)(hh_mix64(hh_pair_key(pr.a, pr.b)) >> (64 - npart_log));
-                    rnk[k] = atomicAdd(&s_cnt[p], 1u);
-                    out[k] = make_int4(pr.a, pr.b, (int)(stream_off + (uint32_t)i), (int)(pr.flags | ((unsigned)p << 8)));
+                    const unsigned p = (unsigned)(hh_mix64(hh_pair_key(pr.a, pr.b)) >> (64 - npart_log));
+                    hh_part_rec(&out[k], pr, (p << 13) | atomicAdd(&s_cnt[p], 1u), p, kbits);
+                    live |= 1u << k;
                     my_used++;
                 }
             }
@@ -399,18 +458,22 @@
             if (s_cnt[k]) s_base[k] = atomicAdd(cursor + k, (unsigned long long)s_cnt[k]);
         const unsigned int n_tile = hh_tile_scan(s_cnt, npart, s_wtot);
 #pragma unroll
-        for (int k = 0; k < 8; ++k)
-            if (rnk[k] != HH_NONE32) s_stage[s_cnt[(unsigned)out[k].w >> 8] + rnk[k]] = out[k];
+        for (int k = 0; k < ITEMS; ++k) {
+            if (!((live >> k) & 1u)) continue;
+            const uint32_t at = hh_rec_z(out[k]);
+            hh_rec_set_z(&out[k], stream_off + (uint32_t)(t * TILE + k * 512 + threadIdx.x));
+            s_stage[s_cnt[at >> 13] + (at & 0x1FFFu)] = out[k];
+        }
         __syncthreads();
         for (unsigned int e = threadIdx.x; e < n_tile; e += 512) {
-            const int4 r = s_stage[e];
-            const unsigned int p = (unsigned)r.w >> 8;
+            const R r = s_stage[e];
+            const unsigned int p = hh_part_of(r, npart_log, kbits);
             const unsigned long long q = s_base[p] + (e - s_cnt[p]);
             if (q < pcap) {
                 pbuf[(size_t)p * (size_t)pcap + (size_t)q] = r;
             } else {
                 const unsigned long long sq = atomicAdd(spill_cursor, 1ull);
-                if (sq < spill_cap) spill[sq] = r;
+                if (sq < spill_cap) hh_rec_put(spill + sq, r, kbits);
                 else atomicExch(counters + 2, 3ull);
             }
         }
@@ -429,13 +492,11 @@
 #define HH_AGG_THREADS 256
 #define HH_AGG_HOT 32
 
-__device__ __forceinline__ uint32_t hh_bucket_of(int4 r, int bucket_log) {
-    return (uint32_t)(hh_mix64(hh_pair_key(r.x, r.y)) >> (64 - bucket_log));
-}
-
+template <typename R>
 __global__ void __launch_bounds__(512)
-hh_k_part_hist(const int4* __restrict__ pbuf, uint64_t pcap, const unsigned long long* __restrict__ cursor, int npart_log, int64_t tpr,
-               const int4* __restrict__ spill, int64_t n_spill, int bucket_log, unsigned int* __restrict__ bcnt) {
+hh_k_part_hist(const R* __restrict__ pbuf, uint64_t pcap, const unsigned long long* __restrict__ cursor, int npart_log, int kbits,
+               int64_t tpr, const int4* __restrict__ spill, int64_t n_spill, int bucket_log, unsigned int* __restrict__ bcnt) {
+    constexpr int TILE = HH_PART_TILE, ITEMS = TILE / 512;
     __shared__ unsigned int s_cnt[1 << HH_SUB_MAX_LOG];
     const int sub_log = bucket_log - npart_log, nsub = 1 << sub_log;
     const int64_t region_tiles = ((int64_t)1 << npart_log) * tpr;
@@ -444,20 +505,20 @@
         if (t >= region_tiles) {
             const int64_t base = (t - region_tiles) * HH_PART_TILE;
             for (int k = threadIdx.x; k < HH_PART_TILE; k += 512)
-                if (base + k < n_spill) atomicAdd(bcnt + hh_bucket_of(hh_ld_stream(spill + base + k), bucket_log), 1u);
+                if (base + k < n_spill) atomicAdd(bcnt + hh_bucket_of(hh_ld_rec(spill + base + k), bucket_log, kbits), 1u);
             continue;
         }
         const int p = (int)(t / tpr);
-        const uint64_t start = (uint64_t)(t % tpr) * HH_PART_TILE;
+        const uint64_t start = (uint64_t)(t % tpr) * TILE;
         const uint64_t fill = min((uint64_t)cursor[p], pcap);
         if (start >= fill) continue;
         for (int k = threadIdx.x; k < nsub; k += 512) s_cnt[k] = 0;
         __syncthreads();
-        const int4* reg = pbuf + (size_t)p * (size_t)pcap;
+        const R* reg = pbuf + (size_t)p * (size_t)pcap;
 #pragma unroll
-        for (int k = 0; k < 8; ++k) {
+        for (int k = 0; k < ITEMS; ++k) {
             const uint64_t i = start + (uint64_t)k * 512 + threadIdx.x;
-            if (i < fill) atomicAdd(&s_cnt[hh_bucket_of(hh_ld_stream(reg + i), bucket_log) & (nsub - 1)], 1u);
+            if (i < fill) atomicAdd(&s_cnt[hh_bucket_of(hh_ld_rec(reg + i), bucket_log, kbits) & (nsub - 1)], 1u);
         }
         __syncthreads();
         for (int k = threadIdx.x; k < nsub; k += 512)
@@ -466,11 +527,14 @@
     }
 }
 
+template <typename R, typename D>
 __global__ void __launch_bounds__(512, 2)
-hh_k_part_scatter2(const int4* __restrict__ pbuf, uint64_t pcap, const unsigned long long* __restrict__ cursor, int npart_log, int64_t tpr,
-                   const int4* __restrict__ spill, int64_t n_spill, int bucket_log, const int64_t* __restrict__ boff,
-                   unsigned int* __restrict__ bfill, int4* __restrict__ out, uint64_t n_out, unsigned long long* __restrict__ counters) {
-    extern __shared__ int4 s_stage[];
+hh_k_part_scatter2(const R* __restrict__ pbuf, uint64_t pcap, const unsigned long long* __restrict__ cursor, int npart_log, int kbits,
+                   int64_t tpr, const int4* __restrict__ spill, int64_t n_spill, int bucket_log, const int64_t* __restrict__ boff,
+                   unsigned int* __restrict__ bfill, D* __restrict__ out, uint64_t n_out, unsigned long long* __restrict__ counters) {
+    constexpr int TILE = HH_PART_TILE, ITEMS = TILE / 512;
+    extern __shared__ int4 s_stage_mem[];
+    R* s_stage = reinterpret_cast<R*>(s_stage_mem);
     __shared__ unsigned int s_cnt[1 << HH_SUB_MAX_LOG];
     __shared__ unsigned int s_base[1 << HH_SUB_MAX_LOG];
     __shared__ unsigned int s_wtot[16];
@@ -482,30 +546,30 @@
             const int64_t base = (t - region_tiles) * HH_PART_TILE;
             for (int k = threadIdx.x; k < HH_PART_TILE; k += 512) {
                 if (base + k >= n_spill) break;
-                const int4 r = hh_ld_stream(spill + base + k);
-                const uint32_t b = hh_bucket_of(r, bucket_log);
+                const int4 r = hh_ld_rec(spill + base + k);
+                const uint32_t b = hh_bucket_of(r, bucket_log, kbits);
                 const uint64_t q = (uint64_t)boff[b] + atomicAdd(bfill + b, 1u);
-                if (q < n_out) out[q] = r;
+                if (q < n_out) hh_rec_put(out + q, r, kbits);
                 else atomicExch(counters + 2, 6ull);
             }
             continue;
         }
         const int p = (int)(t / tpr);
-        const uint64_t start = (uint64_t)(t % tpr) * HH_PART_TILE;
+        const uint64_t start = (uint64_t)(t % tpr) * TILE;
         const uint64_t fill = min((uint64_t)cursor[p], pcap);
         if (start >= fill) continue;
         for (int k = threadIdx.x; k < nsub; k += 512) s_cnt[k] = 0;
         __syncthreads();
-        const int4* reg = pbuf + (size_t)p * (size_t)pcap;
-        int4 r[8];
-        uint32_t at[8];
+        const R* reg = pbuf + (size_t)p * (size_t)pcap;
+        R r[ITEMS];
+        uint32_t at[ITEMS];
 #pragma unroll
-        for (int k = 0; k < 8; ++k) {
+        for (int k = 0; k < ITEMS; ++k) {
             const uint64_t i = start + (uint64_t)k * 512 + threadIdx.x;
             at[k] = HH_NONE32;
             if (i < fill) {
-                r[k] = hh_ld_stream(reg + i);
-                const uint32_t sub = hh_bucket_of(r[k], bucket_log) & (nsub - 1);
+                r[k] = hh_ld_rec(reg + i);
+                const uint32_t sub = hh_bucket_of(r[k], bucket_log, kbits) & (nsub - 1);
                 at[k] = (sub << 16) | atomicAdd(&s_cnt[sub], 1u);
             }
         }
@@ -514,15 +578,15 @@
             if (s_cnt[k]) s_base[k] = atomicAdd(bfill + ((size_t)p << sub_log) + k, s_cnt[k]);
         const unsigned int n_tile = hh_tile_scan(s_cnt, nsub, s_wtot);
 #pragma unroll
-        for (int k = 0; k < 8; ++k)
+        for (int k = 0; k < ITEMS; ++k)
             if (at[k] != HH_NONE32) s_stage[s_cnt[at[k] >> 16] + (at[k] & 0xFFFFu)] = r[k];
         __syncthreads();
         for (unsigned int e = threadIdx.x; e < n_tile; e += 512) {
-            const int4 rec = s_stage[e];
-            const uint32_t sub = hh_bucket_of(rec, bucket_log) & (nsub - 1);
+            const R rec = s_stage[e];
+            const uint32_t sub = hh_bucket_of(rec, bucket_log, kbits) & (nsub - 1);
             const size_t b = ((size_t)p << sub_log) + sub;
             const uint64_t q = (uint64_t)boff[b] + s_base[sub] + (e - s_cnt[sub]);
-            if (q < n_out) out[q] = rec;
+            if (q < n_out) hh_rec_put(out + q, rec, kbits);
             else atomicExch(counters + 2, 6ull);
         }
         __syncthreads();
@@ -580,9 +644,9 @@
     int bucket;
 };
 
-template <typename K, int ITEMS>
+template <typename K, int ITEMS, typename R>
 __global__ void __launch_bounds__(HH_AGG_THREADS, 3)
-hh_k_bucket_count(const int4* __restrict__ rec, const int64_t* __restrict__ boff, int nbuckets, uint64_t hot, int kbits,
+hh_k_bucket_count(const R* __restrict__ rec, const int64_t* __restrict__ boff, int nbuckets, uint64_t hot, int kbits,
                   uint32_t* __restrict__ compact, uint64_t compact_cap, unsigned long long* __restrict__ ctg_links,
                   unsigned long long* __restrict__ counters, unsigned long long* __restrict__ agg, uint32_t* __restrict__ fallback) {
     typedef hh_bc_smem<K, ITEMS> smem_t;
@@ -620,10 +684,10 @@
                 key[q] = ~(K)0;
                 pay[q] = 0;
                 if (l < m) {
-                    const int4 r = hh_ld_stream(rec + lo + c0 + l);
-                    key[q] = ((K)(uint32_t)r.x << kbits) | (K)(uint32_t)r.y;
-                    pay[q] = (uint32_t)l | (((uint32_t)r.w & 7u) << 11);
-                    sm.z[l] = (uint32_t)r.z;
+                    const R r = hh_ld_rec(rec + lo + c0 + l);
+                    key[q] = ((K)hh_rec_i(r, kbits) << kbits) | (K)hh_rec_j(r, kbits);
+                    pay[q] = (uint32_t)l | (hh_rec_flags(r) << 11);
+                    sm.z[l] = hh_rec_z(r);
                 }
             }
             typename smem_t::sort_t(sm.u.sort).Sort(key, pay, 0, 2 * kbits);
@@ -758,8 +822,9 @@
 
 #define HH_FB_BATCH (1 << 19)
 
-__global__ void hh_k_gather_buckets(const int4* __restrict__ src, const int64_t* __restrict__ src_off, const int64_t* __restrict__ pre,
-                                    int nf, int4* __restrict__ dst) {
+template <typename R>
+__global__ void hh_k_gather_buckets(const R* __restrict__ src, const int64_t* __restrict__ src_off, const int64_t* __restrict__ pre,
+                                    int nf, int kbits, int4* __restrict__ dst) {
     const int64_t total = pre[nf];
     const int64_t stride = (int64_t)gridDim.x * blockDim.x;
     for (int64_t i = (int64_t)blockIdx.x * blockDim.x + threadIdx.x; i < total; i += stride) {
@@ -769,7 +834,7 @@
             if (pre[mid] <= i) lo = mid;
             else hi = mid - 1;
         }
-        dst[i] = hh_ld_stream(src + src_off[lo] + (i - pre[lo]));
+        hh_rec_put(dst + i, hh_ld_rec(src + src_off[lo] + (i - pre[lo])), kbits);
     }
 }
 
@@ -1189,6 +1254,8 @@
     lk->n_src = frag_base ? n_src : n_key;
     lk->bin_size = bin_size;
     lk->flank_bp = flank_bp;
+    lk->kbits = 1;
+    while ((1ll << lk->kbits) < (int64_t)n_key) lk->kbits++;
     int rc = HH_OK;
     do {
         if ((rc = hh_dmalloc(&lk->d_len, n_key)) != HH_OK) break;
@@ -1260,13 +1327,21 @@
     return (v && *v) ? atoi(v) : dflt;
 }
 
-static int links_new_partset(hh_links* lk, int64_t n_rec) {
+static bool links_narrow(const hh_links* lk, int64_t stream_end) {
+    return lk->kbits <= HH_NREC_KBITS && stream_end <= HH_NREC_ZEND;
+}
+
+static int links_new_partset(hh_links* lk, int64_t n_rec, int64_t stream_end) {
     const int npart = 1 << lk->npart_log;
     hh_partset ps;
     memset(&ps, 0, sizeof(ps));
     ps.pcap = (uint64_t)((double)n_rec / npart * 1.5) + 4096;
     ps.sized_for = n_rec;
-    HH_CHECK(hh_ws_alloc(lk->ctx, &ps.buf, (size_t)npart * (size_t)ps.pcap));
+    ps.narrow = links_narrow(lk, stream_end);
+    const size_t bytes = ps.narrow ? sizeof(hh_nrec) : sizeof(int4);
+    unsigned char* buf = nullptr;
+    HH_CHECK(hh_ws_alloc(lk->ctx, &buf, (size_t)npart * (size_t)ps.pcap * bytes));
+    ps.buf = buf;
     int rc = hh_dmalloc(&ps.cursor, (size_t)npart);
     if (rc != HH_OK) {
         hh_ws_free(lk->ctx, ps.buf);
@@ -1274,6 +1349,7 @@
     }
     HH_CUDA(cudaMemsetAsync(ps.cursor, 0, (size_t)npart * sizeof(unsigned long long), lk->ctx->stream));
     lk->psets.push_back(ps);
+    lk->set_bytes.push_back((int32_t)bytes);
     return HH_OK;
 }
 
@@ -1296,7 +1372,7 @@
     return HH_OK;
 }
 
-static int links_choose_mode(hh_links* lk, int64_t total) {
+static int links_choose_mode(hh_links* lk, int64_t total, int64_t stream_offset) {
     if (lk->mode) return HH_OK;
     const int want = links_env_int("HH_LINKS_PARTITION", -1);
     const bool can = lk->d_fbase == nullptr && lk->d_keys == nullptr;
@@ -1311,10 +1387,26 @@
     lk->npart_log = links_env_int("HH_LINKS_NPART_LOG", lg);
     if (lk->npart_log < 1) lk->npart_log = 1;
     if (lk->npart_log > 10) lk->npart_log = 10;
-    HH_CHECK(links_new_partset(lk, total));
+    HH_CHECK(links_new_partset(lk, total, stream_offset + total));
     HH_CHECK(links_size_spill(lk));
     HH_CHECK(hh_dmalloc(&lk->d_spill_cursor, 1));
     HH_CUDA(cudaMemsetAsync(lk->d_spill_cursor, 0, sizeof(unsigned long long), lk->ctx->stream));
+    return HH_OK;
+}
+
+template <typename R>
+static int links_launch_scatter(hh_links* lk, R* pbuf, const int4* d_rec, int64_t n_rec, int64_t stream_offset) {
+    hh_ctx* ctx = lk->ctx;
+    auto kernel = hh_k_part_scatter<R>;
+    const int64_t tiles = (n_rec + hh_scatter_tile<R>() - 1) / hh_scatter_tile<R>();
+    int grid = 0;
+    HH_CUDA(cudaFuncSetAttribute(kernel, cudaFuncAttributeMaxDynamicSharedMemorySize, (int)HH_STAGE_SMEM));
+    HH_CHECK(hh_resident_grid(ctx, kernel, 512, HH_STAGE_SMEM, &grid));
+    grid = (int)std::max<int64_t>(1, std::min<int64_t>(tiles, grid));
+    const hh_partset& ps = lk->psets.back();
+    HH_LAUNCH(ctx, kernel, grid, 512, HH_STAGE_SMEM, d_rec, n_rec, (uint32_t)stream_offset, lk->n_ctg, lk->d_len, lk->d_rank, lk->d_nx,
+              lk->flank_bp, lk->npart_log, lk->kbits, pbuf, ps.pcap, ps.cursor, lk->d_spill, lk->spill_cap, lk->d_spill_cursor,
+              lk->d_counters);
     return HH_OK;
 }
 
@@ -1322,16 +1414,9 @@
                                const uint32_t* d_pos = nullptr) {
     hh_ctx* ctx = lk->ctx;
     if (lk->mode == 2 && d_pos == nullptr) {
-        const int64_t tiles = (n_rec + HH_PART_TILE - 1) / HH_PART_TILE;
-        int grid = 0;
-        HH_CUDA(cudaFuncSetAttribute(hh_k_part_scatter, cudaFuncAttributeMaxDynamicSharedMemorySize, (int)HH_STAGE_SMEM));
-        HH_CHECK(hh_resident_grid(ctx, hh_k_part_scatter, 512, HH_STAGE_SMEM, &grid));
-        grid = (int)std::max<int64_t>(1, std::min<int64_t>(tiles, grid));
         const hh_partset& ps = lk->psets.back();
-        HH_LAUNCH(ctx, hh_k_part_scatter, grid, 512, HH_STAGE_SMEM, d_rec, n_rec, (uint32_t)stream_offset, lk->n_ctg, lk->d_len, lk->d_rank, lk->d_nx,
-                  lk->flank_bp, lk->npart_log, ps.buf, ps.pcap, ps.cursor, lk->d_spill, lk->spill_cap, lk->d_spill_cursor,
-                  lk->d_counters);
-        return HH_OK;
+        return ps.narrow ? links_launch_scatter(lk, reinterpret_cast<hh_nrec*>(ps.buf), d_rec, n_rec, stream_offset)
+                         : links_launch_scatter(lk, reinterpret_cast<int4*>(ps.buf), d_rec, n_rec, stream_offset);
     }
     HH_CHECK(links_need_table(lk));
     HH_LAUNCH(ctx, hh_k_links_insert, links_grid(ctx, n_rec), 256, 0, d_rec, n_rec, (uint32_t)stream_offset, lk->n_ctg, lk->d_len,
@@ -1340,10 +1425,11 @@
     return HH_OK;
 }
 
-static int links_part_room(hh_links* lk, int64_t n_rec) {
+static int links_part_room(hh_links* lk, int64_t n_rec, int64_t stream_offset) {
     hh_partset& ps = lk->psets.back();
-    if (ps.sent > 0 && ps.sent + n_rec > ps.sized_for + ps.sized_for / 8) {
-        HH_CHECK(links_new_partset(lk, n_rec));
+    const bool outgrown = ps.sent + n_rec > ps.sized_for + ps.sized_for / 8;
+    if (ps.sent > 0 && (outgrown || (ps.narrow && !links_narrow(lk, stream_offset + n_rec)))) {
+        HH_CHECK(links_new_partset(lk, n_rec, stream_offset + n_rec));
         lk->psets.back().sent = n_rec;
         return links_size_spill(lk);
     }
@@ -1372,8 +1458,8 @@
     HH_REQUIRE(((uintptr_t)rec_dev & 15) == 0, HH_ERR_ARG, "hh_links_add: records must be 16-byte aligned");
     if (n_rec == 0) return HH_OK;
     HH_CUDA(cudaSetDevice(lk->ctx->device));
-    HH_CHECK(links_choose_mode(lk, n_rec));
-    if (lk->mode == 2) HH_CHECK(links_part_room(lk, n_rec));
+    HH_CHECK(links_choose_mode(lk, n_rec, stream_offset));
+    if (lk->mode == 2) HH_CHECK(links_part_room(lk, n_rec, stream_offset));
     HH_CHECK(links_launch_insert(lk, reinterpret_cast<const int4*>(rec_dev), n_rec, stream_offset));
     lk->n_records += n_rec;
     lk->since_known += n_rec;
@@ -1393,8 +1479,8 @@
     hh_ctx* ctx = lk->ctx;
     HH_CUDA(cudaSetDevice(ctx->device));
     const int64_t CH = HH_ADD_CHUNK;
-    HH_CHECK(links_choose_mode(lk, n_rec));
-    if (lk->mode == 2) HH_CHECK(links_part_room(lk, n_rec));
+    HH_CHECK(links_choose_mode(lk, n_rec, stream_offset));
+    if (lk->mode == 2) HH_CHECK(links_part_room(lk, n_rec, stream_offset));
     if (mem == HH_MEM_DEVICE) {
         HH_REQUIRE(((uintptr_t)rec & 15) == 0, HH_ERR_ARG, "hh_links_add: records must be 16-byte aligned");
         HH_CHECK(links_add_chunks(lk, reinterpret_cast<const int4*>(rec), nullptr, n_rec, stream_offset));
@@ -1444,17 +1530,44 @@
     return (uint64_t)HH_AGG_HOT * (mean > HH_AGG_MEAN / 2 ? mean : HH_AGG_MEAN / 2);
 }
 
-template <typename K, int ITEMS>
-static int links_bucket_count(hh_links* lk, const int4* rec, const int64_t* boff, int nb, uint64_t hot, int kbits, uint32_t* compact,
+template <typename K, int ITEMS, typename R>
+static int links_bucket_count(hh_links* lk, const void* rec, const int64_t* boff, int nb, uint64_t hot, int kbits, uint32_t* compact,
                               uint64_t compact_cap, unsigned long long* agg, uint32_t* fallback) {
     hh_ctx* ctx = lk->ctx;
-    auto kernel = hh_k_bucket_count<K, ITEMS>;
+    auto kernel = hh_k_bucket_count<K, ITEMS, R>;
     const size_t smem = sizeof(hh_bc_smem<K, ITEMS>);
     HH_CUDA(cudaFuncSetAttribute(kernel, cudaFuncAttributeMaxDynamicSharedMemorySize, (int)smem));
     int grid = 0;
     HH_CHECK(hh_resident_grid(ctx, kernel, HH_AGG_THREADS, smem, &grid));
-    HH_LAUNCH(ctx, kernel, grid, HH_AGG_THREADS, smem, rec, boff, nb, hot, kbits, compact, compact_cap, lk->d_ctg, lk->d_counters, agg,
+    HH_LAUNCH(ctx, kernel, grid, HH_AGG_THREADS, smem, reinterpret_cast<const R*>(rec), boff, nb, hot, kbits, compact, compact_cap, lk->d_ctg, lk->d_counters, agg,
               fallback);
+    return HH_OK;
+}
+
+template <typename R>
+static int links_launch_hist(hh_links* lk, const hh_partset& ps, int64_t n_spill, int blog, unsigned int* bcnt) {
+    hh_ctx* ctx = lk->ctx;
+    auto kernel = hh_k_part_hist<R>;
+    int grid = 0;
+    HH_CHECK(hh_resident_grid(ctx, kernel, 512, 0, &grid));
+    const int64_t tpr = (int64_t)((ps.pcap + HH_PART_TILE - 1) / HH_PART_TILE);
+    HH_LAUNCH(ctx, kernel, grid, 512, 0, reinterpret_cast<const R*>(ps.buf), ps.pcap, ps.cursor, lk->npart_log, lk->kbits, tpr,
+              lk->d_spill, n_spill, blog, bcnt);
+    return HH_OK;
+}
+
+template <typename R, typename D>
+static int links_launch_scatter2(hh_links* lk, const hh_partset& ps, int64_t n_spill, int blog, const int64_t* boff, unsigned int* bfill,
+                                 void* out, uint64_t n_out) {
+    hh_ctx* ctx = lk->ctx;
+    auto kernel = hh_k_part_scatter2<R, D>;
+    int grid = 0;
+    const size_t smem = (size_t)HH_PART_TILE * sizeof(R);
+    HH_CUDA(cudaFuncSetAttribute(kernel, cudaFuncAttributeMaxDynamicSharedMemorySize, (int)smem));
+    HH_CHECK(hh_resident_grid(ctx, kernel, 512, smem, &grid));
+    const int64_t tpr = (int64_t)((ps.pcap + HH_PART_TILE - 1) / HH_PART_TILE);
+    HH_LAUNCH(ctx, kernel, grid, 512, smem, reinterpret_cast<const R*>(ps.buf), ps.pcap, ps.cursor, lk->npart_log, lk->kbits, tpr,
+              lk->d_spill, n_spill, blog, boff, bfill, reinterpret_cast<D*>(out), n_out, lk->d_counters);
     return HH_OK;
 }
 
@@ -1481,7 +1594,8 @@
     uint32_t *d_fallback = nullptr, *d_stage_compact = nullptr;
     int64_t* d_boff = nullptr;
     unsigned long long* d_agg = nullptr;
-    int4 *d_rec2 = nullptr, *d_fb_rec = nullptr;
+    unsigned char* d_rec2 = nullptr;
+    int4* d_fb_rec = nullptr;
     int64_t* d_fb_off = nullptr;
     uint64_t* skeys[2] = {nullptr, nullptr};
     hh_slot* svals[2] = {nullptr, nullptr};
@@ -1492,34 +1606,32 @@
         HH_CHECK(hh_dmalloc(&d_boff, (size_t)nb + 1));
         HH_CHECK(hh_dmalloc(&d_fallback, (size_t)nb));
         HH_CHECK(hh_dmalloc(&d_agg, 4));
-        HH_CHECK(hh_ws_alloc(ctx, &d_rec2, (size_t)compact_cap));
+        const bool narrow = links_narrow(lk, lk->stream_end);
+        lk->bucket_bytes = narrow ? (int32_t)sizeof(hh_nrec) : (int32_t)sizeof(int4);
+        HH_CHECK(hh_ws_alloc(ctx, &d_rec2, (size_t)compact_cap * (size_t)lk->bucket_bytes));
         HH_CUDA(cudaMemsetAsync(d_bcnt, 0, (size_t)nb * sizeof(unsigned int), ctx->stream));
         HH_CUDA(cudaMemsetAsync(d_bfill, 0, (size_t)nb * sizeof(unsigned int), ctx->stream));
         HH_CUDA(cudaMemsetAsync(d_agg, 0, 4 * sizeof(unsigned long long), ctx->stream));
-        int grid = 0, grid2 = 0;
-        HH_CHECK(hh_resident_grid(ctx, hh_k_part_hist, 512, 0, &grid));
-        HH_CUDA(cudaFuncSetAttribute(hh_k_part_scatter2, cudaFuncAttributeMaxDynamicSharedMemorySize, (int)HH_STAGE_SMEM));
-        HH_CHECK(hh_resident_grid(ctx, hh_k_part_scatter2, 512, HH_STAGE_SMEM, &grid2));
         for (size_t k = 0; k < lk->psets.size(); ++k) {
             const hh_partset& ps = lk->psets[k];
-            const int64_t tpr = (int64_t)((ps.pcap + HH_PART_TILE - 1) / HH_PART_TILE);
-            HH_LAUNCH(ctx, hh_k_part_hist, grid, 512, 0, ps.buf, ps.pcap, ps.cursor, lk->npart_log, tpr, lk->d_spill,
-                      k == 0 ? (int64_t)n_spill : 0, blog, d_bcnt);
+            const int64_t ns = k == 0 ? (int64_t)n_spill : 0;
+            HH_CHECK(ps.narrow ? links_launch_hist<hh_nrec>(lk, ps, ns, blog, d_bcnt) : links_launch_hist<int4>(lk, ps, ns, blog, d_bcnt));
         }
         HH_CHECK(hh_exclusive_scan_i32(ctx, reinterpret_cast<const int*>(d_bcnt), d_boff, nb));
         for (size_t k = 0; k < lk->psets.size(); ++k) {
             const hh_partset& ps = lk->psets[k];
-            const int64_t tpr = (int64_t)((ps.pcap + HH_PART_TILE - 1) / HH_PART_TILE);
-            HH_LAUNCH(ctx, hh_k_part_scatter2, grid2, 512, HH_STAGE_SMEM, ps.buf, ps.pcap, ps.cursor, lk->npart_log, tpr, lk->d_spill,
-                      k == 0 ? (int64_t)n_spill : 0, blog, d_boff, d_bfill, d_rec2, compact_cap, lk->d_counters);
+            const int64_t ns = k == 0 ? (int64_t)n_spill : 0;
+            auto scatter2 = ps.narrow ? (narrow ? links_launch_scatter2<hh_nrec, hh_nrec> : links_launch_scatter2<hh_nrec, int4>)
+                                      : (narrow ? links_launch_scatter2<int4, hh_nrec> : links_launch_scatter2<int4, int4>);
+            HH_CHECK(scatter2(lk, ps, ns, blog, d_boff, d_bfill, d_rec2, compact_cap));
         }
         links_free_partsets(lk);
         HH_CHECK(hh_ws_alloc(ctx, &d_stage_compact, (size_t)compact_cap * HH_E_WORDS));
         HH_CUDA(cudaMemsetAsync(lk->d_counters + 0, 0, sizeof(unsigned long long), ctx->stream));
         HH_CUDA(cudaMemsetAsync(lk->d_counters + 3, 0, sizeof(unsigned long long), ctx->stream));
-        int kbits = 1;
-        while ((1ll << kbits) < (int64_t)lk->n_ctg) kbits++;
-        auto count = 2 * kbits <= 32 ? links_bucket_count<uint32_t, 8> : links_bucket_count<uint64_t, 5>;
+        const int kbits = lk->kbits;
+        auto count = narrow ? links_bucket_count<uint32_t, 8, hh_nrec>
+                            : 2 * kbits <= 32 ? links_bucket_count<uint32_t, 8, int4> : links_bucket_count<uint64_t, 5, int4>;
         HH_CHECK(count(lk, d_rec2, d_boff, nb, hot, kbits, d_stage_compact, compact_cap, d_agg, d_fallback));
         unsigned long long agg[4];
         HH_CUDA(cudaMemcpyAsync(agg, d_agg, sizeof(agg), cudaMemcpyDeviceToHost, ctx->stream));
@@ -1552,7 +1664,12 @@
             HH_CUDA(cudaMemcpyAsync(d_fb_off, src_off.data(), (size_t)nf * sizeof(int64_t), cudaMemcpyHostToDevice, ctx->stream));
             HH_CUDA(cudaMemcpyAsync(d_fb_off + nf, pre.data(), ((size_t)nf + 1) * sizeof(int64_t), cudaMemcpyHostToDevice, ctx->stream));
             HH_CHECK(hh_ws_alloc(ctx, &d_fb_rec, (size_t)pre[nf]));
-            HH_LAUNCH(ctx, hh_k_gather_buckets, hh_grid(ctx, 8), 256, 0, d_rec2, d_fb_off, d_fb_off + nf, nf, d_fb_rec);
+            if (narrow)
+                HH_LAUNCH(ctx, hh_k_gather_buckets<hh_nrec>, hh_grid(ctx, 8), 256, 0, reinterpret_cast<const hh_nrec*>(d_rec2), d_fb_off,
+                          d_fb_off + nf, nf, kbits, d_fb_rec);
+            else
+                HH_LAUNCH(ctx, hh_k_gather_buckets<int4>, hh_grid(ctx, 8), 256, 0, reinterpret_cast<const int4*>(d_rec2), d_fb_off,
+                          d_fb_off + nf, nf, kbits, d_fb_rec);
             hh_ws_free(ctx, d_rec2);
             for (int t = 0; t < 2; ++t) HH_CHECK(links_alloc_table(lk, scap, &skeys[t], &svals[t]));
             const int g = hh_grid(ctx, 8);
@@ -1595,6 +1712,14 @@
     lk->finished = true;
     lk->gen++;
     lk->ordered = false;
+    return HH_OK;
+}
+
+extern "C" int hh_links_record_bytes(hh_links* lk, int32_t* set_bytes, int32_t max_sets, int32_t* n_sets, int32_t* bucket_bytes) {
+    HH_REQUIRE(lk != nullptr && (max_sets <= 0 || set_bytes), HH_ERR_ARG, "hh_links_record_bytes: NULL argument");
+    for (int32_t k = 0; k < max_sets && k < (int32_t)lk->set_bytes.size(); ++k) set_bytes[k] = lk->set_bytes[k];
+    if (n_sets) *n_sets = (int32_t)lk->set_bytes.size();
+    if (bucket_bytes) *bucket_bytes = lk->bucket_bytes;
     return HH_OK;
 }
 
diff --git a/haphic_b200/links.py b/haphic_b200/links.py
--- a/haphic_b200/links.py
+++ b/haphic_b200/links.py
@@ -97,6 +97,13 @@
         b, s, f = C.c_int64(), C.c_int64(), C.c_int64()
         check(load().hh_links_agg_info(self._h, C.byref(b), C.byref(s), C.byref(f)))
         return {"buckets": int(b.value), "smem_buckets": int(s.value), "fallback_buckets": int(f.value)}
+
+    def record_bytes(self) -> dict:
+        n, b = C.c_int32(), C.c_int32()
+        check(load().hh_links_record_bytes(self._h, None, 0, C.byref(n), C.byref(b)))
+        sets = (C.c_int32 * max(1, n.value))()
+        check(load().hh_links_record_bytes(self._h, sets, n.value, C.byref(n), C.byref(b)))
+        return {"sets": [int(x) for x in sets[:n.value]], "buckets": int(b.value)}
 
     def fetch(self, pinned: bool = False) -> dict:
         if self.info is None:
diff --git a/include/haphic_b200.h b/include/haphic_b200.h
--- a/include/haphic_b200.h
+++ b/include/haphic_b200.h
@@ -56,6 +56,7 @@
 
 int hh_links_finish(hh_links* lk, hh_links_info* info);
 int hh_links_agg_info(hh_links* lk, int64_t* buckets, int64_t* smem_buckets, int64_t* fallback_buckets);
+int hh_links_record_bytes(hh_links* lk, int32_t* set_bytes, int32_t max_sets, int32_t* n_sets, int32_t* bucket_bytes);
 
 int hh_links_fetch(hh_links* lk, int32_t* key_i, int32_t* key_j, uint32_t* full, uint32_t* flank,
                    uint32_t* first_full, uint32_t* first_flank, uint32_t* ht);
```

Result: faster. 6.418 billion, median of 6 (+4.0%).
